# near/near-light-client

Measured on AMD Instinct MI355X. Metric: Sync/Verify proofs/sec at 1/2/4/8 MI355X + achieved HBM GB/s vs roofline, higher is better.
Workload: dtype u64 (Goldilocks field, integer)

## Files before the change

### include/nlx.h

```cpp
#ifndef NLX_H
#define NLX_H
#include <stddef.h>
#include <stdint.h>

#ifdef __cplusplus
extern "C" {
#endif

#define NLX_OK 0
#define NLX_E_INVAL (-1)
#define NLX_E_NOMEM (-2)
#define NLX_E_HIP (-3)
#define NLX_E_RANGE (-4)
#define NLX_E_UNSUPPORTED (-5)

typedef struct nlx_ctx nlx_ctx;
typedef struct nlx_commit nlx_commit;

uint32_t nlx_version(void);
const char* nlx_strerror(int32_t code);
void nlx_field_generators(uint64_t out[2]);
int32_t nlx_abi_selftest(int32_t kind);

int32_t nlx_ctx_create(int device, nlx_ctx** out);
void nlx_ctx_destroy(nlx_ctx* ctx);
const char* nlx_last_error(const nlx_ctx* ctx);
int32_t nlx_ctx_set_stream(nlx_ctx* ctx, void* hip_stream);
int32_t nlx_ctx_synchronize(nlx_ctx* ctx);
int32_t nlx_ctx_set_priority(nlx_ctx* ctx, int high);
int32_t nlx_ctx_set_cu_mask(nlx_ctx* ctx, const uint32_t* mask, uint32_t n_words);
typedef struct nlx_buf nlx_buf;
int32_t nlx_buf_create(nlx_ctx* ctx, size_t bytes, nlx_buf** out);
void nlx_buf_destroy(nlx_buf* buf);
void* nlx_buf_device_ptr(const nlx_buf* buf);
size_t nlx_buf_size(const nlx_buf* buf);
int32_t nlx_buf_upload(nlx_buf* buf, size_t offset, const void* src, size_t bytes);
int32_t nlx_buf_download(nlx_buf* buf, size_t offset, void* dst, size_t bytes);
int32_t nlx_ctx_memory(const nlx_ctx* ctx, size_t* reserved_bytes, size_t* in_use_bytes);
int32_t nlx_ctx_trim(nlx_ctx* ctx);
int32_t nlx_ctx_kernel_timing(nlx_ctx* ctx, int enable);
int32_t nlx_ctx_kernel_stats(nlx_ctx* ctx, const char* name, uint64_t* calls, double* total_ms, double* alg_bytes);
int32_t nlx_ctx_kernel_units(nlx_ctx* ctx, const char* name, double* units);

int32_t nlx_field_ops(nlx_ctx* ctx, const uint64_t* a, const uint64_t* b, size_t n, uint64_t* out);

int32_t nlx_poseidon_permute_batch(nlx_ctx* ctx, uint64_t* states, size_t n);

int32_t nlx_hash_rows(nlx_ctx* ctx, const uint64_t* rows, size_t n_rows, size_t row_len, uint64_t* digests_out);

size_t nlx_merkle_digest_words(size_t n_leaves, uint32_t cap_height);
int32_t nlx_merkle_build(nlx_ctx* ctx, const uint64_t* leaves, size_t n_leaves, size_t leaf_len,
                         uint32_t cap_height, uint64_t* digests_out, uint64_t* cap_out);

int32_t nlx_poseidon_bn128_permute_batch(nlx_ctx* ctx, uint64_t* states, size_t n);
int32_t nlx_poseidon_bn128_hash_rows(nlx_ctx* ctx, const uint64_t* rows, size_t n_rows, size_t row_len, uint64_t* digests_out);
int32_t nlx_poseidon_bn128_merkle_build(nlx_ctx* ctx, const uint64_t* leaves, size_t n_leaves, size_t leaf_len, uint32_t cap_height,
                                        uint64_t* digests_out, uint64_t* cap_out);

int32_t nlx_ntt_batch(nlx_ctx* ctx, uint64_t* cols, size_t n_cols, uint32_t log_n, int inverse,
                      uint64_t coset_shift);

int32_t nlx_ntt_split_level(nlx_ctx* ctx, uint64_t* mine, const uint64_t* theirs, size_t n_cols, uint32_t log_n, uint32_t world_log,
                            uint32_t rank, uint32_t level);

#define NLX_BN254_MONTGOMERY 1u
int32_t nlx_bn254_ntt_batch(nlx_ctx* ctx, uint64_t* cols, size_t n_cols, uint32_t log_n, int inverse, uint32_t flags);
#define NLX_BN254_BITREV_OUT 2u
#define NLX_BN254_BITREV_IN 4u
int32_t nlx_bn254_ntt_batch_coset(nlx_ctx* ctx, uint64_t* cols, size_t n_cols, uint32_t log_n, int inverse, uint32_t flags,
                                  const uint64_t* coset_shift);
int32_t nlx_bn254_msm_g1(nlx_ctx* ctx, const uint64_t* points, const uint64_t* scalars, uint64_t n, uint32_t flags, uint64_t out[8]);
int32_t nlx_bn254_msm_g2(nlx_ctx* ctx, const uint64_t* points, const uint64_t* scalars, uint64_t n, uint32_t flags, uint64_t out[16]);
int32_t nlx_bn254_g1_sum(const uint64_t* points, uint64_t n, uint64_t out[8]);
int32_t nlx_bn254_g2_sum(const uint64_t* points, uint64_t n, uint64_t out[16]);
int32_t nlx_bn254_g1_multiples(nlx_ctx* ctx, const uint64_t base[8], uint64_t n, uint64_t* out);

typedef struct {
    uint32_t log_n;
    uint32_t flags;
    const uint64_t *ql, *qr, *qm, *qo, *qk;
    const uint64_t *s1, *s2, *s3;
    const uint64_t *l, *r, *o;
    const uint64_t *z;
    const uint64_t *pi;
    const uint64_t *coset_shift, *k1, *k2;
    const uint64_t *alpha, *beta, *gamma;
    const uint64_t *blinding;
    uint32_t n_commit;
    const uint64_t *const *qcp;
    const uint64_t *const *pi2;
} nlx_bn254_plonk_quotient_args;
#define NLX_BN254_PLONK_BLINDED 0x100u
#define NLX_BN254_PLONK_COMMIT 0x200u
#define NLX_BN254_PLONK_MAX_COMMIT 4u
int32_t nlx_bn254_plonk_quotient(nlx_ctx* ctx, const nlx_bn254_plonk_quotient_args* args, uint64_t* t_out, int32_t* high_chunk_is_zero);
int32_t nlx_bn254_plonk_grand_product(nlx_ctx* ctx, uint32_t log_n, const uint64_t* l, const uint64_t* r, const uint64_t* o,
                                      const uint64_t* s1, const uint64_t* s2, const uint64_t* s3, const uint64_t beta[4],
// ... 366 lines not shown
```

### near-light-client_amd/__init__.py

```python
from . import _lib as lib
from ._lib import Context, DeviceBuffer, NlxError, GOLDILOCKS_P
from .batch import PolynomialBatch, MerkleTree, poseidon_permute, hash_rows, poseidon_bn128_permute, poseidon_bn128_hash_rows, ntt, field_ops, bn254_ntt, bn254_pack, bn254_unpack, BN254_R, bn254_msm_g1, bn254_g1_pack, bn254_g1_unpack, bn254_g1_sum, bn254_g1_multiples, bn254_g2_pack, bn254_g2_unpack, bn254_msm_g2, bn254_g2_sum, BN254_Q, bn254_plonk_quotient, bn254_kzg_open
from .plonk import CircuitConfig, CircuitData, SyntheticCircuit, WitnessReport, pow_grind, batch_prove, ProveJob
from .stark import Air, Stark, StarkConfig, StarkProver, TraceReport, fibonacci_air, fibonacci_trace, wide_air, wide_trace
from . import sha256_air, sha512_air, logup, fp25519, ed25519_air, nearx_io, near_protocol, stark, plonk, succinct_io, split_ntt, bn254_plonk, bn254_groth16
```

### near-light-client_amd/_lib.py

```python
import ctypes
import os

import numpy as np

GOLDILOCKS_P = 0xFFFFFFFF00000001
_HERE = os.path.dirname(os.path.abspath(__file__))
_GEN_SET = os.environ.get("NLX_GL_GENERATOR_SET", "7")
LIB_PATH = os.path.join(_HERE, "libnlx.so" if _GEN_SET == "7" else "libnlx_gen%s.so" % _GEN_SET)
if os.environ.get("NLX_BUILD_VARIANT"):
    LIB_PATH = LIB_PATH[:-3] + "_" + os.environ["NLX_BUILD_VARIANT"] + ".so"

if os.environ.get("NLX_SKIP_TORCH_PRELOAD") != "1":
    try:
        import torch
    except Exception:
        pass

if not os.path.exists(LIB_PATH):
    raise ImportError(
        "nlx_amd: HIP extension %s not found. Build it with `python near-light-client_amd/build.py` "
        "(or __graft_entry__.build()). There is no CPU fallback." % LIB_PATH)

_dll = ctypes.CDLL(LIB_PATH, mode=ctypes.RTLD_GLOBAL)
SYNTH_LIB_PATH = os.path.join(_HERE, os.path.basename(LIB_PATH).replace("libnlx", "libnlx_synth", 1))
if not os.path.exists(SYNTH_LIB_PATH):
    raise ImportError("nlx_amd: %s not found. Build it with `python near-light-client_amd/build.py`." % SYNTH_LIB_PATH)
_synth_dll = ctypes.CDLL(SYNTH_LIB_PATH)

u64p = ctypes.POINTER(ctypes.c_uint64)
c_void_pp = ctypes.POINTER(ctypes.c_void_p)

SIGNATURES = {
    "nlx_version": (ctypes.c_uint32, []),
    "nlx_strerror": (ctypes.c_char_p, [ctypes.c_int32]),
    "nlx_abi_selftest": (ctypes.c_int32, [ctypes.c_int32]),
    "nlx_field_generators": (None, [ctypes.POINTER(ctypes.c_uint64)]),
    "nlx_ctx_create": (ctypes.c_int32, [ctypes.c_int, c_void_pp]),
    "nlx_ctx_destroy": (None, [ctypes.c_void_p]),
    "nlx_last_error": (ctypes.c_char_p, [ctypes.c_void_p]),
    "nlx_ctx_set_stream": (ctypes.c_int32, [ctypes.c_void_p, ctypes.c_void_p]),
    "nlx_ctx_synchronize": (ctypes.c_int32, [ctypes.c_void_p]),
    "nlx_ctx_set_priority": (ctypes.c_int32, [ctypes.c_void_p, ctypes.c_int]),
    "nlx_ctx_set_cu_mask": (ctypes.c_int32, [ctypes.c_void_p, ctypes.POINTER(ctypes.c_uint32), ctypes.c_uint32]),
    "nlx_buf_create": (ctypes.c_int32, [ctypes.c_void_p, ctypes.c_size_t, c_void_pp]),
    "nlx_buf_destroy": (None, [ctypes.c_void_p]),
    "nlx_buf_device_ptr": (ctypes.c_void_p, [ctypes.c_void_p]),
    "nlx_buf_size": (ctypes.c_size_t, [ctypes.c_void_p]),
    "nlx_buf_upload": (ctypes.c_int32, [ctypes.c_void_p, ctypes.c_size_t, ctypes.c_void_p, ctypes.c_size_t]),
    "nlx_buf_download": (ctypes.c_int32, [ctypes.c_void_p, ctypes.c_size_t, ctypes.c_void_p, ctypes.c_size_t]),
    "nlx_ctx_memory": (ctypes.c_int32, [ctypes.c_void_p, ctypes.POINTER(ctypes.c_size_t), ctypes.POINTER(ctypes.c_size_t)]),
    "nlx_ctx_trim": (ctypes.c_int32, [ctypes.c_void_p]),
    "nlx_ctx_kernel_timing": (ctypes.c_int32, [ctypes.c_void_p, ctypes.c_int]),
    "nlx_ctx_kernel_stats": (ctypes.c_int32, [ctypes.c_void_p, ctypes.c_char_p, ctypes.POINTER(ctypes.c_uint64),
                                              ctypes.POINTER(ctypes.c_double), ctypes.POINTER(ctypes.c_double)]),
    "nlx_ctx_kernel_units": (ctypes.c_int32, [ctypes.c_void_p, ctypes.c_char_p, ctypes.POINTER(ctypes.c_double)]),
    "nlx_field_ops": (ctypes.c_int32, [ctypes.c_void_p, ctypes.c_void_p, ctypes.c_void_p, ctypes.c_size_t, ctypes.c_void_p]),
    "nlx_poseidon_permute_batch": (ctypes.c_int32, [ctypes.c_void_p, ctypes.c_void_p, ctypes.c_size_t]),
    "nlx_hash_rows": (ctypes.c_int32, [ctypes.c_void_p, ctypes.c_void_p, ctypes.c_size_t, ctypes.c_size_t,
                                       ctypes.c_void_p]),
    "nlx_merkle_digest_words": (ctypes.c_size_t, [ctypes.c_size_t, ctypes.c_uint32]),
    "nlx_merkle_build": (ctypes.c_int32, [ctypes.c_void_p, ctypes.c_void_p, ctypes.c_size_t, ctypes.c_size_t,
                                          ctypes.c_uint32, ctypes.c_void_p, ctypes.c_void_p]),
    "nlx_poseidon_bn128_permute_batch": (ctypes.c_int32, [ctypes.c_void_p, ctypes.c_void_p, ctypes.c_size_t]),
    "nlx_poseidon_bn128_hash_rows": (ctypes.c_int32, [ctypes.c_void_p, ctypes.c_void_p, ctypes.c_size_t, ctypes.c_size_t,
                                                      ctypes.c_void_p]),
    "nlx_poseidon_bn128_merkle_build": (ctypes.c_int32, [ctypes.c_void_p, ctypes.c_void_p, ctypes.c_size_t, ctypes.c_size_t,
                                                         ctypes.c_uint32, ctypes.c_void_p, ctypes.c_void_p]),
    "nlx_ntt_batch": (ctypes.c_int32, [ctypes.c_void_p, ctypes.c_void_p, ctypes.c_size_t, ctypes.c_uint32,
                                       ctypes.c_int, ctypes.c_uint64]),
    "nlx_ntt_split_level": (ctypes.c_int32, [ctypes.c_void_p, ctypes.c_void_p, ctypes.c_void_p, ctypes.c_size_t, ctypes.c_uint32, ctypes.c_uint32,
                                              ctypes.c_uint32, ctypes.c_uint32]),
    "nlx_bn254_ntt_batch": (ctypes.c_int32, [ctypes.c_void_p, ctypes.c_void_p, ctypes.c_size_t, ctypes.c_uint32, ctypes.c_int,
                                              ctypes.c_uint32]),
    "nlx_bn254_ntt_batch_coset": (ctypes.c_int32, [ctypes.c_void_p, ctypes.c_void_p, ctypes.c_size_t, ctypes.c_uint32, ctypes.c_int,
                                                    ctypes.c_uint32, ctypes.c_void_p]),
    "nlx_bn254_msm_g1": (ctypes.c_int32, [ctypes.c_void_p, ctypes.c_void_p, ctypes.c_void_p, ctypes.c_uint64, ctypes.c_uint32,
                                           ctypes.c_void_p]),
    "nlx_bn254_g1_sum": (ctypes.c_int32, [ctypes.c_void_p, ctypes.c_uint64, ctypes.c_void_p]),
    "nlx_bn254_g2_sum": (ctypes.c_int32, [ctypes.c_void_p, ctypes.c_uint64, ctypes.c_void_p]),
    "nlx_bn254_msm_g2": (ctypes.c_int32, [ctypes.c_void_p, ctypes.c_void_p, ctypes.c_void_p, ctypes.c_uint64, ctypes.c_uint32,
                                           ctypes.c_void_p]),
    "nlx_bn254_g1_multiples": (ctypes.c_int32, [ctypes.c_void_p, ctypes.c_void_p, ctypes.c_uint64, ctypes.c_void_p]),
    "nlx_bn254_plonk_quotient": (ctypes.c_int32, [ctypes.c_void_p, ctypes.c_void_p, ctypes.c_void_p, ctypes.POINTER(ctypes.c_int32)]),
    "nlx_bn254_plonk_grand_product": (ctypes.c_int32, [ctypes.c_void_p, ctypes.c_uint32] + [ctypes.c_void_p] * 11 + [ctypes.POINTER(ctypes.c_int32)]),
    "nlx_bn254_fr_lincomb": (ctypes.c_int32, [ctypes.c_void_p, ctypes.c_uint64, ctypes.c_uint32, ctypes.c_void_p, ctypes.c_void_p, ctypes.c_void_p]),
    "nlx_bn254_groth16_quotient": (ctypes.c_int32, [ctypes.c_void_p, ctypes.c_uint32] + [ctypes.c_void_p] * 5),
    "nlx_bn254_kzg_open": (ctypes.c_int32, [ctypes.c_void_p, ctypes.c_void_p, ctypes.c_uint64, ctypes.c_void_p, ctypes.c_void_p,
                                            ctypes.c_void_p, ctypes.c_void_p, ctypes.c_void_p]),
    "nlx_bn254_groth16_key_create": (ctypes.c_int32, [ctypes.c_void_p, ctypes.c_void_p, c_void_pp]),
    "nlx_bn254_groth16_key_destroy": (None, [ctypes.c_void_p]),
    "nlx_bn254_groth16_key_info": (ctypes.c_int32, [ctypes.c_void_p, ctypes.c_void_p]),
    "nlx_bn254_r1cs_eval": (ctypes.c_int32, [ctypes.c_void_p] * 6),
    "nlx_bn254_groth16_prove": (ctypes.c_int32, [ctypes.c_void_p] * 11),
    "nlx_bn254_groth16_key_create_committed": (ctypes.c_int32, [ctypes.c_void_p, ctypes.c_void_p, ctypes.c_void_p, c_void_pp]),
    "nlx_bn254_groth16_commit": (ctypes.c_int32, [ctypes.c_void_p, ctypes.c_void_p, ctypes.c_uint32, ctypes.c_void_p, ctypes.c_void_p]),
    "nlx_bn254_groth16_prove_committed": (ctypes.c_int32, [ctypes.c_void_p] * 14),
    "nlx_bn254_plonk_key_create": (ctypes.c_int32, [ctypes.c_void_p, ctypes.c_void_p, c_void_pp]),
    "nlx_bn254_plonk_key_destroy": (None, [ctypes.c_void_p]),
    "nlx_bn254_plonk_key_info": (ctypes.c_int32, [ctypes.c_void_p, ctypes.c_void_p]),
    "nlx_bn254_plonk_key_commitments": (ctypes.c_int32, [ctypes.c_void_p, ctypes.c_void_p]),
    "nlx_bn254_plonk_proof_bytes": (ctypes.c_size_t, [ctypes.c_void_p]),
    "nlx_bn254_plonk_commit": (ctypes.c_int32, [ctypes.c_void_p, ctypes.c_void_p, ctypes.c_uint32, ctypes.c_void_p, ctypes.c_void_p,
                                                 ctypes.c_void_p, ctypes.c_void_p]),
    "nlx_bn254_plonk_prove": (ctypes.c_int32, [ctypes.c_void_p] * 6 + [ctypes.c_uint64, ctypes.c_void_p, ctypes.c_void_p, ctypes.c_void_p,
                                                                       ctypes.c_size_t, ctypes.POINTER(ctypes.c_size_t)]),
    "nlx_bn254_fr_eval_many": (ctypes.c_int32, [ctypes.c_void_p, ctypes.c_uint32, ctypes.c_void_p, ctypes.c_void_p, ctypes.c_void_p,
                                                 ctypes.c_void_p]),
    "nlx_bn254_hash_to_field": (ctypes.c_int32, [ctypes.c_void_p, ctypes.c_size_t, ctypes.c_void_p, ctypes.c_size_t, ctypes.c_void_p]),
    "nlx_commit_from_values": (ctypes.c_int32, [ctypes.c_void_p, ctypes.c_void_p, ctypes.c_size_t, ctypes.c_uint32,
# ... 239 lines not shown
```

### near-light-client_amd/airgen.py

```python
import os
import sys
import types

import numpy as np

HERE = os.path.dirname(os.path.abspath(__file__))
OUT_DIR = os.path.join(HERE, "csrc", "airgen")
P = 0xFFFFFFFF00000001
MASK64 = (1 << 64) - 1

(LOCAL, NEXT, PUBLIC, CONST, ADD, SUB, MUL, EMIT_TRANSITION, EMIT_FIRST, EMIT_LAST, EMIT, PERIODIC, PACK_LOCAL, PACK_NEXT, EMIT_BOOL,
 LOADV, XOR3, CH, MAJ, SEGMENT, EMIT_LOGUP, MAC) = range(22)


def program_hash(words):
    h = 0xcbf29ce484222325
    for b in np.ascontiguousarray(words, dtype="<u8").tobytes():
        h = ((h ^ b) * 0x100000001b3) & MASK64
    return h


def canonical_words(words):
    out, i = [int(w) for w in words], 0
    while i < len(out):
        if (out[i] & 0xFF) == CONST:
            out[i + 1] %= P
            i += 2
        else:
            i += 1
    return np.array(out, dtype=np.uint64)


def _segments(words):
    segs, lo, i = [], 0, 0
    while i < len(words):
        op = int(words[i]) & 0xFF
        if op == SEGMENT:
            segs.append((lo, i))
            lo = i + 1
        i += 2 if op == CONST else 1
    segs.append((lo, len(words)))
    return segs


def _emit_constraint(lines, expr):
    lines.append("    c = %s;" % expr)
    lines.append("    acc0 = gl::add(gl::mul(acc0, g.a0), c); acc1 = gl::add(gl::mul(acc1, g.a1), c);")


SCHED_EVERY = 4


def _segment_body(words, lo, hi):
    L, i, since = [], lo, 0
    R = lambda k: "r%d" % k
    while i < hi:
        if since >= SCHED_EVERY:
            L.append("    __builtin_amdgcn_sched_barrier(0);")
            since = 0
        if (int(words[i]) & 0xFF) in (LOCAL, NEXT, PUBLIC, CONST, ADD, SUB, MUL, PERIODIC, PACK_LOCAL, PACK_NEXT, XOR3, CH, MAJ, MAC):
            since += 1
        w = int(words[i])
        op, dst, a, b, sh = w & 0xFF, (w >> 8) & 0xFFFF, (w >> 24) & 0xFFFF, (w >> 40) & 0xFFFF, (w >> 56) & 0x3F
        i += 1
        if op == LOCAL:
            L.append("    %s = COL(%d, g.row);" % (R(dst), a))
        elif op == NEXT:
            L.append("    %s = COL(%d, g.row_next);" % (R(dst), a))
        elif op == PUBLIC:
            L.append("    %s = PIS(%d);" % (R(dst), a))
        elif op == PERIODIC:
            L.append("    %s = g.per[(size_t)%d * g.per_stride + g.per_off];" % (R(dst), a))
        elif op == CONST:
            L.append("    %s = 0x%016xull;" % (R(dst), int(words[i]) % P))
            i += 1
        elif op == ADD:
            L.append("    %s = gl::add(%s, mul_pow2(%s, %d));" % (R(dst), R(a), R(b), sh) if sh else "    %s = gl::add(%s, %s);" % (R(dst), R(a), R(b)))
        elif op == SUB:
            L.append("    %s = gl::sub(%s, mul_pow2(%s, %d));" % (R(dst), R(a), R(b), sh) if sh else "    %s = gl::sub(%s, %s);" % (R(dst), R(a), R(b)))
        elif op == MUL:
            L.append("    %s = gl::mul(%s, %s);" % (R(dst), R(a), R(b)))
        elif op == MAC:
            L.append("    %s = gl::add(%s, gl::mul(%s, %s));" % (R(dst), R(sh), R(a), R(b)))
        elif op == CH:
            L.append("    %s = gl::add(%s, gl::mul(%s, gl::sub(%s, %s)));" % (R(dst), R(sh), R(a), R(b), R(sh)))
        elif op in (XOR3, MAJ):
            L.append("    { const uint64_t xy = gl::mul(%s, %s), sx = gl::sub(gl::add(%s, %s), gl::add(xy, xy));" % (R(a), R(b), R(a), R(b)))
            if op == XOR3:
                L.append("      const uint64_t sz = gl::mul(sx, %s); %s = gl::sub(gl::add(sx, %s), gl::add(sz, sz)); }" % (R(sh), R(dst), R(sh)))
            else:
                L.append("      %s = gl::add(xy, gl::mul(%s, sx)); }" % (R(dst), R(sh)))
        elif op in (PACK_LOCAL, PACK_NEXT):
            row = "g.row" if op == PACK_LOCAL else "g.row_next"
            L.append("    { uint64_t v[%d];" % b)
            for k in range(b):
                L.append("      v[%d] = COL(%d, %s);" % (k, a + k, row))
            L.append("      uint64_t acc = 0;")
            for k in range(b):
                L.append("      acc = gl::add(acc, mul_pow2(v[%d], %d));" % (k, k))
            L.append("      %s = acc; }" % R(dst))
        elif op == EMIT_BOOL:
            cnt = b if b else 1
            for i0 in range(0, cnt, 8):
                m = min(8, cnt - i0)
                L.append("    { uint64_t v[%d];" % m)
                for k in range(m):
                    L.append("      v[%d] = COL(%d, g.row);" % (k, a + i0 + k))
                for k in range(m):
                    L.append("      c = gl::mul(v[%d], gl::sub(v[%d], 1)); acc0 = gl::add(gl::mul(acc0, g.a0), c); acc1 = gl::add(gl::mul(acc1, g.a1), c);" % (k, k))
                L.append("    }")
        elif op == EMIT_LOGUP:
            L.append("    { const uint64_t al0 = PIS(g.n_pis + %d), al1 = PIS(g.n_pis + %d);" % (sh, sh + 1))
            L.append("      const uint64_t h0 = COL(%d, g.row), h1 = COL(%d, g.row), v1 = COL(%d, g.row);" % (b, b + 1, a))
            L.append("      uint64_t c0, c1;")
            if dst == 0xFFFF:
                L.append("      const uint64_t d0 = gl::add(al0, v1);")
                L.append("      c0 = gl::sub(gl::add(gl::mul(h0, d0), mul_pow2(gl::mul(h1, al1), 3)), gl::add(gl::mul(h1, al1), 1));")
                L.append("      c1 = gl::add(gl::mul(h0, al1), gl::mul(h1, d0));")
            else:
                L.append("      const uint64_t v2 = COL(%d, g.row);" % dst)
                L.append("      const uint64_t s2 = gl::add(gl::add(al0, al0), gl::add(v1, v2));")
                L.append("      const uint64_t a1sq = gl::mul(al1, al1);")
                L.append("      const uint64_t u0 = gl::add(gl::mul(gl::add(al0, v1), gl::add(al0, v2)), gl::sub(mul_pow2(a1sq, 3), a1sq));")
                L.append("      const uint64_t u1 = gl::mul(al1, s2);")
                L.append("      const uint64_t hu = gl::mul(h1, u1);")
                L.append("      c0 = gl::sub(gl::add(gl::mul(h0, u0), gl::sub(mul_pow2(hu, 3), hu)), s2);")
                L.append("      c1 = gl::sub(gl::add(gl::mul(h0, u1), gl::mul(h1, u0)), gl::add(al1, al1));")
            L.append("      acc0 = gl::add(gl::mul(gl::add(gl::mul(acc0, g.a0), c0), g.a0), c1);")
            L.append("      acc1 = gl::add(gl::mul(gl::add(gl::mul(acc1, g.a1), c0), g.a1), c1); }")
        elif op == LOADV:
            L.append("    __builtin_amdgcn_sched_barrier(0);")
        elif op == EMIT_TRANSITION:
            _emit_constraint(L, "gl::mul(%s, g.z_last)" % R(a))
        elif op == EMIT_FIRST:
            _emit_constraint(L, "gl::mul(%s, g.l_first)" % R(a))
        elif op == EMIT_LAST:
            _emit_constraint(L, "gl::mul(%s, g.l_last)" % R(a))
        elif op == EMIT:
            _emit_constraint(L, R(a))
        else:
            raise ValueError("unknown opcode %d at word %d" % (op, i - 1))
    return L


def _registers_of(words, lo, hi):
    regs, i = set(), lo
    while i < hi:
        w = int(words[i])
        op = w & 0xFF
        if op in (LOCAL, NEXT, PUBLIC, CONST, ADD, SUB, MUL, PERIODIC, PACK_LOCAL, PACK_NEXT, XOR3, CH, MAJ, MAC):
            regs.add((w >> 8) & 0xFFFF)
        i += 2 if op == CONST else 1
    return sorted(regs)


PART_WORDS = 10000


def generate_sources(name, words):
    words = canonical_words(words)
    h = program_hash(words)
    segs = _segments(words)
    parts, cur, cur_words = [], [], 0
    for lo, hi in segs:
        if cur and cur_words + (hi - lo) > PART_WORDS:
            parts.append(cur)
            cur, cur_words = [], 0
        cur.append((lo, hi))
        cur_words += hi - lo
    parts.append(cur)
    files = {}
    for pi, part in enumerate(parts):
        ns = "airgen_%s_p%d" % (name, pi)
        out = ["// GENERATED by near-light-client_amd/airgen.py from the program words of AIR '%s' (%d words, %d segments, hash 0x%016x):" % (name, len(words), len(segs), h),
               "// part %d of %d, segments starting at words %s." % (pi + 1, len(parts), ", ".join(str(lo) for lo, _ in part)),
               "// Do not edit: the interpreter k_air_quotient (stark.hip) runs the same words and is the parity reference.",
               '#include "../air_vm.hpp"', "", "namespace nlx {", "namespace %s {" % ns, "",
               "// what a segment needs of the point: passed BY VALUE (registers); the wave-uniform members are made scalar again inside",
               "// the function (readfirstlane), so a column's base address is a scalar load and its element ONE vector load",
               "// The column-pointer table and the public inputs are the same for every lane and constant for the launch: read through the",
               "// constant address space they are scalar loads (s_load), and a column's value is then ONE global load with the pointer in",
               "// SGPRs and the row's byte offset in a VGPR.  Through plain pointers hipcc made each a per-lane flat load with a wait",
               "// between the pointer and the value (two memory latencies per column, two more VGPRs per load in flight).",
               "// row / row_next are BYTE offsets (LDE rows * 8 < 2^32: the host selects these kernels for LDEs of <= 2^28 rows only).",
               "typedef const uint64_t __attribute__((address_space(4)))* airgen_kptr;",
               "typedef const char __attribute__((address_space(1)))* airgen_gptr;",
               "#define COL(c, off) (*(const uint64_t __attribute__((address_space(1)))*)((airgen_gptr)((airgen_kptr)g.cols)[c] + (off)))",
               "#define PIS(i) (((airgen_kptr)g.pis)[i])",
               "struct G {", "    uint64_t cols, pis; const uint64_t* per;",
               "    size_t per_stride, per_off; uint64_t a0, a1, z_last, l_first, l_last; uint32_t row, row_next, n_pis;", "};",
               "struct Acc { uint64_t a0, a1; };",
               "template <typename T> __device__ __forceinline__ T* uni(T* p) {",
               "    const uint64_t v = (uint64_t)p;",
               "    return (T*)(((uint64_t)(uint32_t)__builtin_amdgcn_readfirstlane((int)(v >> 32)) << 32) | (uint32_t)__builtin_amdgcn_readfirstlane((int)v));",
               "}",
               "__device__ __forceinline__ uint64_t uni(uint64_t v) {",
               "    return ((uint64_t)(uint32_t)__builtin_amdgcn_readfirstlane((int)(v >> 32)) << 32) | (uint32_t)__builtin_amdgcn_readfirstlane((int)v);",
               "}", ""]
        for lo, hi in part:
            regs = _registers_of(words, lo, hi)
            out.append("static __device__ __noinline__ Acc seg_%d(G gv) {" % lo)
            out.append("    G g = gv;")
            out.append("    g.cols = uni(gv.cols); g.pis = uni(gv.pis); g.per = uni(gv.per); g.per_stride = uni((uint64_t)gv.per_stride);")
            out.append("    g.a0 = uni(gv.a0); g.a1 = uni(gv.a1); g.n_pis = (uint32_t)__builtin_amdgcn_readfirstlane((int)gv.n_pis);")
            out.append("    uint64_t c, acc0 = 0, acc1 = 0;")
            if regs:
                out.append("    uint64_t %s;" % ", ".join("r%d" % r for r in regs))
            out += _segment_body(words, lo, hi)
            out.append("    return Acc{acc0, acc1};")
            out.append("}")
            out.append("")
        out += [
            "// the interpreter's prologue and epilogue (csrc/stark.hip k_air_quotient), the program between them as a switch on the segment",
            "__global__ __launch_bounds__(AIRGEN_BLOCK) void kernel(AirParams p) {",
            "    const uint32_t sg = blockIdx.y;",
            "    const uint32_t first = p.n_seg > 1 ? p.seg[2 * sg] : 0u;",
            "    if (%s) return;   // another part's segment" % " && ".join("first != %du" % lo for lo, _ in part),
            "    const size_t pos = (size_t)blockIdx.x * blockDim.x + threadIdx.x;",
            "    const unsigned log_Q = p.log_n + p.qdb;",
            "    if (pos >> log_Q) return;",
            "    const size_t n = (size_t)1 << p.log_n;",
            "    const uint32_t rq = (uint32_t)(pos >> p.log_n), k = (uint32_t)(pos & (n - 1));",
            "    const uint32_t r = rq << (p.rate_bits - p.qdb);",
            "    const size_t qrow_next = ((size_t)rq << p.log_n) + ((k + 1) & (n - 1));",
            "    const uint64_t x = gl::mul(p.coset_base[rq], root_pow_(p.w_n_table, k, (uint32_t)(n >> 1)));",
            "    const uint64_t zh = gl::inv(p.zh_inv[rq]);",
            "    G g;",
            "    g.cols = (uint64_t)p.cols; g.pis = (uint64_t)p.pis; g.per = p.periodic; g.n_pis = p.n_pis;",
            "    g.row = (uint32_t)((((size_t)r << p.log_n) + k) << 3); g.row_next = (uint32_t)((((size_t)r << p.log_n) + ((k + 1) & (n - 1))) << 3);",
            "    g.per_stride = (size_t)1 << (p.qdb + p.period_bits);",
            "    g.per_off = ((size_t)rq << p.period_bits) + (k & ((1u << p.period_bits) - 1));",
            "    g.a0 = p.alphas[0]; g.a1 = p.alphas[1];",
            "    g.z_last = gl::sub(x, p.g_inv); g.l_first = gl::mul(zh, p.l_inv[pos]); g.l_last = gl::mul(zh, p.l_inv[qrow_next]);",
            "    Acc acc{0, 0};",
            "    switch (first) {",
        ]
        for lo, _ in part:
            out.append("        case %d: acc = seg_%d(g); break;" % (lo, lo))
        out += [
            "        default: break;",
            "    }",
            "    const size_t Q = (size_t)1 << log_Q;",
            "    if (p.n_seg > 1) {",
            "        uint64_t* dst = p.part + (((size_t)sg * p.nc) << log_Q) + pos;",
            "        dst[0] = gl::mul(acc.a0, p.seg_mul[2 * sg]);",
            "        dst[Q] = gl::mul(acc.a1, p.seg_mul[2 * sg + 1]);",
            "        return;",
            "    }",
            "    const uint64_t zi = p.zh_inv[rq];",
            "    p.out[pos] = gl::mul(acc.a0, zi);",
            "    p.out[Q + pos] = gl::mul(acc.a1, zi);",
            "}",
            "",
            "}  // namespace %s" % ns,
            "void airgen_launch_%s_p%d(hipStream_t st, unsigned tiles, unsigned n_segments, const AirParams& p) {" % (name, pi),
            "    hipLaunchKernelGGL(%s::kernel, dim3(tiles, n_segments), dim3(AIRGEN_BLOCK), 0, st, p);" % ns,
            "}",
            "}  // namespace nlx", ""]
        files["air_%s_p%d.hip" % (name, pi)] = "\n".join(out)
    main = ["// GENERATED by near-light-client_amd/airgen.py: AIR '%s' (%d words, %d segments in %d parts, hash 0x%016x)." % (name, len(words), len(segs), len(parts), h),
            '#include "../air_vm.hpp"', "", "namespace nlx {"]
    main += ["void airgen_launch_%s_p%d(hipStream_t st, unsigned tiles, unsigned n_segments, const AirParams& p);" % (name, pi) for pi in range(len(parts))]
    main += ["static void airgen_launch_%s(hipStream_t st, unsigned tiles, unsigned n_segments, const AirParams& p) {" % name]
    main += ["    airgen_launch_%s_p%d(st, tiles, n_segments, p);" % (name, pi) for pi in range(len(parts))]
    main += ["}",
             "#if !defined(__HIP_DEVICE_COMPILE__)   // a host object (it holds a host function's address): not for the device pass",
             'extern const AirGenEntry airgen_entry_%s = {0x%016xull, %du, "%s", airgen_launch_%s};' % (name, h, len(words), name, name),
             "#endif",
             "}  // namespace nlx", ""]
    files["air_%s.hip" % name] = "\n".join(main)
    return files


def registry_source(names):
    out = ["// GENERATED by near-light-client_amd/airgen.py: the table nlx_stark_build searches (csrc/air_vm.hpp airgen_find).",
           '#include "../air_vm.hpp"', "", "namespace nlx {"]
    out += ["extern const AirGenEntry airgen_entry_%s;" % n for n in names]
    out += ["", "#if !defined(__HIP_DEVICE_COMPILE__)", "const AirGenEntry* airgen_find(uint64_t program_hash, uint32_t n_words) {",
            "    static const AirGenEntry* const table[] = {%s};" % ", ".join(["&airgen_entry_%s" % n for n in names] + ["nullptr"]),
            "    for (const AirGenEntry* const* e = table; *e; e++)",
            "        if ((*e)->program_hash == program_hash && (*e)->n_words == n_words) return *e;",
            "    return nullptr;", "}", "#endif", "}  // namespace nlx", ""]
    return "\n".join(out)


# ... 54 lines not shown
```

### near-light-client_amd/batch.py

```python
import ctypes

import numpy as np

from ._lib import dll, ptr


def poseidon_permute(ctx, states):
    s = np.ascontiguousarray(states, dtype=np.uint64).copy()
    if s.ndim != 2 or s.shape[1] != 12:
        raise ValueError("states must have shape (n, 12)")
    ctx.check(dll.nlx_poseidon_permute_batch(ctx.handle, ptr(s), s.shape[0]))
    return s


def field_ops(ctx, a, b):
    a = np.ascontiguousarray(a, dtype=np.uint64)
    b = np.ascontiguousarray(b, dtype=np.uint64)
    out = np.zeros((5, a.size), dtype=np.uint64)
    ctx.check(dll.nlx_field_ops(ctx.handle, ptr(a), ptr(b), a.size, ptr(out)))
    return out


def hash_rows(ctx, rows):
    r = np.ascontiguousarray(rows, dtype=np.uint64)
    out = np.zeros((r.shape[0], 4), dtype=np.uint64)
    ctx.check(dll.nlx_hash_rows(ctx.handle, ptr(r), r.shape[0], r.shape[1], ptr(out)))
    return out


def ntt(ctx, cols, inverse=False, coset_shift=1):
    c = np.ascontiguousarray(cols, dtype=np.uint64).copy()
    n = c.shape[1]
    log_n = n.bit_length() - 1
    if 1 << log_n != n:
        raise ValueError("length must be a power of two")
    ctx.check(dll.nlx_ntt_batch(ctx.handle, ptr(c), c.shape[0], log_n, 1 if inverse else 0, int(coset_shift)))
    return c


HASHERS = {"poseidon_goldilocks": 0, "poseidon_bn128": 1}


def _hasher_id(hasher):
    if hasher not in HASHERS:
        raise ValueError("hasher must be one of %s" % ", ".join(sorted(HASHERS)))
    return HASHERS[hasher]


class MerkleTree:

    def __init__(self, ctx, leaves, cap_height, hasher="poseidon_goldilocks"):
        build = (dll.nlx_merkle_build, dll.nlx_poseidon_bn128_merkle_build)[_hasher_id(hasher)]
        lv = np.ascontiguousarray(leaves, dtype=np.uint64)
        self.n_leaves, self.leaf_len = lv.shape
        self.cap_height = cap_height
        self.hasher = hasher
        words = dll.nlx_merkle_digest_words(self.n_leaves, cap_height)
        if words == 0:
            raise ValueError("n_leaves must be a power of two")
        self.digests = np.zeros(words, dtype=np.uint64)
        self.cap = np.zeros((1 << cap_height, 4), dtype=np.uint64)
        ctx.check(build(ctx.handle, ptr(lv), self.n_leaves, self.leaf_len, cap_height, ptr(self.digests), ptr(self.cap)))
        self.leaves = lv

    def prove(self, leaf_index):
        sib, off, lvl, idx = [], 0, self.n_leaves, leaf_index
        while lvl > (1 << self.cap_height):
            s = off + (idx ^ 1) * 4
            sib.append(self.digests[s:s + 4].copy())
            off += lvl * 4
            lvl >>= 1
            idx >>= 1
# ... 362 lines not shown
```

### near-light-client_amd/build.py

```python
import os
import subprocess
import sys
from concurrent.futures import ThreadPoolExecutor

HERE = os.path.dirname(os.path.abspath(__file__))
CSRC = os.path.join(HERE, "csrc")
GEN_SET = os.environ.get("NLX_GL_GENERATOR_SET", "7")
if GEN_SET not in ("7", "2021"):
    raise RuntimeError("NLX_GL_GENERATOR_SET must be 7 or 2021")
_SUFFIX = "" if GEN_SET == "7" else "_gen" + GEN_SET
VARIANT = os.environ.get("NLX_BUILD_VARIANT", "")
if VARIANT:
    _SUFFIX += "_" + VARIANT
OBJ = os.path.join(CSRC, ".obj" + _SUFFIX)
LIB = os.path.join(HERE, "libnlx%s.so" % _SUFFIX)
SYNTH_SOURCES = ("synth.cpp",)
SYNTH_LIB = os.path.join(HERE, "libnlx_synth%s.so" % _SUFFIX)
HIPCC = os.environ.get("HIPCC", "/opt/rocm/bin/hipcc")
ARCH = "gfx950"
FLAGS = ["-O3", "-std=c++17", "-fPIC", "--offload-arch=" + ARCH, "-Xarch_host", "-mavx2", "-Wall", "-Wno-unused-function",
         "-I", os.path.join(HERE, "..", "include"), "-DNLX_GL_GENERATOR_SET=" + GEN_SET] + os.environ.get("NLX_EXTRA_FLAGS", "").split()


AIRGEN = os.path.join(CSRC, "airgen")


def _generate_air_kernels():
    r = subprocess.run([sys.executable, os.path.join(HERE, "airgen.py")], capture_output=True, text=True)
    if r.returncode != 0:
        raise RuntimeError("airgen.py failed:\n%s\n%s" % (r.stdout, r.stderr))


WITH_AIRGEN = GEN_SET == "7" and os.environ.get("NLX_NO_AIRGEN", "") != "1"
if not WITH_AIRGEN:
    FLAGS.append("-DNLX_NO_AIRGEN")


def _sources():
    top = sorted(f for f in os.listdir(CSRC) if f.endswith((".hip", ".cpp")))
    gen = sorted(os.path.join("airgen", f) for f in os.listdir(AIRGEN) if f.endswith(".hip")) if WITH_AIRGEN and os.path.isdir(AIRGEN) else []
    return top + gen


def _headers_mtime(only=None):
    m = 0.0
    for root in (CSRC, os.path.join(HERE, "..", "include")):
        for f in os.listdir(root):
            if f.endswith((".hpp", ".h", ".inc")) and (only is None or f in only):
                m = max(m, os.path.getmtime(os.path.join(root, f)))
    return m


AIRGEN_HEADERS = ("air_vm.hpp", "gl.hpp", "nlx.h", "nlx_field.h")


def _compile(src, verbose):
    obj = os.path.join(OBJ, src.replace(os.sep, "_") + ".o")
    cmd = [HIPCC] + FLAGS + ["-c", os.path.join(CSRC, src), "-o", obj]
    if verbose:
        print(" ".join(cmd), flush=True)
    r = subprocess.run(cmd, capture_output=True, text=True)
    if r.returncode != 0:
        raise RuntimeError("hipcc failed for %s:\n%s\n%s" % (src, r.stdout, r.stderr))
    if verbose and r.stderr.strip():
        print(r.stderr, file=sys.stderr)
    return obj


def build_lib(force=False, verbose=False):
    os.makedirs(OBJ, exist_ok=True)
    if WITH_AIRGEN:
        _generate_air_kernels()
    hm, hm_gen = _headers_mtime(), _headers_mtime(AIRGEN_HEADERS)
    todo, objs, synth_objs = [], [], []
    for src in _sources():
        obj = os.path.join(OBJ, src.replace(os.sep, "_") + ".o")
        (synth_objs if src in SYNTH_SOURCES else objs).append(obj)
        sm = max(os.path.getmtime(os.path.join(CSRC, src)), hm_gen if src.startswith("airgen" + os.sep) else hm)
        if force or not os.path.exists(obj) or os.path.getmtime(obj) < sm:
            todo.append(src)
    if todo:
        todo.sort(key=lambda s_: -os.path.getsize(os.path.join(CSRC, s_)))
        with ThreadPoolExecutor(max_workers=min(8, len(todo))) as ex:
            list(ex.map(lambda s: _compile(s, verbose), todo))
    for lib, members in ((LIB, objs), (SYNTH_LIB, synth_objs)):
        if todo or not os.path.exists(lib):
            cmd = [HIPCC, "-shared", "-fPIC", "--offload-arch=" + ARCH, "-o", lib] + members + os.environ.get("NLX_EXTRA_LDFLAGS", "").split()
            if verbose:
                print(" ".join(cmd), flush=True)
            r = subprocess.run(cmd, capture_output=True, text=True)
            if r.returncode != 0:
                raise RuntimeError("link failed:\n%s\n%s" % (r.stdout, r.stderr))
    return LIB


if __name__ == "__main__":
    print(build_lib(force="--force" in sys.argv, verbose=True))
```

### near-light-client_amd/csrc/air_vm.hpp

```cpp
#pragma once
#include <hip/hip_runtime.h>
#include <cstdint>
#include "gl.hpp"
#include "nlx.h"

namespace nlx {

struct AirParams {
    const uint64_t* const* cols;
    const uint64_t* program;
    const uint64_t* pis;
    const uint64_t* coset_base;
    const uint64_t* zh_inv;
    const uint64_t* l_inv;
    const uint64_t* periodic;
    const uint64_t* w_n_table;
    uint64_t* out;
    const uint32_t* seg;
    const uint64_t* seg_mul;
    uint64_t* part;
    uint32_t n_seg;
    uint64_t alphas[2];
    uint64_t g_inv;
    uint32_t log_n, rate_bits, qdb, n_words, nc, n_regs, period_bits, n_pis;
};

__device__ __forceinline__ uint64_t mul_pow2(uint64_t x, uint32_t sh) {
    if (sh == 0) return x;
    return gl::reduce128(x << sh, x >> (64 - sh));
}

__device__ __forceinline__ uint64_t root_pow_(const uint64_t* __restrict__ half_table, uint32_t e, uint32_t half) {
    return e < half ? half_table[e] : gl::P - half_table[e - half];
}


struct AirGenEntry {
    uint64_t program_hash;
    uint32_t n_words;
    const char* name;
    void (*launch)(hipStream_t st, unsigned tiles, unsigned n_segments, const AirParams& p);
};
constexpr unsigned AIRGEN_BLOCK = 256;
inline uint64_t airgen_program_hash(const uint64_t* words, size_t n) {
    uint64_t h = 0xcbf29ce484222325ull;
    for (size_t i = 0; i < n; i++)
        for (int b = 0; b < 8; b++) {
            h ^= (words[i] >> (8 * b)) & 0xFF;
            h *= 0x100000001b3ull;
        }
    return h;
}
#if defined(NLX_NO_AIRGEN)
inline const AirGenEntry* airgen_find(uint64_t, uint32_t) { return nullptr; }
#else
const AirGenEntry* airgen_find(uint64_t program_hash, uint32_t n_words);
#endif

}
```

### near-light-client_amd/csrc/commit.hip

```cpp
#include "commit.hpp"
#include "gl.hpp"
#include "poly.hpp"

namespace nlx {

size_t merkle_digest_words(size_t n_leaves, uint32_t cap_height) {
    size_t w = 0, lvl = n_leaves, cap = (size_t)1 << cap_height;
    for (;;) {
        w += lvl * 4;
        if (lvl <= cap) break;
        lvl >>= 1;
    }
    return w;
}

nlx_commit commit_view(const nlx_commit* c, uint32_t k) {
    nlx_commit v = *c;
    v.owner = false;
    v.n_trees = 1;
    v.group_digests = nullptr;
    if (c->n_trees > 1) {
        const uint32_t c0 = k * c->batch_cols;
        v.n_cols = c->n_cols - c0 < c->batch_cols ? c->n_cols - c0 : c->batch_cols;
        v.coeffs_br = c->coeffs_br + (size_t)c0 * c->n();
// ... 101 lines not shown
        ctx->end_kernel();
    } else {
        ctx->begin_kernel("hash_lde_leaves", 8.0 * n_cols * L + 32.0 * L, n_cols <= 4 ? 0.0 : (double)L * ((n_cols + 7) / 8));
        launch_hash_lde_leaves(st, c->lde, L, n_cols, log_n, rate_bits, c->digests);
        ctx->end_kernel();
    }
    if (!bn128) {
        ctx->begin_kernel("merkle_levels", 64.0 * L * c->n_trees, ((double)L - (double)((size_t)1 << cap_height)) * c->n_trees);
        c->cap = launch_merkle_levels(st, c->digests, L, cap_height, c->n_trees, c->tree_words);
        ctx->end_kernel();
    }
    hipError_t e = hipGetLastError();
    if (e != hipSuccess) {
        ctx->release(c->coeffs_br);
        ctx->release(c->lde);
        ctx->release(c->digests);
        ctx->release(c->group_digests);
        delete c;
        return ctx->hip_fail(e, "commit_build launch");
    }
    *out = c;
    return NLX_OK;
}

static int32_t copy_out(nlx_ctx* ctx, void* user, const void* dev, size_t bytes) {
    hipError_t e = hipMemcpyAsync(user, dev, bytes, is_device_ptr(user) ? hipMemcpyDeviceToDevice : hipMemcpyDeviceToHost,
                                  ctx->stream);
    if (e != hipSuccess) return ctx->hip_fail(e, "hipMemcpyAsync(out)");
    return NLX_OK;
}

}

using namespace nlx;

extern "C" {

int32_t nlx_field_ops(nlx_ctx* ctx, const uint64_t* a, const uint64_t* b, size_t n, uint64_t* out) NLX_TRY {
    if (!ctx) return NLX_E_INVAL;
    if (n == 0) return NLX_OK;
    if (!a || !b || !out) return ctx->fail(NLX_E_INVAL, "NULL buffer");
    (void)hipSetDevice(ctx->device);
    Staged sa(ctx, a, n * 8, true, false), sb(ctx, b, n * 8, true, false), so(ctx, out, 5 * n * 8, false, true);
    if (sa.status) return sa.status;
    if (sb.status) return sb.status;
    if (so.status) return so.status;
    launch_field_ops(ctx->stream, sa.as<uint64_t>(), sb.as<uint64_t>(), n, so.as<uint64_t>());
    int32_t rc = so.finish();
    if (rc) return rc;
    NLX_HIP(ctx, hipStreamSynchronize(ctx->stream));
    return NLX_OK;
} NLX_CATCH(ctx)

int32_t nlx_poseidon_permute_batch(nlx_ctx* ctx, uint64_t* states, size_t n) NLX_TRY {
    if (!ctx) return NLX_E_INVAL;
    if (n == 0) return NLX_OK;
    if (!states) return ctx->fail(NLX_E_INVAL, "states is NULL");
    (void)hipSetDevice(ctx->device);
    Staged s(ctx, states, n * 12 * 8, true, true);
    if (s.status) return s.status;
    launch_permute_batch(ctx->stream, s.as<uint64_t>(), n);
    int32_t rc = s.finish();
    if (rc) return rc;
    NLX_HIP(ctx, hipStreamSynchronize(ctx->stream));
    return NLX_OK;
} NLX_CATCH(ctx)

int32_t nlx_hash_rows(nlx_ctx* ctx, const uint64_t* rows, size_t n_rows, size_t row_len, uint64_t* digests_out) NLX_TRY {
    if (!ctx) return NLX_E_INVAL;
    if (n_rows == 0) return NLX_OK;
    if (!digests_out || (!rows && row_len)) return ctx->fail(NLX_E_INVAL, "NULL buffer");
    if (row_len > 0xFFFFFFFFull) return ctx->fail(NLX_E_RANGE, "row_len too large");
    (void)hipSetDevice(ctx->device);
    Staged in(ctx, rows, n_rows * row_len * 8, true, false);
    Staged out(ctx, digests_out, n_rows * 32, false, true);
    if (in.status) return in.status;
    if (out.status) return out.status;
    launch_hash_leaves_rowmajor(ctx->stream, in.as<uint64_t>(), (uint32_t)row_len, n_rows, out.as<uint64_t>());
    int32_t rc = out.finish();
    if (rc) return rc;
    NLX_HIP(ctx, hipStreamSynchronize(ctx->stream));
    return NLX_OK;
} NLX_CATCH(ctx)

size_t nlx_merkle_digest_words(size_t n_leaves, uint32_t cap_height) NLX_TRY {
    if (n_leaves == 0 || (n_leaves & (n_leaves - 1)) || cap_height > 63) return 0;
    return merkle_digest_words(n_leaves, cap_height);
} NLX_CATCH_VALUE(nullptr, 0)

int32_t nlx_merkle_build(nlx_ctx* ctx, const uint64_t* leaves, size_t n_leaves, size_t leaf_len, uint32_t cap_height,
                         uint64_t* digests_out, uint64_t* cap_out) NLX_TRY {
    if (!ctx) return NLX_E_INVAL;
    if (n_leaves == 0 || (n_leaves & (n_leaves - 1))) return ctx->fail(NLX_E_INVAL, "n_leaves must be a power of two");
    if (cap_height > 63 || ((size_t)1 << cap_height) > n_leaves)
        return ctx->fail(NLX_E_RANGE, "cap_height %u exceeds log2(n_leaves)", cap_height);
    if (!cap_out || (!leaves && leaf_len)) return ctx->fail(NLX_E_INVAL, "NULL buffer");
    if (leaf_len > 0xFFFFFFFFull) return ctx->fail(NLX_E_RANGE, "leaf_len too large");
    (void)hipSetDevice(ctx->device);
    size_t words = merkle_digest_words(n_leaves, cap_height);
    Staged in(ctx, leaves, n_leaves * leaf_len * 8, true, false);
    if (in.status) return in.status;
    Scratch scratch(ctx);
    const bool own_dig = !(digests_out && is_device_ptr(digests_out));
    uint64_t* d_dig = own_dig ? scratch.alloc_as<uint64_t>(words * 8) : digests_out;
    if (!d_dig) return NLX_E_NOMEM;
    launch_hash_leaves_rowmajor(ctx->stream, in.as<uint64_t>(), (uint32_t)leaf_len, n_leaves, d_dig);
// ... 261 lines not shown
```

### near-light-client_amd/csrc/gl.hpp

```cpp
#pragma once
#include <stdint.h>
#include <stddef.h>
#include "nlx_field.h"

#if defined(__HIP__)
#include <hip/hip_runtime.h>
#define GL_HD __host__ __device__ __forceinline__
#define GL_H __host__ inline
#else
#define GL_HD inline
#define GL_H inline
#endif

namespace gl {

constexpr uint64_t P = 0xFFFFFFFF00000001ULL;
constexpr uint64_t EPS = 0xFFFFFFFFULL;
constexpr uint64_t GEN = NLX_GL_MULTIPLICATIVE_GROUP_GENERATOR;
constexpr uint64_t POW2_GEN = NLX_GL_POWER_OF_TWO_GENERATOR;
constexpr unsigned TWO_ADICITY = 32;
constexpr uint64_t W = 7;

GL_HD uint64_t mulhi64(uint64_t a, uint64_t b) {
#if defined(__HIP_DEVICE_COMPILE__)
// ... 68 lines not shown
        : "vcc");
    uint64_t r;
    asm("v_mad_u64_u32 %[r], vcc, %[m], 1, %[s]" : [r] "=&v"(r) : [m] "v"(m), [s] "v"(((uint64_t)s1 << 32) | s0) : "vcc");
    return r;
}
#endif
GL_H uint64_t add_loose(uint64_t a, uint64_t c) {
    uint64_t s = a + c;
    return s < a ? s + EPS : s;
}

GL_HD uint64_t reduce128_loose(uint64_t lo, uint64_t hi) {
    uint64_t hi_hi = hi >> 32, hi_lo = hi & EPS;
    uint64_t t0 = lo - hi_hi;
    if (lo < hi_hi) t0 -= EPS;
    uint64_t t1 = (hi_lo << 32) - hi_lo;
    uint64_t r = t0 + t1;
    if (r < t1) r += EPS;
    return r;
}
GL_HD uint64_t reduce128(uint64_t lo, uint64_t hi) { return canon(reduce128_loose(lo, hi)); }

#if defined(__HIP_DEVICE_COMPILE__)
__device__ __forceinline__ uint64_t mul_loose_asm(uint64_t a, uint64_t b) {
    const uint32_t a0 = (uint32_t)a, a1 = (uint32_t)(a >> 32), b0 = (uint32_t)b, b1 = (uint32_t)(b >> 32);
    const uint64_t p0 = (uint64_t)a0 * b0;
    const uint64_t p1 = (uint64_t)a0 * b1 + (p0 >> 32);
    const uint64_t p2 = (uint64_t)a1 * b0 + (uint32_t)p1;
    uint64_t p3 = (uint64_t)a1 * b1 + (p1 >> 32), sink;
    asm("v_mad_u64_u32 %0, %1, %2, 1, %3" : "=v"(p3), "=s"(sink) : "v"((uint32_t)(p2 >> 32)), "v"(p3));
    uint32_t r0, r1, t0;
    const uint32_t w2 = (uint32_t)p3;
    asm("v_sub_co_u32 %[r0], vcc, %[w0], %[w3]\n\t"
        "v_subbrev_co_u32 %[r1], vcc, 0, %[w1], vcc\n\t"
        "v_cndmask_b32_e64 %[t0], 0, -1, vcc\n\t"
        "v_sub_co_u32 %[r0], vcc, %[r0], %[t0]\n\t"
        "v_subbrev_co_u32 %[r1], vcc, 0, %[r1], vcc"
        : [r0] "=&v"(r0), [r1] "=&v"(r1), [t0] "=&v"(t0)
        : [w0] "v"((uint32_t)p0), [w1] "v"((uint32_t)p2), [w3] "v"((uint32_t)(p3 >> 32))
        : "vcc");
    const uint64_t base = ((uint64_t)r1 << 32) | r0;
    uint64_t r;
    uint32_t tm;
    asm("v_mad_u64_u32 %[r], vcc, %[w2], -1, %[base]\n\t"
        "v_cndmask_b32_e64 %[t], 0, -1, vcc\n\t"
        "v_mad_u64_u32 %[r], vcc, %[t], 1, %[r]"
        : [r] "=&v"(r), [t] "=&v"(tm)
        : [w2] "v"(w2), [base] "v"(base)
        : "vcc");
    return r;
}
#endif

GL_HD uint64_t mul_loose(uint64_t a, uint64_t b) {
#if defined(__HIP_DEVICE_COMPILE__)
    return mul_loose_asm(a, b);
#else
    return reduce128_loose(a * b, mulhi64(a, b));
#endif
}
GL_HD uint64_t mul(uint64_t a, uint64_t b) { return canon(mul_loose(a, b)); }
GL_HD uint64_t sqr(uint64_t a) { return mul(a, a); }

GL_HD uint64_t pow(uint64_t b, uint64_t e) {
    uint64_t r = 1;
    while (e) {
        if (e & 1) r = mul(r, b);
        b = sqr(b);
        e >>= 1;
    }
    return r;
}
GL_HD uint64_t exp_pow2(uint64_t a, unsigned k) {
    while (k--) a = sqr(a);
    return a;
}
GL_HD uint64_t inv(uint64_t a) {
    uint64_t t2 = mul(sqr(a), a);
    uint64_t t3 = mul(sqr(t2), a);
    uint64_t t6 = mul(exp_pow2(t3, 3), t3);
    uint64_t t12 = mul(exp_pow2(t6, 6), t6);
    uint64_t t24 = mul(exp_pow2(t12, 12), t12);
    uint64_t t30 = mul(exp_pow2(t24, 6), t6);
    uint64_t t31 = mul(sqr(t30), a);
    uint64_t t32 = mul(sqr(t31), a);
    return mul(exp_pow2(t31, 33), t32);
}
GL_HD uint64_t root_of_unity(unsigned n_log) { return exp_pow2(POW2_GEN, TWO_ADICITY - n_log); }

struct Ext {
    uint64_t a, b;
};
GL_HD Ext ext(uint64_t a, uint64_t b = 0) { return Ext{a, b}; }
GL_HD Ext add(Ext x, Ext y) { return Ext{add(x.a, y.a), add(x.b, y.b)}; }
GL_HD Ext sub(Ext x, Ext y) { return Ext{sub(x.a, y.a), sub(x.b, y.b)}; }
GL_HD Ext mul(Ext x, Ext y) {
    uint64_t bb = mul(x.b, y.b);
    uint64_t c0 = add(mul(x.a, y.a), reduce128(bb * W, mulhi64(bb, W)));
    uint64_t c1 = add(mul(x.a, y.b), mul(x.b, y.a));
    return Ext{c0, c1};
}
GL_HD Ext mul(Ext x, uint64_t s) { return Ext{mul(x.a, s), mul(x.b, s)}; }
GL_HD Ext inv(Ext x) {
    uint64_t n = sub(sqr(x.a), mul(W, sqr(x.b)));
    uint64_t ni = inv(n);
    return Ext{mul(x.a, ni), mul(neg(x.b), ni)};
}
GL_HD Ext pow(Ext b, uint64_t e) {
    Ext r{1, 0};
    while (e) {
        if (e & 1) r = mul(r, b);
        b = mul(b, b);
        e >>= 1;
    }
    return r;
}
GL_HD bool eq(Ext x, Ext y) { return x.a == y.a && x.b == y.b; }

GL_HD uint32_t bitrev32(uint32_t x, unsigned bits) {
#if defined(__HIP_DEVICE_COMPILE__)
    return bits ? (__brev(x) >> (32 - bits)) : 0;
#else
    uint32_t r = 0;
    for (unsigned i = 0; i < bits; i++) r |= ((x >> i) & 1u) << (bits - 1 - i);
    return r;
#endif
}

}
```

### near-light-client_amd/csrc/poly.hpp

```cpp
#pragma once
#include <hip/hip_runtime.h>
#include <stdint.h>
#include <stddef.h>

namespace nlx {
size_t eval_scratch_words(uint32_t n_cols, unsigned log_n);
void launch_eval_br(hipStream_t st, const uint64_t* d_coeffs_br, size_t stride, uint32_t n_cols, unsigned log_n,
                    const uint64_t* d_z, uint64_t* d_out_ext, uint64_t* d_scratch, const uint64_t* d_zpow = nullptr);
void launch_gather_rows(hipStream_t st, const uint64_t* d_lde, size_t col_stride, uint32_t n_cols, unsigned log_n,
                        unsigned rate_bits, const uint64_t* d_idx, size_t k, uint64_t* d_rows_out);
void launch_gather_paths(hipStream_t st, const uint64_t* d_digests, unsigned log_leaves, unsigned cap_height,
                         const uint64_t* d_idx, size_t k, uint64_t* d_paths_out);
void launch_table_to_leaves(hipStream_t st, const uint64_t* d_lde, size_t col_stride, uint32_t n_cols,
                            unsigned log_n, unsigned rate_bits, uint64_t* d_leaves);
void launch_field_ops(hipStream_t st, const uint64_t* d_a, const uint64_t* d_b, size_t n, uint64_t* d_out);
}
```

### near-light-client_amd/csrc/poly_kernels.hip

```cpp
#include <hip/hip_runtime.h>
#include "gl.hpp"
#include "launch.hpp"
#include "poly.hpp"

namespace nlx {

constexpr unsigned EVAL_CHUNK_LOG = 11;

__device__ __forceinline__ gl::Ext shfl_down_ext(gl::Ext v, int d) {
    gl::Ext r;
    r.a = ((uint64_t)__shfl_down((uint32_t)(v.a >> 32), d, 64) << 32) | __shfl_down((uint32_t)v.a, d, 64);
    r.b = ((uint64_t)__shfl_down((uint32_t)(v.b >> 32), d, 64) << 32) | __shfl_down((uint32_t)v.b, d, 64);
    return r;
}

template <bool EXT_IN>
__global__ __launch_bounds__(256) void k_eval_fold(const uint64_t* __restrict__ in, size_t in_stride,
                                                   unsigned log_count,
                                                   unsigned level0,
                                                   unsigned log_n, const uint64_t* __restrict__ zpow,
                                                   uint64_t* __restrict__ out, size_t out_stride) {
    __shared__ uint64_t wave_part[8];
    const unsigned tid = threadIdx.x;
    const unsigned log_chunk = log_count < EVAL_CHUNK_LOG ? log_count : EVAL_CHUNK_LOG;
// ... 234 lines not shown
                       d_idx, k, d_rows_out);
}

__global__ void k_gather_paths(const uint64_t* __restrict__ digests, unsigned log_leaves, unsigned cap_height,
                               const uint64_t* __restrict__ idx, size_t k, uint64_t* __restrict__ paths_out) {
    size_t q = blockIdx.x;
    unsigned path_len = log_leaves - cap_height;
    unsigned lvl = threadIdx.x >> 2, w = threadIdx.x & 3;
    if (q >= k || lvl >= path_len) return;
    if (idx[q] >> log_leaves) return;
    size_t L = (size_t)1 << log_leaves;
    size_t off = 4 * (2 * L - (2 * L >> lvl));
    size_t node = (idx[q] >> lvl) ^ 1;
    paths_out[(q * path_len + lvl) * 4 + w] = digests[off + node * 4 + w];
}
void launch_gather_paths(hipStream_t st, const uint64_t* d_digests, unsigned log_leaves, unsigned cap_height,
                         const uint64_t* d_idx, size_t k, uint64_t* d_paths_out) {
    if (!k || log_leaves <= cap_height) return;
    hipLaunchKernelGGL(k_gather_paths, dim3((unsigned)k), dim3(128), 0, st, d_digests, log_leaves, cap_height, d_idx,
                       k, d_paths_out);
}

__global__ void k_table_to_leaves(const uint64_t* __restrict__ lde, size_t col_stride, uint32_t n_cols,
                                  unsigned log_n, unsigned rate_bits, uint64_t* __restrict__ leaves) {
    size_t leaf = (size_t)blockIdx.x * blockDim.x + threadIdx.x;
    if (leaf >> (log_n + rate_bits)) return;
    size_t pos = leaf_to_pos(leaf, log_n, rate_bits);
    for (uint32_t c = 0; c < n_cols; c++) leaves[leaf * n_cols + c] = lde[(size_t)c * col_stride + pos];
}
void launch_table_to_leaves(hipStream_t st, const uint64_t* d_lde, size_t col_stride, uint32_t n_cols,
                            unsigned log_n, unsigned rate_bits, uint64_t* d_leaves) {
    size_t rows = (size_t)1 << (log_n + rate_bits);
    hipLaunchKernelGGL(k_table_to_leaves, dim3((unsigned)((rows + 255) / 256)), dim3(256), 0, st, d_lde, col_stride,
                       n_cols, log_n, rate_bits, d_leaves);
}

__global__ void k_field_ops(const uint64_t* __restrict__ a, const uint64_t* __restrict__ b, size_t n,
                            uint64_t* __restrict__ out) {
    size_t i = (size_t)blockIdx.x * blockDim.x + threadIdx.x;
    if (i >= n) return;
    const uint64_t ar = a[i], br = b[i];
    const uint64_t x = gl::canon(ar), y = gl::canon(br);
    out[i] = gl::mul(x, y);
    out[n + i] = gl::add(x, y);
    out[2 * n + i] = gl::sub(x, y);
    out[3 * n + i] = x ? gl::inv(x) : 0;
    out[4 * n + i] = gl::canon(gl::mul_loose(ar, br));
}
void launch_field_ops(hipStream_t st, const uint64_t* d_a, const uint64_t* d_b, size_t n, uint64_t* d_out) {
    if (!n) return;
    hipLaunchKernelGGL(k_field_ops, dim3((unsigned)((n + 255) / 256)), dim3(256), 0, st, d_a, d_b, n, d_out);
}

}
```

### near-light-client_amd/csrc/prover.hip

```cpp
#include <algorithm>
#include <cstdlib>
#include <cstring>
#include <vector>
#include "commit.hpp"
#include "gl.hpp"
#include "poly.hpp"
#include "poseidon.hpp"
#include "prover.hpp"
#include "fri.hpp"
#include "transcript.hpp"

using namespace nlx;

namespace {
uint32_t fri_num_rounds(const nlx_circuit_desc& d) {
    return nlx::fri_num_rounds(d.degree_bits, d.rate_bits, d.cap_height, d.fri_arity_bits, d.fri_final_poly_bits);
}

uint32_t gate_num_constraints(const nlx_gate_desc& g) {
    const uint32_t p0 = g.param0, p1 = g.param1;
    switch (g.kind) {
        case NLX_GATE_CONSTANT: case NLX_GATE_ARITHMETIC: return p0;
        case NLX_GATE_PUBLIC_INPUT: return 4;
        case NLX_GATE_BASE_SUM: return 1 + p1;
// ... 127 lines not shown
        if (gt.kind == NLX_GATE_U32_ADD_MANY && (gt.param0 < 1 || gt.param0 > 15 || gt.param1 < 1 || (gt.param0 + 3 + 18) * gt.param1 > d.num_wires))
            return ctx->fail(NLX_E_INVAL, "U32AddManyGate does not fit the wires");
        if (gt.kind == NLX_GATE_U32_ARITHMETIC && (gt.param0 < 1 || (6 + 32) * gt.param0 > d.num_wires)) return ctx->fail(NLX_E_INVAL, "U32ArithmeticGate too wide");
        if (gt.kind == NLX_GATE_U32_SUBTRACTION && (gt.param0 < 1 || (5 + 16) * gt.param0 > d.num_wires)) return ctx->fail(NLX_E_INVAL, "U32SubtractionGate too wide");
        if (gt.kind == NLX_GATE_U32_RANGE_CHECK && (gt.param0 < 1 || 17 * gt.param0 > d.num_wires)) return ctx->fail(NLX_E_INVAL, "U32RangeCheckGate too wide");
        if (gt.kind == NLX_GATE_COMPARISON) {
            const uint32_t cb = gt.param1 ? (gt.param0 + gt.param1 - 1) / gt.param1 : 0;
            if (gt.param1 < 1 || cb < 1 || cb > 3 || cb * gt.param1 > 62 || 4 + 5 * gt.param1 + cb + 1 > d.num_wires)
                return ctx->fail(NLX_E_INVAL, "ComparisonGate: chunk_bits must be in [1, 3] and the gate must fit the wires");
        }
        if (gt.kind == NLX_GATE_COSET_INTERPOLATION) {
            const uint32_t np = gt.param0 <= 5 ? 1u << gt.param0 : 0;
            if (np < 4 || gt.param1 < 2 || gt.param1 > np || d.degree_bits < gt.param0 + 1 ||
                1 + 2 * np + 4 + 4 * ((np - 2) / (gt.param1 - 1)) + 2 > d.num_wires)
                return ctx->fail(NLX_E_INVAL, "CosetInterpolationGate does not fit");
        }
        if (gt.kind == NLX_GATE_RANDOM_ACCESS) {
            const uint32_t bits = gt.param0, copies = gt.param1 & 0xFFFF, extra = gt.param1 >> 16;
            if (bits < 1 || bits > 6 || copies < 1 || extra > d.num_constants ||
                (2 + (1u << bits)) * copies + extra + copies * bits > d.num_wires)
                return ctx->fail(NLX_E_INVAL, "RandomAccessGate does not fit the wires");
        }
        if (gt.kind == NLX_GATE_REDUCING_EXT && (gt.param0 < 1 || 6 + 2 * gt.param0 + 2 * (gt.param0 - 1) > d.num_wires)) return ctx->fail(NLX_E_INVAL, "ReducingExtensionGate too wide");
        if (gt.selector_index >= d.num_selectors || gt.group_end > d.num_gates || gt.group_start > gt.group_end)
            return ctx->fail(NLX_E_INVAL, "gate %u: bad selector group", g);
        if (gt.kind == NLX_GATE_POSEIDON && d.num_wires < 135) return ctx->fail(NLX_E_INVAL, "PoseidonGate needs 135 wires");
        if (gt.kind == NLX_GATE_ARITHMETIC && 4 * gt.param0 > d.num_wires) return ctx->fail(NLX_E_INVAL, "ArithmeticGate too wide");
        if (gt.kind == NLX_GATE_BASE_SUM && 1 + gt.param1 > d.num_wires) return ctx->fail(NLX_E_INVAL, "BaseSumGate too wide");
        if (gt.kind == NLX_GATE_CONSTANT && gt.param0 > d.num_constants) return ctx->fail(NLX_E_INVAL, "ConstantGate too wide");
    }
    if (d.num_luts) {
        if (d.num_luts > 16) return ctx->fail(NLX_E_RANGE, "at most 16 lookup tables");
        if (!d.lut_sizes || !d.lut_pairs || !d.lookup_rows || !d.lut_num_lookups) return ctx->fail(NLX_E_INVAL, "NULL lookup table array");
        const uint32_t n_lu = d.num_routed_wires / 2, n_lut = d.num_routed_wires / 3;
        if (n_lut < 1 || d.quotient_degree_factor < 2) return ctx->fail(NLX_E_INVAL, "too few routed wires for the lookup gates");
        for (uint32_t t = 0; t < d.num_luts; t++) {
            const uint32_t len = d.lut_sizes[t], lookups = d.lut_num_lookups[t];
            const uint32_t last_lu = d.lookup_rows[3 * t], last_lut = d.lookup_rows[3 * t + 1], first_lut = d.lookup_rows[3 * t + 2];
            if (len < 1 || len > 65536 || lookups < 1) return ctx->fail(NLX_E_RANGE, "table %u: 1 .. 65536 entries and at least one lookup", t);
            if (!(last_lu < last_lut && last_lut <= first_lut) || (uint64_t)first_lut + 1 >= ((uint64_t)1 << d.degree_bits))
                return ctx->fail(NLX_E_INVAL, "table %u: lookup rows out of order or past the circuit", t);
            if (last_lut - last_lu != (lookups + n_lu - 1) / n_lu || first_lut - last_lut + 1 != (len + n_lut - 1) / n_lut)
                return ctx->fail(NLX_E_INVAL, "table %u: row counts do not match its lookups / entries", t);
        }
    }
    (void)hipSetDevice(ctx->device);
    nlx_circuit* c = new (std::nothrow) nlx_circuit();
    if (!c) return ctx->fail(NLX_E_NOMEM, "host allocation failed");
    c->ctx = ctx;
    c->d = d;
    c->hasher = hasher;
    c->gates.assign(d.gates, d.gates + d.num_gates);
    for (const nlx_gate_desc& gt : c->gates) c->max_gate_constraints = std::max(c->max_gate_constraints, gate_num_constraints(gt));
    c->k_is.assign(d.k_is, d.k_is + d.num_routed_wires);
    c->d.gates = c->gates.data();
    c->d.k_is = c->k_is.data();
    if (d.num_luts) {
        const uint32_t T = d.num_luts;
        c->lk.num_luts = T;
        c->lk.n_lu_slots = d.num_routed_wires / 2;
        c->lk.n_lut_slots = d.num_routed_wires / 3;
        c->lk.lu_degree = d.quotient_degree_factor - 1;
        c->lk.n_sldc = (c->lk.n_lu_slots + c->lk.lu_degree - 1) / c->lk.lu_degree;
        c->lk.lut_degree = (c->lk.n_lut_slots + c->lk.n_sldc - 1) / c->lk.n_sldc;
        c->n_lk_sel = 4 + T;
        c->n_lk_polys = d.num_challenges * (1 + c->lk.n_sldc);
        c->n_lk_terms = 4 + T + 2 * c->lk.n_sldc;
        c->lut_sizes.assign(d.lut_sizes, d.lut_sizes + T);
        c->lut_num_lookups.assign(d.lut_num_lookups, d.lut_num_lookups + T);
        c->lookup_rows.assign(d.lookup_rows, d.lookup_rows + 3 * T);
        c->lut_offsets.assign(T + 1, 0);
        for (uint32_t t = 0; t < T; t++) c->lut_offsets[t + 1] = c->lut_offsets[t] + c->lut_sizes[t];
        c->lut_pairs.assign(d.lut_pairs, d.lut_pairs + 2 * (size_t)c->lut_offsets[T]);
        c->d.lut_sizes = c->lut_sizes.data(); c->d.lut_num_lookups = c->lut_num_lookups.data();
        c->d.lookup_rows = c->lookup_rows.data(); c->d.lut_pairs = c->lut_pairs.data();
    }
    c->n_consts_all = d.num_selectors + c->n_lk_sel + d.num_constants;
    c->n_cs = c->n_consts_all + d.num_routed_wires;
    c->n_zpp = d.num_challenges * (1 + d.num_partial_products);
    c->n_zs = c->n_zpp + c->n_lk_polys;
    c->n_q = d.num_challenges * d.quotient_degree_factor;
    c->n_fri_rounds = fri_num_rounds(d);
    const size_t n = c->n(), L = c->L();
    const unsigned log_n = d.degree_bits, log_L = d.degree_bits + d.rate_bits;
    const uint32_t R = 1u << d.rate_bits, A = 1u << d.fri_arity_bits;
    int32_t rc = ctx->ensure_tables(log_L);
    auto fail = [&](int32_t code) {
        nlx_circuit_destroy(c);
        return code;
    };
    if (rc) return fail(rc);
    rc = ctx->get_coset_scale(log_n, d.rate_bits, &c->d_inv_scale_br, true);
    if (rc) return fail(rc);
    if (hasher == NLX_HASHER_POSEIDON_BN128) {
        c->d_bad = (uint32_t*)ctx->alloc(256);
        if (!c->d_bad) return fail(NLX_E_NOMEM);
        if (hipMemsetAsync(c->d_bad, 0, 4, ctx->stream) != hipSuccess) return fail(ctx->fail(NLX_E_HIP, "hipMemsetAsync failed"));
    }

    {
        uint64_t* d_vals = (uint64_t*)ctx->alloc((size_t)c->n_cs * n * 8);
        if (!d_vals) return fail(NLX_E_NOMEM);
        const size_t cb = (size_t)c->n_consts_all * n * 8, sb = (size_t)d.num_routed_wires * n * 8;
        hipError_t e1 = hipMemcpyAsync(d_vals, constants, cb, is_device_ptr(constants) ? hipMemcpyDeviceToDevice : hipMemcpyHostToDevice, ctx->stream);
        hipError_t e2 = hipMemcpyAsync((uint8_t*)d_vals + cb, sigmas, sb, is_device_ptr(sigmas) ? hipMemcpyDeviceToDevice : hipMemcpyHostToDevice, ctx->stream);
        if (e1 != hipSuccess || e2 != hipSuccess) { ctx->release(d_vals); return fail(ctx->hip_fail(e1 != hipSuccess ? e1 : e2, "hipMemcpyAsync")); }
// ... 263 lines not shown
    zp.sigmas = c->d_sigma_values;
    zp.k_is = c->d_k_is;
    zp.w_n_table = ctx->tables.fwd[log_n];
    for (int i = 0; i < 2; i++) { zp.betas[i] = betas[i]; zp.gammas[i] = gammas[i]; }
    zp.out = d_zs;
    zp.log_n = log_n; zp.routed = d.num_routed_wires; zp.chunk = d.quotient_degree_factor; zp.nc = d.num_challenges;
    zp.npp = d.num_partial_products;
    launch_zs(ctx->stream, zp, d_zs_scratch);
    if (c->n_lk_polys)
        launch_lookup_polys(ctx->stream, c->lk, c->d_tabs, c->h_tabs.data(), d_wire_values, n, d.num_challenges, d_deltas,
                            d_zs + (size_t)c->n_zpp * n);
    return commit_for(c, d_zs, CommitInput::ValuesNatural, c->n_zs, cz);
}

int32_t quotient_degree_check(nlx_circuit* c, const uint64_t* d_qchunks) {
    nlx_ctx* ctx = c->ctx;
    const nlx_circuit_desc& d = c->d;
    const size_t n = c->n();
    const uint32_t R = 1u << d.rate_bits, nc = d.num_challenges;
    if (n < 2 * (size_t)R) return NLX_OK;
    uint64_t top[2 * 8];
    const size_t stride = n / R;
    int32_t rc = ensure_pinned(ctx, 1u << 20);
    if (rc) return rc;
    for (uint32_t ch = 0; ch < nc; ch++) {
        const uint64_t* src = d_qchunks + ((size_t)ch * R + (R - 1)) * n + (stride - 1);
        NLX_HIP(ctx, hipMemcpy2DAsync((uint64_t*)ctx->pinned + (size_t)ch * R, 8, src, stride * 8, 8, R, hipMemcpyDeviceToHost, ctx->stream));
    }
    NLX_HIP(ctx, hipStreamSynchronize(ctx->stream));
    memcpy(top, ctx->pinned, (size_t)nc * R * 8);
    for (uint32_t i = 0; i < nc * R; i++)
        if (gl::canon(top[i]) != 0)
            return ctx->fail(NLX_E_INVAL, "the witness does not satisfy the circuit: the quotient of challenge %u has degree above %u n - %u (the vanishing polynomial is not divisible by Z_H)",
                             i / R, R, R + 1);
    return NLX_OK;
}

int32_t quotient_stage(nlx_circuit* c, const nlx_commit* cw, const nlx_commit* cz, const uint64_t betas[2],
                       const uint64_t gammas[2], const uint64_t alphas[2], const uint64_t pih[4],
                       const uint64_t* d_deltas, const uint64_t* d_lut_polys, CommitPtr& cq, StageClock& clock, Scratch& scratch) {
    nlx_ctx* ctx = c->ctx;
    const nlx_circuit_desc& d = c->d;
    hipStream_t st = ctx->stream;
    const unsigned log_n = d.degree_bits;
    const size_t L = c->L();
    const uint32_t nc = d.num_challenges, npp = d.num_partial_products;
    c->n_terms = nc + nc * (npp + 1) + nc * c->n_lk_terms + c->max_gate_constraints;
    uint64_t* d_alpha_pows = scratch.alloc_as<uint64_t>((size_t)2 * c->n_terms * 8);
    uint64_t* d_qvals = scratch.alloc_as<uint64_t>((size_t)nc * L * 8);
    uint64_t* d_qchunks = scratch.alloc_as<uint64_t>((size_t)nc * L * 8);
    if (!d_alpha_pows || !d_qvals || !d_qchunks) return NLX_E_NOMEM;
    launch_pow_table(st, d_alpha_pows, alphas[0], alphas[1], c->n_terms, c->n_terms);
    QuotientParams qp{};
    qp.cs = c->cs->lde; qp.wires = cw->lde; qp.zs = cz->lde;
    qp.gates = c->d_gates; qp.k_is = c->d_k_is; qp.coset_base = c->d_coset_base;
    qp.w_n_table = ctx->tables.fwd[log_n];
    qp.zh_inv = c->d_zh_inv; qp.l0_scaled = c->d_l0_scaled; qp.alpha_pows = d_alpha_pows;
    qp.out = d_qvals;
    for (int i = 0; i < 2; i++) { qp.betas[i] = betas[i]; qp.gammas[i] = gammas[i]; }
    for (int i = 0; i < 4; i++) qp.pih[i] = pih[i];
    qp.alpha_stride = c->n_terms;
    qp.num_wires = d.num_wires; qp.work = c->d_work; qp.work_stride = c->work_stride;
    qp.log_n = log_n; qp.rate_bits = d.rate_bits; qp.n_gates = d.num_gates; qp.n_selectors = d.num_selectors;
    qp.n_consts_all = c->n_consts_all; qp.routed = d.num_routed_wires; qp.chunk = d.quotient_degree_factor; qp.nc = nc; qp.npp = npp;
    qp.gate_const0 = d.num_selectors + c->n_lk_sel;
    qp.n_lk_terms = c->n_lk_terms;
    if (c->n_lk_terms) {
        LookupTermsParams lp{};
        lp.cs = c->cs->lde; lp.wires = cw->lde; lp.zs = cz->lde;
        lp.deltas = d_deltas; lp.lut_polys = d_lut_polys; lp.alpha_pows = d_alpha_pows; lp.out = d_qvals;
        lp.alpha_stride = c->n_terms; lp.t_lk = nc + nc * (npp + 1);
        lp.log_n = log_n; lp.rate_bits = d.rate_bits; lp.nc = nc; lp.sel0 = d.num_selectors; lp.lk0 = c->n_zpp;
        lp.n_lk_terms = c->n_lk_terms; lp.s = c->lk;
        ctx->begin_kernel("lookup_terms", 8.0 * L * (c->n_lk_sel + d.num_routed_wires + 2.0 * c->n_lk_polys + nc));
        launch_lookup_terms(st, lp);
        ctx->end_kernel();
        qp.accumulate = 1;
    }
    ctx->begin_kernel("quotient", 8.0 * L * (c->n_cs + d.num_wires + c->n_zs + nc) + 8.0 * L * nc);
    for (uint32_t g : c->poseidon_gates) {
        launch_quotient_poseidon(st, qp, g, qp.accumulate != 0);
        qp.accumulate = 1;
    }
    launch_quotient(st, qp);
    ctx->end_kernel();
    clock.stage("quotient_intt");
    launch_intt_dif_cosets(st, ctx->tables, d_qvals, nc, log_n, d.rate_bits, c->d_inv_scale_br);
    launch_quotient_chunks(st, d_qvals, d_qchunks, log_n, d.rate_bits, nc, c->d_wR_inv, c->d_chunk_scale);
    clock.stage("commit_quotient");
    NLX_RC(commit_for(c, d_qchunks, CommitInput::CoeffsBitrev, c->n_q, cq));
    return c->hasher == NLX_HASHER_POSEIDON_BN128 ? quotient_degree_check(c, d_qchunks) : NLX_OK;
}

struct ProveCall {
    CommitPtr cw, cz, cq;
    uint64_t deltas[8] = {}, lut_polys[2 * 16] = {};
    OpeningPoints points;
    Scratch scratch;
    explicit ProveCall(nlx_ctx* ctx) : scratch(ctx) {}
};

int32_t prove_stages(nlx_circuit* c, ProveCall& pc, const uint64_t* wires, const uint64_t* public_inputs, Writer& w, size_t* proof_len) {
    nlx_ctx* ctx = c->ctx;
    const nlx_circuit_desc& d = c->d;
    hipStream_t st = ctx->stream;
    const size_t n = c->n();
// ... 540 lines not shown
```

### near-light-client_amd/csrc/prover.hpp

```cpp
#pragma once
#include <hip/hip_runtime.h>
#include <stdint.h>
#include <stddef.h>
#include "../../include/nlx.h"

namespace nlx {

struct GateDev {
    uint32_t kind, selector_index, group_start, group_end, index, param0, param1;
};

struct ZsParams {
    const uint64_t* wires;
    size_t wires_stride;
    const uint64_t* sigmas;
    const uint64_t* k_is;
    const uint64_t* w_n_table;
    uint64_t betas[2], gammas[2];
    uint64_t* out;
    uint32_t log_n, routed, chunk, nc, npp;
};
size_t zs_scratch_words(unsigned log_n, uint32_t nc);
void launch_zs(hipStream_t st, const ZsParams& p, uint64_t* d_scratch);

struct QuotientParams {
    const uint64_t* cs;
    const uint64_t* wires;
    const uint64_t* zs;
    const GateDev* gates;
    const uint64_t* k_is;
    const uint64_t* coset_base;
    const uint64_t* w_n_table;
    const uint64_t* zh_inv;
    const uint64_t* l0_scaled;
    const uint64_t* alpha_pows;
    uint64_t* out;
    uint64_t betas[2], gammas[2], pih[4];
    uint32_t alpha_stride;
    uint32_t log_n, rate_bits, n_gates, n_selectors, n_consts_all, routed, chunk, nc, npp;
    uint32_t gate_const0;
    uint32_t n_lk_terms;
    uint32_t accumulate;
    uint32_t num_wires;
    const uint32_t* work;
    uint32_t work_stride;
};
void launch_quotient(hipStream_t st, const QuotientParams& p);
void launch_quotient_poseidon(hipStream_t st, const QuotientParams& p, uint32_t gate, bool add);
size_t quotient_lds_bytes(uint32_t num_wires, uint32_t n_consts_all);
uint32_t quotient_waves();
void launch_l0_table(hipStream_t st, uint64_t* d_out, unsigned log_n, unsigned rate_bits, const uint64_t* d_coset_base,
                     const uint64_t* d_w_n_table);
void launch_quotient_chunks(hipStream_t st, const uint64_t* d_in, uint64_t* d_out, unsigned log_n, unsigned rate_bits,
                            uint32_t nc, const uint64_t* d_w_R_inv_pows, const uint64_t* d_chunk_scale);

struct LookupShape {
    uint32_t num_luts, n_lu_slots, n_lut_slots, lu_degree, lut_degree, n_sldc;
};
struct LookupTableDev {
    uint32_t len, lookups, last_lu, last_lut, first_lut, pad_;
    const uint32_t* pairs;
    const int32_t* idx_of;
    uint32_t* mult;
};
void launch_set_lookup_wires(hipStream_t st, const LookupShape& s, const LookupTableDev* d_tabs, const LookupTableDev* h_tabs,
                             uint64_t* d_wires, size_t n, uint32_t* d_mult_all, size_t mult_words, uint32_t* d_err);
void launch_lookup_polys(hipStream_t st, const LookupShape& s, const LookupTableDev* d_tabs, const LookupTableDev* h_tabs,
                         const uint64_t* d_wires, size_t n, uint32_t nc, const uint64_t* d_deltas, uint64_t* d_cols);
struct LookupTermsParams {
    const uint64_t* cs;
    const uint64_t* wires;
    const uint64_t* zs;
    const uint64_t* deltas;
    const uint64_t* lut_polys;
    const uint64_t* alpha_pows;
    uint64_t* out;
    uint32_t alpha_stride, t_lk;
    uint32_t log_n, rate_bits, nc, sel0, lk0, n_lk_terms;
    LookupShape s;
};
void launch_lookup_terms(hipStream_t st, const LookupTermsParams& p);

struct CheckBlock {
    unsigned long long gate_rows_bad, gate_first;
    unsigned long long copy_cells_bad, copy_first;
    unsigned long long lookup_slots_bad, lookup_first;
    unsigned long long sigma_undecodable;
    unsigned long long gate_value;
// ... 2 lines not shown
constexpr unsigned long long CHECK_NONE = ~0ull;
void launch_check_reset(hipStream_t st, CheckBlock* d_block);
struct CheckGatesParams {
    QuotientParams q;
    const uint64_t* consts;
    const uint64_t* wires;
    CheckBlock* block;
};
void launch_check_gates(hipStream_t st, const CheckGatesParams& p, uint32_t report_row);
void launch_sigma_decode(hipStream_t st, const uint64_t* d_sigmas, const uint64_t* d_k_is, const uint64_t* d_kn, const uint64_t* d_kinv,
                         const uint64_t* d_w_n_table, const uint64_t* d_w_n_inv_table, unsigned log_n, uint32_t routed,
                         uint32_t* d_to_row, uint16_t* d_to_col, CheckBlock* d_block);
void launch_check_copies(hipStream_t st, const uint64_t* d_wires, unsigned log_n, uint32_t routed, const uint32_t* d_to_row,
                         const uint16_t* d_to_col, CheckBlock* d_block);
void launch_check_lookups(hipStream_t st, const LookupShape& s, const LookupTableDev* d_tabs, const LookupTableDev* h_tabs,
                          const uint64_t* d_wires, size_t n, CheckBlock* d_block);

constexpr int FRI_VIEWS = 33;
struct FriCombineParams {
    const uint64_t* tables[FRI_VIEWS];
    uint32_t n_cols[FRI_VIEWS];
    const uint64_t* alpha_pows;
    const uint64_t* coset_base;
    const uint64_t* w_n_table;
    uint64_t zeta[2], gzeta[2], c0[2], c1[2], alpha_nz[2];
    uint64_t* out;
    uint32_t log_n, rate_bits;
    uint32_t nz[FRI_VIEWS];
    uint32_t nz_off[FRI_VIEWS];
};
size_t fri_combine_scratch_words(const FriCombineParams& p);
void launch_fri_combine(hipStream_t st, const FriCombineParams& p, uint64_t* scratch);
void launch_fri_leaves(hipStream_t st, const uint64_t* d_values, unsigned log_n, unsigned rate_bits,
                       unsigned arity_bits, uint64_t* d_digests);
void launch_fri_leaves_wide(hipStream_t st, const uint64_t* d_values, unsigned log_n, unsigned rate_bits,
                            unsigned arity_bits, uint64_t* d_digests);
void launch_fri_fold(hipStream_t st, const uint64_t* d_values, uint64_t* d_out, unsigned log_n, unsigned rate_bits,
                     unsigned arity_bits, const uint64_t beta[2], uint64_t shift_inv, const uint64_t* d_w_L_inv_table,
                     const uint64_t* d_w_A_inv_pows);
void launch_fri_final_coeffs(hipStream_t st, const uint64_t* d_values, unsigned log_n, unsigned rate_bits,
                             uint64_t shift, uint64_t* d_out, uint32_t n_out);

struct PowParams {
    uint64_t state[12];
    uint64_t max_rounds;
    uint32_t pos, bits;
};
void launch_pow_grind(hipStream_t st, const PowParams& p, unsigned long long* d_best);
void launch_fri_gather_leaf(hipStream_t st, const uint64_t* d_values, unsigned log_n, unsigned rate_bits,
                            unsigned arity_bits, const uint64_t* d_leaf_idx, uint32_t n_q, uint64_t* d_out,
                            size_t out_stride_words);
void launch_shift_indices(hipStream_t st, const uint64_t* d_in, uint64_t* d_out, uint32_t n, unsigned shift);
void launch_pow_table(hipStream_t st, uint64_t* d_out, uint64_t a0, uint64_t a1, uint32_t count, uint32_t stride);
void launch_ext_pow_table(hipStream_t st, uint64_t* d_out, const uint64_t alpha[2], uint32_t count);

}
```

### near-light-client_amd/csrc/prover_kernels.hip

```cpp
#include <hip/hip_runtime.h>
#include "gl.hpp"
#include "poseidon.hpp"
#include "poseidon_fast_constants.inc"
#include "prover.hpp"

namespace nlx {

__constant__ static const uint64_t FAST_FIRST[12] = NLX_POSEIDON_FAST_FIRST_RC_INIT;
__constant__ static const uint64_t FAST_RC[22] = NLX_POSEIDON_FAST_RC_INIT;
__constant__ static const uint64_t FAST_VS[22][11] = NLX_POSEIDON_FAST_VS_INIT;
__constant__ static const uint64_t FAST_W[22][11] = NLX_POSEIDON_FAST_W_HATS_INIT;
__constant__ static const uint64_t FAST_INIT[11][11] = NLX_POSEIDON_FAST_INITIAL_MATRIX_INIT;

__device__ __forceinline__ uint64_t root_pow(const uint64_t* __restrict__ half_table, uint32_t e, uint32_t half) {
    return e < half ? half_table[e] : gl::P - half_table[e - half];
}

__global__ __launch_bounds__(256) void k_zs_row_products(ZsParams p) {
    const size_t i = (size_t)blockIdx.x * blockDim.x + threadIdx.x;
    const size_t n = (size_t)1 << p.log_n;
    if (i >= n) return;
    const uint64_t x = root_pow(p.w_n_table, (uint32_t)i, (uint32_t)(n >> 1));
    constexpr int MAXQ = 10;
    uint64_t num[2 * MAXQ], den[2 * MAXQ];
    const uint32_t n_chunks = (p.routed + p.chunk - 1) / p.chunk;
    const uint64_t bx0 = gl::mul(p.betas[0], x), bx1 = gl::mul(p.betas[1], x);
#pragma unroll
    for (int q = 0; q < MAXQ; q++) {
        uint64_t nm0 = 1, dn0 = 1, nm1 = 1, dn1 = 1;
        if ((uint32_t)q < n_chunks) {
            for (uint32_t j = q * p.chunk; j < (q + 1) * p.chunk && j < p.routed; j++) {
                const uint64_t w = p.wires[(size_t)j * p.wires_stride + i];
                const uint64_t sg = p.sigmas[(size_t)j * n + i];
                const uint64_t kj = p.k_is[j];
                nm0 = gl::mul(nm0, gl::add(gl::add(w, gl::mul(bx0, kj)), p.gammas[0]));
                dn0 = gl::mul(dn0, gl::add(gl::add(w, gl::mul(p.betas[0], sg)), p.gammas[0]));
                if (p.nc > 1) {
                    nm1 = gl::mul(nm1, gl::add(gl::add(w, gl::mul(bx1, kj)), p.gammas[1]));
                    dn1 = gl::mul(dn1, gl::add(gl::add(w, gl::mul(p.betas[1], sg)), p.gammas[1]));
                }
            }
        }
        num[q] = nm0;
        den[q] = dn0;
        num[MAXQ + q] = nm1;
        den[MAXQ + q] = dn1;
    }
    uint64_t pref[2 * MAXQ];
    uint64_t acc = 1;
#pragma unroll
    for (int t = 0; t < 2 * MAXQ; t++) {
        pref[t] = acc;
        acc = gl::mul(acc, den[t]);
    }
// ... 60 lines not shown
        run = gl::mul(run, v[k]);
    }
    if (threadIdx.x == 255) totals[(size_t)blockIdx.y * totals_stride + blockIdx.x] = run;
}

__global__ __launch_bounds__(256) void k_scan_mul_apply(uint64_t* __restrict__ data, size_t stride, size_t count,
                                                        const uint64_t* __restrict__ prefix, size_t prefix_stride) {
    const size_t i = (size_t)blockIdx.x * blockDim.x + threadIdx.x;
    if (i >= count) return;
    uint64_t* col = data + (size_t)blockIdx.y * stride;
    const uint64_t f = prefix[(size_t)blockIdx.y * prefix_stride + i / SCAN_ELEMS];
    col[i] = gl::mul(col[i], f);
}

__global__ __launch_bounds__(256) void k_zs_apply(uint64_t* __restrict__ out, unsigned log_n, uint32_t nc, uint32_t npp) {
    const size_t i = (size_t)blockIdx.x * blockDim.x + threadIdx.x;
    const size_t n = (size_t)1 << log_n;
    if (i >= n) return;
    const uint32_t c = blockIdx.y / npp, q = blockIdx.y % npp;
    const uint64_t z = out[(size_t)c * n + i];
    uint64_t* pp = out + (size_t)(nc + c * npp + q) * n;
    pp[i] = gl::mul(pp[i], z);
}

void launch_zs(hipStream_t st, const ZsParams& p, uint64_t* d_scratch) {
    const size_t n = (size_t)1 << p.log_n;
    const unsigned blocks = (unsigned)((n + 255) / 256);
    hipLaunchKernelGGL(k_zs_row_products, dim3(blocks), dim3(256), 0, st, p);
    size_t count = n;
    size_t nb = (count + SCAN_ELEMS - 1) / SCAN_ELEMS;
    uint64_t* tot1 = d_scratch;
    uint64_t* tot2 = d_scratch + p.nc * nb;
    hipLaunchKernelGGL(k_scan_mul_local, dim3((unsigned)nb, p.nc), dim3(256), 0, st, p.out, n, count, tot1, nb);
    if (nb > 1) {
        size_t nb2 = (nb + SCAN_ELEMS - 1) / SCAN_ELEMS;
        hipLaunchKernelGGL(k_scan_mul_local, dim3((unsigned)nb2, p.nc), dim3(256), 0, st, tot1, nb, nb, tot2, nb2);
        if (nb2 > 1) {
            uint64_t* tot3 = tot2 + p.nc * nb2;
            hipLaunchKernelGGL(k_scan_mul_local, dim3(1, p.nc), dim3(256), 0, st, tot2, nb2, nb2, tot3, (size_t)1);
            hipLaunchKernelGGL(k_scan_mul_apply, dim3((unsigned)((nb + 255) / 256), p.nc), dim3(256), 0, st, tot1, nb, nb,
                               tot2, nb2);
        }
        hipLaunchKernelGGL(k_scan_mul_apply, dim3(blocks, p.nc), dim3(256), 0, st, p.out, n, count, tot1, nb);
    }
    hipLaunchKernelGGL(k_zs_apply, dim3(blocks, p.nc * p.npp), dim3(256), 0, st, p.out, p.log_n, p.nc, p.npp);
}
size_t zs_scratch_words(unsigned log_n, uint32_t nc) {
    size_t n = (size_t)1 << log_n;
    size_t nb = (n + SCAN_ELEMS - 1) / SCAN_ELEMS;
    size_t nb2 = (nb + SCAN_ELEMS - 1) / SCAN_ELEMS;
    return nc * (nb + nb2 + 2) + 16;
}

struct GateAcc {
    const uint64_t* __restrict__ ap0;
    const uint64_t* __restrict__ ap1;
    uint64_t a[8];
    uint32_t kc[8];
    uint32_t k;
    uint64_t base[2];
    __device__ __forceinline__ void reset() {
#pragma unroll
        for (int i = 0; i < 8; i++) { a[i] = 0; kc[i] = 0; }
        k = 0;
        base[0] = base[1] = 0;
    }
    __device__ __forceinline__ void stash() {
        base[0] = gl::add(base[0], fold_columns(a, kc));
        base[1] = gl::add(base[1], fold_columns(a + 4, kc + 4));
#pragma unroll
        for (int i = 0; i < 8; i++) { a[i] = 0; kc[i] = 0; }
    }
    __device__ __forceinline__ void emit_at(uint32_t idx, uint64_t c) { mac(c, ap0[idx], ap1[idx]); }
    __device__ __forceinline__ void mac(uint64_t c, uint64_t b0, uint64_t b1) {
        const uint32_t c0 = (uint32_t)c, c1 = (uint32_t)(c >> 32);
        asm("v_mad_u64_u32 %[a0], vcc, %[c0], %[p0], %[a0]\n\t"
            "v_addc_co_u32 %[k0], vcc, 0, %[k0], vcc\n\t"
            "v_mad_u64_u32 %[a1], vcc, %[c0], %[p1], %[a1]\n\t"
            "v_addc_co_u32 %[k1], vcc, 0, %[k1], vcc\n\t"
            "v_mad_u64_u32 %[a2], vcc, %[c1], %[p0], %[a2]\n\t"
            "v_addc_co_u32 %[k2], vcc, 0, %[k2], vcc\n\t"
            "v_mad_u64_u32 %[a3], vcc, %[c1], %[p1], %[a3]\n\t"
            "v_addc_co_u32 %[k3], vcc, 0, %[k3], vcc\n\t"
            "v_mad_u64_u32 %[a4], vcc, %[c0], %[q0], %[a4]\n\t"
            "v_addc_co_u32 %[k4], vcc, 0, %[k4], vcc\n\t"
            "v_mad_u64_u32 %[a5], vcc, %[c0], %[q1], %[a5]\n\t"
            "v_addc_co_u32 %[k5], vcc, 0, %[k5], vcc\n\t"
            "v_mad_u64_u32 %[a6], vcc, %[c1], %[q0], %[a6]\n\t"
            "v_addc_co_u32 %[k6], vcc, 0, %[k6], vcc\n\t"
            "v_mad_u64_u32 %[a7], vcc, %[c1], %[q1], %[a7]\n\t"
            "v_addc_co_u32 %[k7], vcc, 0, %[k7], vcc"
            : [a0] "+v"(a[0]), [a1] "+v"(a[1]), [a2] "+v"(a[2]), [a3] "+v"(a[3]), [a4] "+v"(a[4]), [a5] "+v"(a[5]),
              [a6] "+v"(a[6]), [a7] "+v"(a[7]), [k0] "+v"(kc[0]), [k1] "+v"(kc[1]), [k2] "+v"(kc[2]), [k3] "+v"(kc[3]),
              [k4] "+v"(kc[4]), [k5] "+v"(kc[5]), [k6] "+v"(kc[6]), [k7] "+v"(kc[7])
            : [c0] "v"(c0), [c1] "v"(c1), [p0] "s"((uint32_t)b0), [p1] "s"((uint32_t)(b0 >> 32)), [q0] "s"((uint32_t)b1),
              [q1] "s"((uint32_t)(b1 >> 32))
            : "vcc");
    }
    __device__ __forceinline__ void emit(uint64_t c) { emit_at(k++, c); }
    __device__ __forceinline__ uint64_t finish(int ch) const { return gl::add(fold_columns(a + 4 * ch, kc + 4 * ch), base[ch]); }
    static __device__ __forceinline__ uint64_t fold_columns(const uint64_t* A, const uint32_t* K) {
        uint32_t t1, t2, t3, t4, m0, m1, cm;
        asm("v_add_co_u32 %[m0], vcc, %[a1l], %[a2l]\n\t"
            "v_addc_co_u32 %[m1], vcc, %[a1h], %[a2h], vcc\n\t"
            "v_addc_co_u32 %[cm], vcc, 0, 0, vcc\n\t"
            "v_add_co_u32 %[t1], vcc, %[a0h], %[m0]\n\t"
            "v_addc_co_u32 %[t2], vcc, %[m1], %[a3l], vcc\n\t"
            "v_addc_co_u32 %[t3], vcc, %[cm], %[a3h], vcc\n\t"
            "v_addc_co_u32 %[t4], vcc, 0, %[k3], vcc\n\t"
            "v_add_co_u32 %[t2], vcc, %[t2], %[k0]\n\t"
            "v_addc_co_u32 %[t3], vcc, %[t3], %[k1], vcc\n\t"
            "v_addc_co_u32 %[t4], vcc, 0, %[t4], vcc\n\t"
            "v_add_co_u32 %[t3], vcc, %[t3], %[k2]\n\t"
            "v_addc_co_u32 %[t4], vcc, 0, %[t4], vcc"
            : [t1] "=&v"(t1), [t2] "=&v"(t2), [t3] "=&v"(t3), [t4] "=&v"(t4), [m0] "=&v"(m0), [m1] "=&v"(m1), [cm] "=&v"(cm)
            : [a0h] "v"((uint32_t)(A[0] >> 32)), [a1l] "v"((uint32_t)A[1]), [a1h] "v"((uint32_t)(A[1] >> 32)), [a2l] "v"((uint32_t)A[2]),
              [a2h] "v"((uint32_t)(A[2] >> 32)), [a3l] "v"((uint32_t)A[3]), [a3h] "v"((uint32_t)(A[3] >> 32)), [k0] "v"(K[0]),
              [k1] "v"(K[1]), [k2] "v"(K[2]), [k3] "v"(K[3])
            : "vcc");
        const uint64_t r = gl::canon(gl32::to_u64(gl32::reduce128((uint32_t)A[0], t1, t2, t3)));
        return gl::sub(r, (uint64_t)t4 << 32);
    }
};

struct DotAcc {
    uint64_t a[4];
    uint32_t kc[4];
    __device__ __forceinline__ void reset() {
#pragma unroll
        for (int i = 0; i < 4; i++) { a[i] = 0; kc[i] = 0; }
    }
    __device__ __forceinline__ void mac(uint64_t x, uint64_t c) {
        const uint32_t x0 = (uint32_t)x, x1 = (uint32_t)(x >> 32);
        asm("v_mad_u64_u32 %[a0], vcc, %[x0], %[c0], %[a0]\n\t"
            "v_addc_co_u32 %[k0], vcc, 0, %[k0], vcc\n\t"
            "v_mad_u64_u32 %[a1], vcc, %[x0], %[c1], %[a1]\n\t"
            "v_addc_co_u32 %[k1], vcc, 0, %[k1], vcc\n\t"
            "v_mad_u64_u32 %[a2], vcc, %[x1], %[c0], %[a2]\n\t"
            "v_addc_co_u32 %[k2], vcc, 0, %[k2], vcc\n\t"
            "v_mad_u64_u32 %[a3], vcc, %[x1], %[c1], %[a3]\n\t"
            "v_addc_co_u32 %[k3], vcc, 0, %[k3], vcc"
            : [a0] "+v"(a[0]), [a1] "+v"(a[1]), [a2] "+v"(a[2]), [a3] "+v"(a[3]), [k0] "+v"(kc[0]), [k1] "+v"(kc[1]),
              [k2] "+v"(kc[2]), [k3] "+v"(kc[3])
            : [x0] "v"(x0), [x1] "v"(x1), [c0] "s"((uint32_t)c), [c1] "s"((uint32_t)(c >> 32))
            : "vcc");
    }
    __device__ __forceinline__ uint64_t value() const { return GateAcc::fold_columns(a, kc); }
};

struct Sum128 {
    uint64_t lo = 0, hi = 0;
    __device__ __forceinline__ void add(uint64_t x, uint32_t sh) {
        const uint64_t tl = x << sh, th = sh ? x >> (64 - sh) : 0;
        lo += tl;
        hi += th + (lo < tl ? 1u : 0u);
    }
    __device__ __forceinline__ uint64_t value() const { return gl::reduce128(lo, hi); }
};

__device__ __forceinline__ uint64_t limb4(uint64_t l) {
    const uint64_t u = gl::mul_loose(l, gl::sub(l, 3));
    return gl::mul_loose(u, gl::add_loose(u, 2));
}

__device__ __forceinline__ uint64_t sbox7c(uint64_t x) {
    uint64_t x2 = gl::mul_loose(x, x), x4 = gl::mul_loose(x2, x2), x3 = gl::mul_loose(x, x2);
    const uint64_t r = gl::mul_loose(x3, x4);
    __builtin_amdgcn_sched_barrier(0);
    return r;
}
__device__ __forceinline__ void mds_canon(uint64_t (&s)[12]) {
    constexpr uint32_t C[12] = {17, 15, 41, 16, 2, 28, 13, 13, 39, 18, 34, 20};
    uint64_t o[12];
#pragma unroll
    for (int r = 0; r < 12; r++) {
        uint64_t al = 0, ah = 0;
#pragma unroll
        for (int i = 0; i < 12; i++) {
            al += (uint64_t)(uint32_t)s[(i + r) % 12] * C[i];
            ah += (uint64_t)(uint32_t)(s[(i + r) % 12] >> 32) * C[i];
        }
        if (r == 0) {
            al += (uint64_t)(uint32_t)s[0] * 8u;
            ah += (uint64_t)(uint32_t)(s[0] >> 32) * 8u;
        }
        o[r] = gl::canon(gl32::to_u64(gl32::fold_acc(al, ah)));
        __builtin_amdgcn_sched_barrier(0);
    }
#pragma unroll
    for (int i = 0; i < 12; i++) s[i] = o[i];
}

template <class WireFn, class Acc>
struct GateBlockSboxes {
    Acc& acc;
    WireFn W;
    uint32_t r0;
    __device__ __forceinline__ gl32::F at(uint32_t r, gl32::F computed) const {
        const uint64_t in = W(65 + r);
        acc.emit_at(41 + r, gl::sub(gl32::to_u64(computed), in));
        const gl32::F u = gl32::sbox7(gl32::from_u64(in));
        __builtin_amdgcn_sched_barrier(0);
        return u;
    }
    __device__ __forceinline__ gl32::F first(gl32::F s0) const { return at(r0, s0); }
    __device__ __forceinline__ gl32::F inner(int i, gl32::F w) const { return at(r0 + (uint32_t)i, w); }
    __device__ __forceinline__ void before_matrix_pass() const { acc.stash(); }
};

template <class WireFn, class Acc>
__device__ __forceinline__ void gate_poseidon_mx(WireFn W, Acc& acc, uint32_t parts) {
    const uint64_t* RC = poseidon::RC_DEV;
    const uint64_t* rcb = poseidon::LAYER_RCB_DEV;
    uint32_t lane = threadIdx.x & 63;
    asm("" : "+v"(lane) : "s"(parts));
    const gl32::i32x4_t afrag = gl32::mds_a_fragment(lane);
    gl32::F t[12];
    auto sbox_of_wires = [&](uint32_t w0) {
#pragma unroll
        for (int i = 0; i < 12; i++) {
            t[i] = gl32::sbox7(gl32::from_u64(W(w0 + i)));
            __builtin_amdgcn_sched_barrier(0);
        }
    };
    auto check_against_wires = [&](uint32_t c0, uint32_t w0) {
#pragma unroll
        for (int i = 0; i < 12; i++) {
            acc.emit_at(c0 + i, gl::sub(gl32::to_u64(t[i]), W(w0 + i)));
            __builtin_amdgcn_sched_barrier(0);
        }
    };
    if (parts & 1u) {
        const uint64_t swap = W(24);
        acc.emit_at(0, gl::mul(swap, gl::sub(swap, 1)));
        uint64_t st[12];
#pragma unroll
        for (int i = 0; i < 4; i++) {
            const uint64_t lhs = W(i), rhs = W(i + 4), delta = W(25 + i);
            acc.emit_at(1 + i, gl::sub(gl::mul(swap, gl::sub(rhs, lhs)), delta));
            st[i] = gl::add(lhs, delta);
            st[i + 4] = gl::sub(rhs, delta);
        }
#pragma unroll
        for (int i = 8; i < 12; i++) st[i] = W(i);
#pragma unroll
        for (int i = 0; i < 12; i++) {
            t[i] = gl32::sbox7(gl32::from_u64(gl::add_loose(st[i], RC[i])));
            __builtin_amdgcn_sched_barrier(0);
        }
#pragma unroll 1
        for (int r = 0; r < 3; r++) {
            if (r) sbox_of_wires(29 + 12 * (r - 1));
            gl32::mds_layer_mfma<2>(t, afrag, rcb + (r + 1) * 24);
            check_against_wires(5 + 12 * r, 29 + 12 * r);
        }
    }
    if (parts & 2u) {
        const gl32::BlockOperands op = poseidon::block_operands(lane);
        sbox_of_wires(29 + 24);
        gl32::mds_layer_mfma<2>(t, afrag, rcb + 4 * 24);
#pragma unroll 1
        for (uint32_t b = 0; b < NLX_POSEIDON_N_BLOCKS; b++)
            gl32::partial_block3<NLX_POSEIDON_BLOCK_GAMMA21>(t, op, poseidon::BLOCK_KAPPA_DEV + b * 6, GateBlockSboxes<WireFn, Acc>{acc, W, 3 * b});
        t[0] = GateBlockSboxes<WireFn, Acc>{acc, W, 21}.first(t[0]);
        gl32::mds_layer_mfma<2>(t, afrag, rcb + 26 * 24);
        check_against_wires(63, 87);
    }
    if (parts & 4u) {
#pragma unroll 1
        for (int r = 0; r < 4; r++) {
            sbox_of_wires(87 + 12 * r);
            if (r < 3) {
                gl32::mds_layer_mfma<2>(t, afrag, rcb + (27 + r) * 24);
                check_against_wires(63 + 12 * (r + 1), 87 + 12 * (r + 1));
            } else {
                gl32::mds_layer_mfma<0>(t, afrag, rcb);
                check_against_wires(111, 12);
            }
        }
    }
}

template <class WireFn, class Acc>
__device__ __forceinline__ void gate_poseidon_fast(WireFn W, Acc& acc, uint32_t parts) {
    const uint64_t* RC = poseidon::RC_DEV;
    uint64_t st[12];
    if (parts & 1u) {
        const uint64_t swap = W(24);
        acc.emit_at(0, gl::mul(swap, gl::sub(swap, 1)));
#pragma unroll
        for (int i = 0; i < 4; i++) {
            const uint64_t lhs = W(i), rhs = W(i + 4), delta = W(25 + i);
            acc.emit_at(1 + i, gl::sub(gl::mul(swap, gl::sub(rhs, lhs)), delta));
            st[i] = gl::add(lhs, delta);
            st[i + 4] = gl::sub(rhs, delta);
        }
#pragma unroll
        for (int i = 8; i < 12; i++) st[i] = W(i);
#pragma unroll
        for (int i = 0; i < 12; i++) st[i] = gl::add_loose(st[i], RC[i]);
#pragma unroll 1
        for (int r = 0; r < 3; r++) {
#pragma unroll
            for (int i = 0; i < 12; i++) st[i] = sbox7c(st[i]);
            mds_canon(st);
            __builtin_amdgcn_sched_barrier(0);
#pragma unroll
            for (int i = 0; i < 12; i++) {
                const uint64_t in = W(29 + 12 * r + i);
                acc.emit_at(5 + 12 * r + i, gl::sub(gl::add(st[i], RC[(r + 1) * 12 + i]), in));
                st[i] = in;
                __builtin_amdgcn_sched_barrier(0);
            }
        }
    }
    if (parts & 2u) {
#pragma unroll
        for (int i = 0; i < 12; i++) st[i] = sbox7c(W(29 + 24 + i));
        mds_canon(st);
#pragma unroll
        for (int i = 0; i < 12; i++) st[i] = gl::add(st[i], FAST_FIRST[i]);
        {
            uint64_t res[12];
            res[0] = st[0];
#pragma unroll
            for (int c = 1; c < 12; c++) {
                DotAcc dot;
                dot.reset();
#pragma unroll
                for (int r = 1; r < 12; r++) dot.mac(st[r], FAST_INIT[r - 1][c - 1]);
                res[c] = dot.value();
                __builtin_amdgcn_sched_barrier(0);
            }
#pragma unroll
            for (int i = 0; i < 12; i++) st[i] = res[i];
        }
#pragma unroll 1
        for (int r = 0; r < 22; r++) {
            const uint64_t in = W(65 + r);
            acc.emit_at(41 + r, gl::sub(st[0], in));
            uint64_t s0 = sbox7c(in);
            if (r < 21) s0 = gl::add_loose(s0, FAST_RC[r]);
            DotAcc dot;
            dot.reset();
            dot.mac(s0, 25);
#pragma unroll
            for (int i = 1; i < 12; i++) {
                dot.mac(st[i], FAST_W[r][i - 1]);
                st[i] = gl::add(st[i], gl::mul(s0, FAST_VS[r][i - 1]));
                __builtin_amdgcn_sched_barrier(0);
            }
            st[0] = dot.value();
        }
#pragma unroll
        for (int i = 0; i < 12; i++)
            acc.emit_at(63 + i, gl::sub(gl::add(st[i], RC[26 * 12 + i]), W(87 + i)));
    }
    if (parts & 4u) {
#pragma unroll 1
        for (int r = 0; r < 4; r++) {
            if (r != 0) {
#pragma unroll
                for (int i = 0; i < 12; i++) {
                    acc.emit_at(63 + 12 * r + i, gl::sub(gl::add(st[i], RC[(26 + r) * 12 + i]), W(87 + 12 * r + i)));
                    __builtin_amdgcn_sched_barrier(0);
                }
            }
#pragma unroll
            for (int i = 0; i < 12; i++) st[i] = sbox7c(W(87 + 12 * r + i));
            mds_canon(st);
            __builtin_amdgcn_sched_barrier(0);
        }
#pragma unroll
        for (int i = 0; i < 12; i++) acc.emit_at(111 + i, gl::sub(st[i], W(12 + i)));
    }
}

#ifndef NLX_PGATE_MX
#define NLX_PGATE_MX 0u
#endif
template <class WireFn, class Acc>
__device__ __forceinline__ void gate_poseidon(WireFn W, Acc& acc, uint32_t parts) {
    if (parts & NLX_PGATE_MX) gate_poseidon_mx(W, acc, parts & NLX_PGATE_MX);
    if (parts & ~NLX_PGATE_MX) gate_poseidon_fast(W, acc, parts & ~NLX_PGATE_MX);
}

template <class WireFn, class ConstFn, class Acc>
__device__ __forceinline__ void eval_gate(const GateDev& gd, const QuotientParams& p, WireFn W, ConstFn CC, Acc& acc, size_t n,
                                          uint32_t parts) {
    switch (gd.kind) {
        case NLX_GATE_CONSTANT:
            for (uint32_t i = 0; i < gd.param0; i++) acc.emit(gl::sub(CC(p.gate_const0 + i), W(i)));
            break;
        case NLX_GATE_PUBLIC_INPUT:
            for (uint32_t i = 0; i < 4; i++) acc.emit(gl::sub(W(i), p.pih[i]));
            break;
        case NLX_GATE_ARITHMETIC: {
            const uint64_t c0 = CC(p.gate_const0), c1 = CC(p.gate_const0 + 1);
            for (uint32_t i = 0; i < gd.param0; i++) {
                const uint64_t m0 = W(4 * i), m1 = W(4 * i + 1), ad = W(4 * i + 2), o = W(4 * i + 3);
                acc.emit(gl::sub(o, gl::add(gl::mul(gl::mul(m0, m1), c0), gl::mul(ad, c1))));
            }
            break;
        }
        case NLX_GATE_BASE_SUM: {
            const uint32_t B = gd.param0, nl = gd.param1;
            uint64_t sum = 0;
            for (uint32_t i = nl; i-- > 0;) sum = gl::add(gl::mul(sum, (uint64_t)B), W(1 + i));
            acc.emit(gl::sub(sum, W(0)));
            for (uint32_t i = 0; i < nl; i++) {
                const uint64_t limb = W(1 + i);
                uint64_t prod = 1;
                for (uint32_t t = 0; t < B; t++) prod = gl::mul(prod, gl::sub(limb, (uint64_t)t));
                acc.emit(prod);
            }
            break;
        }
        case NLX_GATE_POSEIDON:
            gate_poseidon(W, acc, parts);
            break;
        case NLX_GATE_ARITHMETIC_EXT: {
            const uint64_t c0 = CC(p.gate_const0), c1 = CC(p.gate_const0 + 1);
            for (uint32_t i = 0; i < gd.param0; i++) {
                const gl::Ext m0{W(8 * i), W(8 * i + 1)}, m1{W(8 * i + 2), W(8 * i + 3)};
                const gl::Ext pr = gl::mul(m0, m1);
                acc.emit(gl::sub(W(8 * i + 6), gl::add(gl::mul(pr.a, c0), gl::mul(W(8 * i + 4), c1))));
                acc.emit(gl::sub(W(8 * i + 7), gl::add(gl::mul(pr.b, c0), gl::mul(W(8 * i + 5), c1))));
            }
            break;
        }
        case NLX_GATE_MUL_EXT: {
            const uint64_t c0 = CC(p.gate_const0);
            for (uint32_t i = 0; i < gd.param0; i++) {
                const gl::Ext m0{W(6 * i), W(6 * i + 1)}, m1{W(6 * i + 2), W(6 * i + 3)};
                const gl::Ext pr = gl::mul(m0, m1);
                acc.emit(gl::sub(W(6 * i + 4), gl::mul(pr.a, c0)));
                acc.emit(gl::sub(W(6 * i + 5), gl::mul(pr.b, c0)));
            }
            break;
        }
        case NLX_GATE_REDUCING:
        case NLX_GATE_REDUCING_EXT: {
            const uint32_t nco = gd.param0;
            const bool ext = gd.kind == NLX_GATE_REDUCING_EXT;
            const uint32_t start_coeffs = 6, start_accs = start_coeffs + (ext ? 2 * nco : nco);
            const gl::Ext alpha{W(2), W(3)};
            gl::Ext a{W(4), W(5)};
            for (uint32_t i = 0; i < nco; i++) {
                const uint32_t aw = (i == nco - 1) ? 0 : start_accs + 2 * i;
                const gl::Ext nxt{W(aw), W(aw + 1)};
                const gl::Ext pr = gl::mul(a, alpha);
                if (ext) {
                    acc.emit(gl::sub(gl::add(pr.a, W(start_coeffs + 2 * i)), nxt.a));
                    acc.emit(gl::sub(gl::add(pr.b, W(start_coeffs + 2 * i + 1)), nxt.b));
                } else {
                    acc.emit(gl::sub(gl::add(pr.a, W(start_coeffs + i)), nxt.a));
                    acc.emit(gl::sub(pr.b, nxt.b));
                }
                a = nxt;
            }
            break;
        }
        case NLX_GATE_POSEIDON_MDS: {
#pragma unroll 1
            for (uint32_t comp = 0; comp < 2; comp++) {
                uint64_t st[12];
#pragma unroll
                for (int i = 0; i < 12; i++) st[i] = W(2 * i + comp);
                mds_canon(st);
                __builtin_amdgcn_sched_barrier(0);
#pragma unroll
                for (int rr = 0; rr < 12; rr++) {
                    acc.emit_at(2 * rr + comp, gl::sub(W(24 + 2 * rr + comp), st[rr]));
                    __builtin_amdgcn_sched_barrier(0);
                }
            }
            acc.k += 24;
            break;
        }
        case NLX_GATE_EXPONENTIATION: {
            const uint32_t nb = gd.param0;
            const uint64_t base = W(0);
            uint64_t prev_iv = 1;
            for (uint32_t i = 0; i < nb; i++) {
                const uint64_t prev = i ? gl::mul(prev_iv, prev_iv) : 1;
                const uint64_t bit = W(1 + (nb - 1 - i));
                const uint64_t sel = gl::add(gl::mul(bit, base), gl::sub(1, bit));
                const uint64_t iv = W(2 + nb + i);
                acc.emit(gl::sub(gl::mul(prev, sel), iv));
                prev_iv = iv;
            }
            acc.emit(gl::sub(W(1 + nb), prev_iv));
            break;
        }
        case NLX_GATE_U32_ADD_MANY: {
            const uint32_t na = gd.param0, nops = gd.param1, nl = 18, nrl = 16;
            for (uint32_t i = 0; i < nops; i++) {
                const uint32_t b0 = (na + 3) * i, lb = (na + 3) * nops + nl * i;
                uint64_t computed = W(b0 + na);
                for (uint32_t j = 0; j < na; j++) computed = gl::add(computed, W(b0 + j));
                const uint64_t res = W(b0 + na + 1), cy = W(b0 + na + 2);
                acc.emit(gl::sub(gl::add(gl::mul(cy, 1ULL << 32), res), computed));
                Sum128 cr, cc;
                for (uint32_t j = nl; j-- > 0;) {
                    const uint64_t l = W(lb + j);
                    acc.emit(limb4(l));
                    if (j < nrl) cr.add(l, 2 * j);
                    else cc.add(l, 2 * (j - nrl));
                }
                acc.emit(gl::sub(cr.value(), res));
                acc.emit(gl::sub(cc.value(), cy));
            }
            break;
        }
        case NLX_GATE_U32_ARITHMETIC: {
            const uint32_t nops = gd.param0;
            for (uint32_t i = 0; i < nops; i++) {
                const uint32_t b0 = 6 * i, lb = 6 * nops + 32 * i;
                const uint64_t computed = gl::add(gl::mul(W(b0), W(b0 + 1)), W(b0 + 2));
                const uint64_t lo = W(b0 + 3), hi = W(b0 + 4), inv = W(b0 + 5);
                const uint64_t hi_not_max = gl::sub(gl::mul(inv, gl::sub(0xFFFFFFFFULL, hi)), 1);
                acc.emit(gl::mul(hi_not_max, lo));
                acc.emit(gl::sub(gl::add(gl::mul(hi, 1ULL << 32), lo), computed));
                Sum128 cl, ch;
                for (uint32_t j = 32; j-- > 0;) {
                    const uint64_t l = W(lb + j);
                    acc.emit(limb4(l));
                    if (j < 16) cl.add(l, 2 * j);
                    else ch.add(l, 2 * (j - 16));
                }
                acc.emit(gl::sub(cl.value(), lo));
                acc.emit(gl::sub(ch.value(), hi));
            }
            break;
        }
        case NLX_GATE_U32_SUBTRACTION: {
            const uint32_t nops = gd.param0;
            for (uint32_t i = 0; i < nops; i++) {
                const uint32_t b0 = 5 * i, lb = 5 * nops + 16 * i;
                const uint64_t initial = gl::sub(gl::sub(W(b0), W(b0 + 1)), W(b0 + 2));
                const uint64_t res = W(b0 + 3), bo = W(b0 + 4);
                acc.emit(gl::sub(res, gl::add(initial, gl::mul(bo, 1ULL << 32))));
                Sum128 c;
                for (uint32_t j = 16; j-- > 0;) {
                    const uint64_t l = W(lb + j);
                    acc.emit(limb4(l));
                    c.add(l, 2 * j);
                }
                acc.emit(gl::sub(c.value(), res));
                acc.emit(gl::mul(bo, gl::sub(1, bo)));
            }
            break;
        }
        case NLX_GATE_U32_RANGE_CHECK: {
            const uint32_t nin = gd.param0;
            for (uint32_t i = 0; i < nin; i++) {
                const uint32_t ab = nin + 16 * i;
                Sum128 sum;
                for (uint32_t j = 0; j < 16; j++) sum.add(W(ab + j), 2 * j);
                acc.emit(gl::sub(sum.value(), W(i)));
                for (uint32_t j = 0; j < 16; j++) acc.emit(limb4(W(ab + j)));
            }
            break;
        }
        case NLX_GATE_COMPARISON: {
            const uint32_t nbits = gd.param0, nch = gd.param1, cb = (nbits + nch - 1) / nch;
            const uint32_t fc = 4, sc = 4 + nch, eqd = 4 + 2 * nch, ceq = 4 + 3 * nch, iv = 4 + 4 * nch, msb = 4 + 5 * nch;
            Sum128 fcomb, scomb;
            for (uint32_t i = 0; i < nch; i++) {
                fcomb.add(W(fc + i), cb * i);
                scomb.add(W(sc + i), cb * i);
            }
            acc.emit(gl::sub(fcomb.value(), W(0)));
            acc.emit(gl::sub(scomb.value(), W(1)));
            uint64_t msd = 0;
            for (uint32_t i = 0; i < nch; i++) {
                const uint64_t f = W(fc + i), s2 = W(sc + i);
                uint64_t p1, p2;
                if (cb == 2) {
                    p1 = limb4(f);
                    p2 = limb4(s2);
                } else {
                    p1 = f;
                    p2 = s2;
                    for (uint32_t x2 = 1; x2 < (1u << cb); x2++) {
                        p1 = gl::mul(p1, gl::sub(f, (uint64_t)x2));
                        p2 = gl::mul(p2, gl::sub(s2, (uint64_t)x2));
                    }
                }
                acc.emit(p1);
                acc.emit(p2);
                const uint64_t diff = gl::sub(s2, f), e = W(ceq + i), ivv = W(iv + i);
                acc.emit(gl::sub(gl::mul(diff, W(eqd + i)), gl::sub(1, e)));
                acc.emit(gl::mul(e, diff));
                acc.emit(gl::sub(ivv, gl::mul(e, msd)));
                msd = gl::add(ivv, gl::mul(gl::sub(1, e), diff));
            }
            acc.emit(gl::sub(W(3), msd));
            uint64_t bc = 0;
            for (uint32_t b = 0; b <= cb; b++) {
                const uint64_t bit = W(msb + b);
                acc.emit(gl::mul(bit, gl::sub(1, bit)));
            }
            for (uint32_t b = cb + 1; b-- > 0;) bc = gl::add(gl::add(bc, bc), W(msb + b));
            acc.emit(gl::sub(gl::add(1ULL << cb, W(3)), bc));
            acc.emit(gl::sub(W(2), W(msb + cb)));
            break;
        }
        case NLX_GATE_COSET_INTERPOLATION: {
            const uint32_t bits = gd.param0, deg = gd.param1, np = 1u << bits;
            const uint32_t sep = 1 + 2 * np, sev = sep + 2, si = sev + 2, ni = (np - 2) / (deg - 1), ssh = si + 4 * ni;
            const uint64_t shift = W(0);
            const gl::Ext pt{W(ssh), W(ssh + 1)};
            acc.emit(gl::sub(W(sep), gl::mul(pt.a, shift)));
            acc.emit(gl::sub(W(sep + 1), gl::mul(pt.b, shift)));
            uint64_t np_inv = 1;
            for (uint32_t i = 0; i < bits; i++) np_inv = gl::mul(np_inv, 0x7FFFFFFF80000001ULL);
            const uint32_t stride = (uint32_t)(n >> bits), half = (uint32_t)(n >> 1);
            gl::Ext ev{0, 0}, pr{1, 0};
            for (uint32_t c = 0; c <= ni; c++) {
                const uint32_t start = c == 0 ? 0 : 1 + (deg - 1) * c;
                uint32_t end = c == 0 ? deg : start + deg - 1;
                end = end > np ? np : end;
                for (uint32_t j = start; j < end; j++) {
                    const uint64_t xj = root_pow(p.w_n_table, j * stride, half);
                    const gl::Ext term{gl::sub(pt.a, xj), pt.b};
                    const gl::Ext vp = gl::mul(gl::Ext{W(1 + 2 * j), W(2 + 2 * j)}, pr);
                    ev = gl::add(gl::mul(ev, term), gl::mul(vp, gl::mul(xj, np_inv)));
                    pr = gl::mul(pr, term);
                }
                if (c < ni) {
                    const gl::Ext ie{W(si + 2 * c), W(si + 2 * c + 1)}, ip{W(si + 2 * (ni + c)), W(si + 2 * (ni + c) + 1)};
                    acc.emit(gl::sub(ie.a, ev.a));
                    acc.emit(gl::sub(ie.b, ev.b));
                    acc.emit(gl::sub(ip.a, pr.a));
                    acc.emit(gl::sub(ip.b, pr.b));
                    ev = ie;
                    pr = ip;
                }
            }
            acc.emit(gl::sub(W(sev), ev.a));
            acc.emit(gl::sub(W(sev + 1), ev.b));
            break;
        }
        case NLX_GATE_RANDOM_ACCESS: {
            const uint32_t bits = gd.param0, copies = gd.param1 & 0xFFFF, extra = gd.param1 >> 16;
            const uint32_t vec = 1u << bits, rt = (2 + vec) * copies + extra;
            for (uint32_t cpy = 0; cpy < copies; cpy++) {
                const uint32_t b0 = (2 + vec) * cpy, bw = rt + cpy * bits;
                for (uint32_t i = 0; i < bits; i++) {
                    const uint64_t b = W(bw + i);
                    acc.emit(gl::mul(b, gl::sub(b, 1)));
                }
                uint64_t rec = 0;
                for (uint32_t i = bits; i-- > 0;) rec = gl::add(gl::add(rec, rec), W(bw + i));
                acc.emit(gl::sub(rec, W(b0)));
                uint64_t stack[7];
                uint32_t depth_of[7];
                int sp = 0;
                for (uint32_t leaf = 0; leaf < vec; leaf++) {
                    uint64_t v = W(b0 + 2 + leaf);
                    uint32_t lvl = 0;
                    while (sp > 0 && depth_of[sp - 1] == lvl) {
                        const uint64_t left = stack[--sp];
                        const uint64_t b = W(bw + lvl);
                        v = gl::add(left, gl::mul(b, gl::sub(v, left)));
                        lvl++;
                    }
                    stack[sp] = v;
                    depth_of[sp] = lvl;
                    sp++;
                }
                acc.emit(gl::sub(stack[0], W(b0 + 1)));
            }
            for (uint32_t i = 0; i < extra; i++) acc.emit(gl::sub(CC(p.gate_const0 + i), W((2 + vec) * copies + i)));
            break;
        }
        default: break;
    }
}

#ifndef NLX_QW
#define NLX_QW 8
#endif
#ifndef NLX_QMINW
#define NLX_QMINW 4
#endif
constexpr int QW = NLX_QW;

__global__ __launch_bounds__(64 * QW, NLX_QMINW) void k_quotient(QuotientParams p) {
    extern __shared__ uint64_t q_lds[];
    const uint32_t lane = threadIdx.x & 63, wv = __builtin_amdgcn_readfirstlane(threadIdx.x >> 6);
    const unsigned log_L = p.log_n + p.rate_bits;
    const size_t n = (size_t)1 << p.log_n, L = (size_t)1 << log_L;
    struct Point { size_t pos; uint32_t r, k; bool live; };
    auto point_of = [&](uint32_t ln) {
        const size_t pos_raw = (size_t)blockIdx.x * 64 + ln;
        Point q;
        q.live = pos_raw < L;
        q.pos = q.live ? pos_raw : L - 1;
        q.r = (uint32_t)(q.pos >> p.log_n);
        q.k = (uint32_t)(q.pos & (n - 1));
        return q;
    };
    auto opaque = [](uint32_t v, uint32_t where) {
        asm("" : "+v"(v) : "s"(where));
        return v;
    };
    const size_t pos = point_of(lane).pos;
    uint64_t* lw = q_lds;
    uint64_t* lc = q_lds + (size_t)p.num_wires * 64;
    for (uint32_t c = wv; c < p.num_wires; c += QW) lw[c * 64 + lane] = p.wires[(size_t)c * L + pos];
    for (uint32_t c = wv; c < p.n_consts_all; c += QW) lc[c * 64 + lane] = p.cs[(size_t)c * L + pos];
    __syncthreads();
    auto W = [&](uint32_t c) { return lw[c * 64 + lane]; };
    auto CC = [&](uint32_t c) { return lc[c * 64 + lane]; };

    const uint32_t nc = p.nc, npp = p.npp;
    const uint32_t T0 = nc + nc * (npp + 1) + nc * p.n_lk_terms;
    const uint64_t* ap0 = p.alpha_pows;
    const uint64_t* ap1 = p.alpha_pows + p.alpha_stride;
    uint64_t tot0 = 0, tot1 = 0;
    uint64_t l0a = 0, l0b = 0;
    GateAcc acc;
    acc.ap0 = ap0 + T0;
    acc.ap1 = ap1 + T0;
    const uint32_t* work = p.work + (size_t)wv * p.work_stride;
    for (uint32_t wi = 0;; wi++) {
        const uint32_t word = __builtin_amdgcn_readfirstlane(work[wi]);
        if (word == 0xFFFFFFFFu) break;
        const uint32_t item = word & 0xFFFFu, parts = (word >> 16) ? (word >> 16) : 7u;
        if (item < p.n_gates) {
            const GateDev gd = p.gates[item];
            const uint64_t s = CC(gd.selector_index);
            uint64_t f = 1;
            for (uint32_t i = gd.group_start; i < gd.group_end; i++)
                if (i != gd.index) f = gl::mul(f, gl::sub((uint64_t)i, s));
            if (p.n_selectors > 1) f = gl::mul(f, gl::sub(0xFFFFFFFFULL, s));
            acc.reset();
            eval_gate(gd, p, W, CC, acc, n, parts);
            tot0 = gl::add(tot0, gl::mul(f, acc.finish(0)));
            tot1 = gl::add(tot1, gl::mul(f, acc.finish(1)));
        } else {
            const uint32_t c = item - p.n_gates;
            const uint32_t n_chunks = (p.routed + p.chunk - 1) / p.chunk;
            const Point pt = point_of(opaque(lane, wi));
            const size_t pos = pt.pos;
            auto ZS = [&](uint32_t col) { return p.zs[(size_t)col * L + pos]; };
            const size_t pos_next = ((size_t)pt.r << p.log_n) + ((pt.k + 1) & (n - 1));
            const uint64_t x = gl::mul(p.coset_base[pt.r], root_pow(p.w_n_table, pt.k, (uint32_t)(n >> 1)));
            const uint64_t beta = p.betas[c], gamma = p.gammas[c];
            const uint64_t bx = gl::mul(beta, x);
            const uint64_t z_x = ZS(c);
            const uint64_t z_gx = p.zs[(size_t)c * L + pos_next];
            const uint64_t zm1 = gl::sub(z_x, 1);
            l0a = gl::add(l0a, gl::mul(zm1, ap0[c]));
            l0b = gl::add(l0b, gl::mul(zm1, ap1[c]));
            uint64_t accv = z_x;
#pragma unroll 1
            for (uint32_t q = 0; q < n_chunks; q++) {
                uint64_t nm = 1, dn = 1;
                for (uint32_t j = q * p.chunk; j < (q + 1) * p.chunk && j < p.routed; j++) {
                    const uint64_t wg = gl::add(W(j), gamma);
                    const uint64_t sg = p.cs[(size_t)(p.n_consts_all + j) * L + pos];
                    nm = gl::mul_loose(nm, gl::add_loose(gl::mul_loose(bx, p.k_is[j]), wg));
                    dn = gl::mul_loose(dn, gl::add_loose(gl::mul_loose(beta, sg), wg));
                }
                const uint64_t new_acc = (q + 1 < n_chunks) ? ZS(nc + c * npp + q) : z_gx;
                const uint64_t term = gl::sub(gl::mul(accv, nm), gl::mul(new_acc, dn));
                const uint32_t t = nc + c * (npp + 1) + q;
                tot0 = gl::add(tot0, gl::mul(term, ap0[t]));
                tot1 = gl::add(tot1, gl::mul(term, ap1[t]));
                accv = new_acc;
            }
        }
    }
    __syncthreads();
    uint64_t* red = q_lds;
    red[(wv * 4 + 0) * 64 + lane] = tot0;
    red[(wv * 4 + 1) * 64 + lane] = tot1;
    red[(wv * 4 + 2) * 64 + lane] = l0a;
    red[(wv * 4 + 3) * 64 + lane] = l0b;
    __syncthreads();
    if (wv != 0) return;
    for (uint32_t w2 = 1; w2 < QW; w2++) {
        tot0 = gl::add(tot0, red[(w2 * 4 + 0) * 64 + lane]);
        tot1 = gl::add(tot1, red[(w2 * 4 + 1) * 64 + lane]);
        l0a = gl::add(l0a, red[(w2 * 4 + 2) * 64 + lane]);
        l0b = gl::add(l0b, red[(w2 * 4 + 3) * 64 + lane]);
    }
    const Point pe = point_of(opaque(lane, 0xFFFFFFFFu));
    const uint64_t zh_inv = p.zh_inv[pe.r];
    const uint64_t l0s = p.l0_scaled[pe.pos];
    if (!pe.live) return;
    if (p.accumulate) {
        tot0 = gl::add(tot0, p.out[pe.pos]);
        if (nc > 1) tot1 = gl::add(tot1, p.out[L + pe.pos]);
    }
    p.out[pe.pos] = gl::add(gl::mul(tot0, zh_inv), gl::mul(l0a, l0s));
    if (nc > 1) p.out[L + pe.pos] = gl::add(gl::mul(tot1, zh_inv), gl::mul(l0b, l0s));
}

size_t quotient_lds_bytes(uint32_t num_wires, uint32_t n_consts_all) {
    const size_t tile = (size_t)(num_wires + n_consts_all) * 64 * 8, red = (size_t)QW * 4 * 64 * 8;
    return tile > red ? tile : red;
}
uint32_t quotient_waves() { return QW; }

void launch_quotient(hipStream_t st, const QuotientParams& p) {
    const size_t L = (size_t)1 << (p.log_n + p.rate_bits);
    const size_t lds = quotient_lds_bytes(p.num_wires, p.n_consts_all);
    (void)hipFuncSetAttribute((const void*)k_quotient, hipFuncAttributeMaxDynamicSharedMemorySize, (int)lds);
    hipLaunchKernelGGL(k_quotient, dim3((unsigned)((L + 63) / 64)), dim3(64 * QW), lds, st, p);
}

__global__ __launch_bounds__(256, 3) void k_quotient_poseidon(QuotientParams p, uint32_t gate, uint32_t add) {
    const unsigned log_L = p.log_n + p.rate_bits;
    const size_t L = (size_t)1 << log_L;
    const size_t pos_raw = (size_t)blockIdx.x * blockDim.x + threadIdx.x;
    const bool live = pos_raw < L;
    const size_t pos = live ? pos_raw : L - 1;
    auto W = [&](uint32_t c) { return p.wires[(size_t)c * L + pos]; };
    const GateDev gd = p.gates[gate];
    const uint64_t s = p.cs[(size_t)gd.selector_index * L + pos];
    uint64_t f = 1;
    for (uint32_t i = gd.group_start; i < gd.group_end; i++)
        if (i != gd.index) f = gl::mul(f, gl::sub((uint64_t)i, s));
    if (p.n_selectors > 1) f = gl::mul(f, gl::sub(0xFFFFFFFFULL, s));
    const uint32_t T0 = p.nc + p.nc * (p.npp + 1) + p.nc * p.n_lk_terms;
    GateAcc acc;
    acc.ap0 = p.alpha_pows + T0;
    acc.ap1 = p.alpha_pows + p.alpha_stride + T0;
    acc.reset();
    gate_poseidon_mx(W, acc, 2u);
    uint64_t t0 = gl::mul(f, acc.finish(0)), t1 = gl::mul(f, acc.finish(1));
    if (!live) return;
    if (add) {
        t0 = gl::add(t0, p.out[pos]);
        if (p.nc > 1) t1 = gl::add(t1, p.out[L + pos]);
    }
    p.out[pos] = t0;
    if (p.nc > 1) p.out[L + pos] = t1;
}
void launch_quotient_poseidon(hipStream_t st, const QuotientParams& p, uint32_t gate, bool add) {
    const size_t L = (size_t)1 << (p.log_n + p.rate_bits);
    hipLaunchKernelGGL(k_quotient_poseidon, dim3((unsigned)((L + 255) / 256)), dim3(256), 0, st, p, gate, add ? 1u : 0u);
}

__global__ __launch_bounds__(256) void k_l0_table(uint64_t* __restrict__ out, unsigned log_n, unsigned rate_bits,
                                                  const uint64_t* __restrict__ coset_base,
                                                  const uint64_t* __restrict__ w_n_table) {
    const size_t pos = (size_t)blockIdx.x * blockDim.x + threadIdx.x;
    if (pos >> (log_n + rate_bits)) return;
    const size_t n = (size_t)1 << log_n;
    const uint32_t r = (uint32_t)(pos >> log_n), k = (uint32_t)(pos & (n - 1));
    const uint64_t x = gl::mul(coset_base[r], root_pow(w_n_table, k, (uint32_t)(n >> 1)));
    out[pos] = gl::inv(gl::mul((uint64_t)(n % gl::P), gl::sub(x, 1)));
}
void launch_l0_table(hipStream_t st, uint64_t* d_out, unsigned log_n, unsigned rate_bits, const uint64_t* d_coset_base,
                     const uint64_t* d_w_n_table) {
    const size_t L = (size_t)1 << (log_n + rate_bits);
    hipLaunchKernelGGL(k_l0_table, dim3((unsigned)((L + 255) / 256)), dim3(256), 0, st, d_out, log_n, rate_bits,
                       d_coset_base, d_w_n_table);
}

__global__ __launch_bounds__(256) void k_quotient_chunks(const uint64_t* __restrict__ in, uint64_t* __restrict__ out,
                                                         unsigned log_n, unsigned rate_bits,
                                                         const uint64_t* __restrict__ w_R_inv_pows,
                                                         const uint64_t* __restrict__ chunk_scale) {
    const size_t j = (size_t)blockIdx.x * blockDim.x + threadIdx.x;
    const size_t n = (size_t)1 << log_n;
    if (j >= n) return;
    const uint32_t R = 1u << rate_bits;
    const uint64_t* src = in + ((size_t)blockIdx.y << (log_n + rate_bits));
    uint64_t* dst = out + ((size_t)blockIdx.y << (log_n + rate_bits));
    uint64_t a[8];
    for (uint32_t r = 0; r < R; r++) a[r] = src[(size_t)r * n + j];
    for (uint32_t c = 0; c < R; c++) {
        uint64_t s = 0;
        for (uint32_t r = 0; r < R; r++) s = gl::add(s, gl::mul(a[r], w_R_inv_pows[(c * r) & (R - 1)]));
        dst[(size_t)c * n + j] = gl::mul(s, chunk_scale[c]);
    }
}
void launch_quotient_chunks(hipStream_t st, const uint64_t* d_in, uint64_t* d_out, unsigned log_n, unsigned rate_bits,
                            uint32_t nc, const uint64_t* d_w_R_inv_pows, const uint64_t* d_chunk_scale) {
// ... 261 lines not shown
#pragma unroll
        for (int i = 0; i < 8; i++)
            if ((uint32_t)i == p.pos) s[i] = cand;
        poseidon::permute(s);
        const uint64_t resp = s[7];
        const unsigned lz = resp ? (unsigned)__clzll((long long)resp) : 64u;
        if (valid && lz >= p.bits) atomicMin(best, (unsigned long long)cand);
    }
}
void launch_pow_grind(hipStream_t st, const PowParams& p, unsigned long long* d_best) {
    (void)hipMemsetAsync(d_best, 0xFF, 8, st);
    hipLaunchKernelGGL(k_pow_grind, dim3(POW_GRID), dim3(POW_BLOCK), 0, st, p, d_best);
}

__global__ void k_fri_gather_leaf(const uint64_t* __restrict__ values, unsigned log_n, unsigned rate_bits,
                                  unsigned arity_bits, const uint64_t* __restrict__ leaf_idx, uint64_t* __restrict__ out,
                                  size_t out_stride_words) {
    const uint32_t q = blockIdx.x;
    const uint32_t m = threadIdx.x;
    const uint32_t arity = 1u << arity_bits;
    if (m >= arity) return;
    const unsigned log_np = log_n - arity_bits;
    const size_t np = (size_t)1 << log_np, n = (size_t)1 << log_n;
    const uint64_t leaf = leaf_idx[q];
    const uint32_t r = gl::bitrev32((uint32_t)(leaf >> log_np), rate_bits);
    const uint32_t kp = gl::bitrev32((uint32_t)(leaf & (np - 1)), log_np);
    const uint32_t mm = gl::bitrev32(m, arity_bits);
    const size_t pos = (size_t)r * n + kp + (size_t)mm * np;
    uint64_t* o = out + (size_t)q * out_stride_words + 2 * m;
    o[0] = values[2 * pos];
    o[1] = values[2 * pos + 1];
}
void launch_fri_gather_leaf(hipStream_t st, const uint64_t* d_values, unsigned log_n, unsigned rate_bits,
                            unsigned arity_bits, const uint64_t* d_leaf_idx, uint32_t n_q, uint64_t* d_out,
                            size_t out_stride_words) {
    hipLaunchKernelGGL(k_fri_gather_leaf, dim3(n_q), dim3(64), 0, st, d_values, log_n, rate_bits, arity_bits,
                       d_leaf_idx, d_out, out_stride_words);
}

__global__ void k_shift_indices(const uint64_t* __restrict__ in, uint64_t* __restrict__ out, uint32_t n, unsigned shift) {
    const uint32_t q = blockIdx.x * blockDim.x + threadIdx.x;
    if (q < n) out[q] = in[q] >> shift;
}
void launch_shift_indices(hipStream_t st, const uint64_t* d_in, uint64_t* d_out, uint32_t n, unsigned shift) {
    hipLaunchKernelGGL(k_shift_indices, dim3((n + 63) / 64), dim3(64), 0, st, d_in, d_out, n, shift);
}

__global__ void k_pow_table(uint64_t* __restrict__ out, uint64_t a0, uint64_t a1, uint32_t count, uint32_t stride) {
    const uint32_t t = blockIdx.x * blockDim.x + threadIdx.x;
    if (t >= count) return;
    out[t] = gl::pow(a0, t);
    out[stride + t] = gl::pow(a1, t);
}
void launch_pow_table(hipStream_t st, uint64_t* d_out, uint64_t a0, uint64_t a1, uint32_t count, uint32_t stride) {
    hipLaunchKernelGGL(k_pow_table, dim3((count + 63) / 64), dim3(64), 0, st, d_out, a0, a1, count, stride);
}
__global__ void k_ext_pow_table(uint64_t* __restrict__ out, uint64_t a, uint64_t b, uint32_t count) {
    const uint32_t t = blockIdx.x * blockDim.x + threadIdx.x;
    if (t >= count) return;
    const gl::Ext v = gl::pow(gl::Ext{a, b}, t);
    out[2 * t] = v.a;
    out[2 * t + 1] = v.b;
}
void launch_ext_pow_table(hipStream_t st, uint64_t* d_out, const uint64_t alpha[2], uint32_t count) {
    hipLaunchKernelGGL(k_ext_pow_table, dim3((count + 63) / 64), dim3(64), 0, st, d_out, alpha[0], alpha[1], count);
}

struct CheckAcc {
    uint32_t k, first;
    uint64_t value;
    __device__ __forceinline__ void reset() { k = 0; first = 0xFFFFFFFFu; value = 0; }
    __device__ __forceinline__ void stash() {}
    __device__ __forceinline__ void emit_at(uint32_t idx, uint64_t c) {
        const uint64_t v = gl::canon(c);
        if (v != 0 && idx < first) { first = idx; value = v; }
    }
    __device__ __forceinline__ void emit(uint64_t c) { emit_at(k++, c); }
};

__global__ void k_check_reset(CheckBlock* __restrict__ b) {
    b->gate_rows_bad = b->copy_cells_bad = b->lookup_slots_bad = 0;
    b->gate_first = b->copy_first = b->lookup_first = b->sigma_undecodable = CHECK_NONE;
    b->gate_value = 0;
    b->gate_index = b->gate_constraint = 0;
}
void launch_check_reset(hipStream_t st, CheckBlock* d_block) { hipLaunchKernelGGL(k_check_reset, dim3(1), dim3(1), 0, st, d_block); }

__device__ __forceinline__ void check_report(bool bad, unsigned long long key, unsigned long long* count, unsigned long long* first) {
    const unsigned long long m = __ballot(bad);
    if (m == 0) return;
    if ((threadIdx.x & 63) == (uint32_t)__ffsll((long long)m) - 1) atomicAdd(count, (unsigned long long)__popcll(m));
    if (bad) atomicMin(first, key);
}

__global__ __launch_bounds__(256) void k_check_gates(CheckGatesParams p, uint32_t row0, uint32_t report_row) {
    const size_t n = (size_t)1 << p.q.log_n;
    const size_t raw = (size_t)row0 + (size_t)blockIdx.x * blockDim.x + threadIdx.x;
    const bool live = raw < n;
    const size_t row = live ? raw : n - 1;
    auto W = [&](uint32_t c) { return p.wires[(size_t)c * n + row]; };
    auto CC = [&](uint32_t c) { return p.consts[(size_t)c * n + row]; };
    uint32_t first = 0xFFFFFFFFu, gate = 0;
    uint64_t value = 0;
    for (uint32_t g = 0; g < p.q.n_gates; g++) {
        const GateDev gd = p.q.gates[g];
        const bool mine = live && CC(gd.selector_index) == (uint64_t)gd.index;
// ... 92 lines not shown
```

### near-light-client_amd/csrc/stark.hip

```cpp
#include <algorithm>
#include <vector>
#include "commit.hpp"
#include "fri.hpp"
#include "gl.hpp"
#include "poly.hpp"
#include "prover.hpp"
#include "transcript.hpp"
#include "air_vm.hpp"
#include "stark.hpp"

using namespace nlx;

namespace nlx {

__global__ __launch_bounds__(256) void k_air_quotient(AirParams p) {
    extern __shared__ uint64_t regs[];
    const size_t pos = (size_t)blockIdx.x * blockDim.x + threadIdx.x;
    const unsigned log_Q = p.log_n + p.qdb;
    if (pos >> log_Q) return;
    const size_t n = (size_t)1 << p.log_n;
    const uint32_t rq = (uint32_t)(pos >> p.log_n), k = (uint32_t)(pos & (n - 1));
    const uint32_t r = rq << (p.rate_bits - p.qdb);
    const size_t row = ((size_t)r << p.log_n) + k, row_next = ((size_t)r << p.log_n) + ((k + 1) & (n - 1));
    const size_t qrow_next = ((size_t)rq << p.log_n) + ((k + 1) & (n - 1));
// ... 507 lines not shown
    uint32_t col0[4] = {0, 0, 0, 0};
    Challenger ch;
    ch.observe(s->air_digest, 4);
    ch.observe(public_inputs, d.num_public_inputs);
    std::vector<uint64_t> cap(capw);
    std::vector<uint64_t>& values = sc.values;
    values.assign(public_inputs, public_inputs + d.num_public_inputs);
    std::vector<uint64_t> round_vals;
    std::vector<const uint64_t*>& h_cols = sc.h_cols;
    h_cols.resize(ncols);

    s->clock.begin(st);
    s->clock.stage("commit_trace");
    for (uint32_t r = 0; r < NRD; r++) {
        const uint32_t rcols = s->round_cols[r];
        const uint32_t n_rv = s->round_values[r];
        uint64_t rv[64];
        const uint64_t* tr_ptr = round_fn(user, r, values.data() + d.num_public_inputs, (uint32_t)(values.size() - d.num_public_inputs),
                                          n_rv ? rv : nullptr);
        if (!tr_ptr) return ctx->fail(NLX_E_INVAL, "round %u: the round callback returned NULL", r);
        for (uint32_t k = 0; k < n_rv; k++) rv[k] %= gl::P;
        Staged tr(ctx, tr_ptr, (size_t)rcols * n * 8, true, false);
        NLX_RC(tr.status);
        NLX_RC(commit_build(ctx, tr.as<uint64_t>(), n, CommitInput::ValuesNatural, rcols, log_n, d.rate_bits, cap_h, cr[r], d.leaf_group_cols,
                           d.batch_cols));
        for (uint32_t k = 0; k < cr[r]->n_trees; k++) {
            NLX_RC(fetch(ctx, cap.data(), cr[r]->cap + (size_t)k * cr[r]->tree_words, capw * 8));
            w.u64s(cap.data(), capw);
            ch.observe(cap.data(), capw);
        }
        if (n_rv) {
            ch.observe(rv, n_rv);
            values.insert(values.end(), rv, rv + n_rv);
            round_vals.insert(round_vals.end(), rv, rv + n_rv);
        }
        for (uint32_t k = 0; k < s->round_challenges[r]; k++) values.push_back(ch.challenge());
        for (uint32_t c = 0; c < rcols; c++) h_cols[col0[r] + c] = cr[r]->lde + (size_t)c * L;
        col0[r + 1] = col0[r] + rcols;
    }
    uint64_t alphas[2] = {0, 0};
    for (uint32_t i = 0; i < nc; i++) alphas[i] = ch.challenge();

    s->clock.stage("quotient_eval");
    const size_t Q = n << qdb;
    const uint32_t n_seg = (uint32_t)s->seg_after.size();
    const size_t n_values = values.size();
    for (uint32_t sg = 0; sg < n_seg; sg++)
        for (uint32_t i = 0; i < 2; i++) values.push_back(gl::pow(alphas[i], s->seg_after[sg]));
    uint64_t* d_pis = scratch.alloc_as<uint64_t>(values.size() * 8);
    const uint64_t** d_cols = scratch.alloc_as<const uint64_t*>((size_t)ncols * 8);
    uint64_t* d_qvals = scratch.alloc_as<uint64_t>((size_t)nc * Q * 8);
    uint64_t* d_qchunks = scratch.alloc_as<uint64_t>((size_t)nc * Q * 8);
    uint64_t* d_part = n_seg > 1 ? scratch.alloc_as<uint64_t>((size_t)n_seg * nc * Q * 8) : nullptr;
    if (!d_pis || !d_cols || !d_qvals || !d_qchunks || (n_seg > 1 && !d_part)) return NLX_E_NOMEM;
    NLX_HIP(ctx, hipMemcpyAsync(d_pis, values.data(), values.size() * 8, hipMemcpyHostToDevice, st));
    NLX_HIP(ctx, hipMemcpyAsync(d_cols, h_cols.data(), (size_t)ncols * 8, hipMemcpyHostToDevice, st));
    {
        AirParams ap{};
        ap.cols = d_cols; ap.program = s->d_program; ap.pis = d_pis;
        ap.coset_base = s->d_q_coset_base; ap.zh_inv = s->d_q_zh_inv; ap.l_inv = s->d_l_inv;
        ap.periodic = s->d_periodic; ap.period_bits = d.period_bits;
        ap.w_n_table = ctx->tables.fwd[log_n];
        ap.out = d_qvals;
        ap.alphas[0] = alphas[0]; ap.alphas[1] = alphas[1];
        ap.g_inv = gl::inv(gl::root_of_unity(log_n));
        ap.log_n = log_n; ap.rate_bits = d.rate_bits; ap.qdb = qdb; ap.n_words = d.n_words; ap.nc = nc;
        ap.n_regs = s->n_regs; ap.n_pis = d.num_public_inputs;
        ap.seg = s->d_seg; ap.seg_mul = d_pis + n_values; ap.part = d_part; ap.n_seg = n_seg;
        unsigned bs = 64;
        while (bs > n) bs >>= 1;
        ctx->begin_kernel("air_quotient", 8.0 * Q * (2.0 * ncols + nc));
        if (s->gen) s->gen->launch(st, (unsigned)(Q / AIRGEN_BLOCK), n_seg, ap);
        for (size_t gi = 0; !s->gen && gi < s->seg_group.size(); gi++) {
            const uint32_t first = s->seg_group[gi], last = gi + 1 < s->seg_group.size() ? s->seg_group[gi + 1] : n_seg;
            AirParams gp = ap;
            gp.seg = ap.seg + 2 * first;
            gp.seg_mul = ap.seg_mul + 2 * first;
            gp.part = n_seg > 1 ? ap.part + (size_t)first * nc * Q : nullptr;
            const size_t lds = (size_t)bs * s->seg_regs[last - 1] * 8;
            hipLaunchKernelGGL(k_air_quotient, dim3((unsigned)(Q / bs), last - first), dim3(bs), lds, st, gp);
        }
        if (n_seg > 1)
            hipLaunchKernelGGL(k_air_combine, dim3((unsigned)((nc * Q + 255) / 256)), dim3(256), 0, st, d_part, s->d_q_zh_inv,
                               d_qvals, n_seg, nc, log_n, log_n + qdb);
        ctx->end_kernel();
    }
    s->clock.stage("quotient_intt");
    launch_intt_dif_cosets(st, ctx->tables, d_qvals, nc, log_n, qdb, s->d_q_inv_scale_br);
    launch_quotient_chunks(st, d_qvals, d_qchunks, log_n, qdb, nc, s->d_q_wR_inv, s->d_q_chunk_scale);
    s->clock.stage("commit_quotient");
    NLX_RC(commit_build(ctx, d_qchunks, n, CommitInput::CoeffsBitrev, nq, log_n, d.rate_bits, cap_h, cq, d.leaf_group_cols));
    NLX_RC(fetch(ctx, cap.data(), cq->cap, capw * 8));
    w.u64s(cap.data(), capw);
    ch.observe(cap.data(), capw);

    s->clock.stage("openings");
    uint64_t zeta[2], gzeta[2];
    ch.ext_challenge(zeta);
    {
        const uint64_t g = gl::root_of_unity(log_n);
        gzeta[0] = gl::mul(zeta[0], g);
        gzeta[1] = gl::mul(zeta[1], g);
    }
    const uint32_t n_open = ncols + nq;
    uint32_t widest = nq;
    for (uint32_t r = 0; r < NRD; r++) widest = s->round_cols[r] > widest ? s->round_cols[r] : widest;
    const OpeningPoints& pts = sc.points;
    NLX_RC(sc.points.upload(scratch, zeta, gzeta, log_n));
    const size_t open_words = (size_t)(n_open + ncols) * 2;
    const size_t og = d.openings_group, og_runs = og ? (open_words + og - 1) / og : 0;
    uint64_t* d_open = scratch.alloc_as<uint64_t>((og ? og_runs * og + 4 * og_runs : open_words) * 8);
    uint64_t* d_eval_scratch = scratch.alloc_as<uint64_t>(eval_scratch_words(widest, log_n) * 8);
    if (!d_open || !d_eval_scratch) return NLX_E_NOMEM;
    {
        for (uint32_t r = 0; r < NRD; r++) {
            launch_eval_br(st, cr[r]->coeffs_br, n, s->round_cols[r], log_n, pts.zeta(), d_open + 2 * (size_t)col0[r],
                           d_eval_scratch, pts.zeta_pows());
// ... 96 lines not shown
```

Measured before the change: 23.24.

## Replace Horner constraint folding with wide lazy-reduced alpha-power MAC accumulators

Generated AIR segments now fold each constraint with precomputed alpha powers, accumulated in 32x32 MAD columns with carry counters and reduced once at the end, instead of a fully reduced Horner multiply-add per constraint. Many field multiplies and adds across the quotient and gate kernels switch to loose (non-canonical) variants, with canonicalisation only where values are reused. A per-proof alpha power table is built on the device, and an ext_ops test entry point is added. The aim is to cut modular reduction work in the constraint-heavy quotient kernels, at the cost of more registers, extra table loads and a risk of correctness bugs in the lazy arithmetic.

```diff
diff --git a/include/nlx.h b/include/nlx.h
--- a/include/nlx.h
+++ b/include/nlx.h
@@ -43,6 +43,7 @@
 int32_t nlx_ctx_kernel_units(nlx_ctx* ctx, const char* name, double* units);
 
 int32_t nlx_field_ops(nlx_ctx* ctx, const uint64_t* a, const uint64_t* b, size_t n, uint64_t* out);
+int32_t nlx_ext_ops(nlx_ctx* ctx, const uint64_t* a, const uint64_t* b, size_t n, uint64_t* out);
 
 int32_t nlx_poseidon_permute_batch(nlx_ctx* ctx, uint64_t* states, size_t n);
 
diff --git a/near-light-client_amd/__init__.py b/near-light-client_amd/__init__.py
--- a/near-light-client_amd/__init__.py
+++ b/near-light-client_amd/__init__.py
@@ -1,6 +1,6 @@
 from . import _lib as lib
 from ._lib import Context, DeviceBuffer, NlxError, GOLDILOCKS_P
-from .batch import PolynomialBatch, MerkleTree, poseidon_permute, hash_rows, poseidon_bn128_permute, poseidon_bn128_hash_rows, ntt, field_ops, bn254_ntt, bn254_pack, bn254_unpack, BN254_R, bn254_msm_g1, bn254_g1_pack, bn254_g1_unpack, bn254_g1_sum, bn254_g1_multiples, bn254_g2_pack, bn254_g2_unpack, bn254_msm_g2, bn254_g2_sum, BN254_Q, bn254_plonk_quotient, bn254_kzg_open
+from .batch import PolynomialBatch, MerkleTree, poseidon_permute, hash_rows, poseidon_bn128_permute, poseidon_bn128_hash_rows, ntt, field_ops, ext_ops, bn254_ntt, bn254_pack, bn254_unpack, BN254_R, bn254_msm_g1, bn254_g1_pack, bn254_g1_unpack, bn254_g1_sum, bn254_g1_multiples, bn254_g2_pack, bn254_g2_unpack, bn254_msm_g2, bn254_g2_sum, BN254_Q, bn254_plonk_quotient, bn254_kzg_open
 from .plonk import CircuitConfig, CircuitData, SyntheticCircuit, WitnessReport, pow_grind, batch_prove, ProveJob
 from .stark import Air, Stark, StarkConfig, StarkProver, TraceReport, fibonacci_air, fibonacci_trace, wide_air, wide_trace
 from . import sha256_air, sha512_air, logup, fp25519, ed25519_air, nearx_io, near_protocol, stark, plonk, succinct_io, split_ntt, bn254_plonk, bn254_groth16
diff --git a/near-light-client_amd/_lib.py b/near-light-client_amd/_lib.py
--- a/near-light-client_amd/_lib.py
+++ b/near-light-client_amd/_lib.py
@@ -55,6 +55,7 @@
                                               ctypes.POINTER(ctypes.c_double), ctypes.POINTER(ctypes.c_double)]),
     "nlx_ctx_kernel_units": (ctypes.c_int32, [ctypes.c_void_p, ctypes.c_char_p, ctypes.POINTER(ctypes.c_double)]),
     "nlx_field_ops": (ctypes.c_int32, [ctypes.c_void_p, ctypes.c_void_p, ctypes.c_void_p, ctypes.c_size_t, ctypes.c_void_p]),
+    "nlx_ext_ops": (ctypes.c_int32, [ctypes.c_void_p, ctypes.c_void_p, ctypes.c_void_p, ctypes.c_size_t, ctypes.c_void_p]),
     "nlx_poseidon_permute_batch": (ctypes.c_int32, [ctypes.c_void_p, ctypes.c_void_p, ctypes.c_size_t]),
     "nlx_hash_rows": (ctypes.c_int32, [ctypes.c_void_p, ctypes.c_void_p, ctypes.c_size_t, ctypes.c_size_t,
                                        ctypes.c_void_p]),
diff --git a/near-light-client_amd/airgen.py b/near-light-client_amd/airgen.py
--- a/near-light-client_amd/airgen.py
+++ b/near-light-client_amd/airgen.py
@@ -43,16 +43,49 @@
     return segs
 
 
-def _emit_constraint(lines, expr):
-    lines.append("    c = %s;" % expr)
-    lines.append("    acc0 = gl::add(gl::mul(acc0, g.a0), c); acc1 = gl::add(gl::mul(acc1, g.a1), c);")
+HORNER = "acc0 = gl::add_loose(gl::mul_loose(acc0, g.a0), %s); acc1 = gl::add_loose(gl::mul_loose(acc1, g.a1), %s);"
+HORNER_SEGMENTS = {
+    "ed25519_2p7_tagged": (2646, 6297, 6956, 7679, 8370, 9093, 14490, 15181, 15872),
+    "sha512_tagged": (8982, 10259, 11536, 12813, 14090, 15367, 16644, 17921, 19198, 20475, 21752, 23029, 24306, 25583, 26144, 26705,
+                      27266),
+}
+
+
+def segment_exponents(words, lo, hi):
+    n, i = 0, lo
+    while i < hi:
+        w = int(words[i])
+        op = w & 0xFF
+        if op in (EMIT_TRANSITION, EMIT_FIRST, EMIT_LAST, EMIT):
+            n += 1
+        elif op == EMIT_LOGUP:
+            n += 2
+        elif op == EMIT_BOOL:
+            n += ((w >> 40) & 0xFFFF) or 1
+        i += 2 if op == CONST else 1
+    return [n - 1 - k for k in range(n)]
+
+
+class _Fold:
+
+    def __init__(self, exponents, wide):
+        self.exponents, self.wide, self.k = exponents, wide, 0
+
+    def emit(self, lines, expr, indent="    ", canonical=False):
+        if self.wide:
+            e = self.exponents[self.k]
+            lines.append("%sacc.mac(%s, AP0(%d), AP1(%d));" % (indent, expr if canonical else expr.replace("gl::mul(", "gl::mul_loose(", 1), e, e))
+        else:
+            lines.append("%sc = %s; " % (indent, expr) + HORNER % ("c", "c"))
+        self.k += 1
 
 
 SCHED_EVERY = 4
 
 
-def _segment_body(words, lo, hi):
+def _segment_body(words, lo, hi, wide=False):
     L, i, since = [], lo, 0
+    fold = _Fold(segment_exponents(words, lo, hi), wide)
     R = lambda k: "r%d" % k
     while i < hi:
         if since >= SCHED_EVERY:
@@ -107,7 +140,7 @@
                 for k in range(m):
                     L.append("      v[%d] = COL(%d, g.row);" % (k, a + i0 + k))
                 for k in range(m):
-                    L.append("      c = gl::mul(v[%d], gl::sub(v[%d], 1)); acc0 = gl::add(gl::mul(acc0, g.a0), c); acc1 = gl::add(gl::mul(acc1, g.a1), c);" % (k, k))
+                    fold.emit(L, "gl::mul(v[%d], gl::sub(v[%d], 1))" % (k, k), indent="      ")
                 L.append("    }")
         elif op == EMIT_LOGUP:
             L.append("    { const uint64_t al0 = PIS(g.n_pis + %d), al1 = PIS(g.n_pis + %d);" % (sh, sh + 1))
@@ -126,20 +159,22 @@
                 L.append("      const uint64_t hu = gl::mul(h1, u1);")
                 L.append("      c0 = gl::sub(gl::add(gl::mul(h0, u0), gl::sub(mul_pow2(hu, 3), hu)), s2);")
                 L.append("      c1 = gl::sub(gl::add(gl::mul(h0, u1), gl::mul(h1, u0)), gl::add(al1, al1));")
-            L.append("      acc0 = gl::add(gl::mul(gl::add(gl::mul(acc0, g.a0), c0), g.a0), c1);")
-            L.append("      acc1 = gl::add(gl::mul(gl::add(gl::mul(acc1, g.a1), c0), g.a1), c1); }")
+            fold.emit(L, "c0", indent="      ", canonical=True)
+            fold.emit(L, "c1", indent="      ", canonical=True)
+            L.append("    }")
         elif op == LOADV:
             L.append("    __builtin_amdgcn_sched_barrier(0);")
         elif op == EMIT_TRANSITION:
-            _emit_constraint(L, "gl::mul(%s, g.z_last)" % R(a))
+            fold.emit(L, "gl::mul(%s, g.z_last)" % R(a))
         elif op == EMIT_FIRST:
-            _emit_constraint(L, "gl::mul(%s, g.l_first)" % R(a))
+            fold.emit(L, "gl::mul(%s, g.l_first)" % R(a))
         elif op == EMIT_LAST:
-            _emit_constraint(L, "gl::mul(%s, g.l_last)" % R(a))
+            fold.emit(L, "gl::mul(%s, g.l_last)" % R(a))
         elif op == EMIT:
-            _emit_constraint(L, R(a))
+            fold.emit(L, R(a), canonical=True)
         else:
             raise ValueError("unknown opcode %d at word %d" % (op, i - 1))
+    assert fold.k == len(fold.exponents)
     return L
 
 
@@ -187,7 +222,9 @@
                "typedef const char __attribute__((address_space(1)))* airgen_gptr;",
                "#define COL(c, off) (*(const uint64_t __attribute__((address_space(1)))*)((airgen_gptr)((airgen_kptr)g.cols)[c] + (off)))",
                "#define PIS(i) (((airgen_kptr)g.pis)[i])",
-               "struct G {", "    uint64_t cols, pis; const uint64_t* per;",
+               "#define AP0(j) (((airgen_kptr)g.ap0)[j])",
+               "#define AP1(j) (((airgen_kptr)g.ap1)[j])",
+               "struct G {", "    uint64_t cols, pis, ap0, ap1; const uint64_t* per;",
                "    size_t per_stride, per_off; uint64_t a0, a1, z_last, l_first, l_last; uint32_t row, row_next, n_pis;", "};",
                "struct Acc { uint64_t a0, a1; };",
                "template <typename T> __device__ __forceinline__ T* uni(T* p) {",
@@ -203,11 +240,20 @@
             out.append("    G g = gv;")
             out.append("    g.cols = uni(gv.cols); g.pis = uni(gv.pis); g.per = uni(gv.per); g.per_stride = uni((uint64_t)gv.per_stride);")
             out.append("    g.a0 = uni(gv.a0); g.a1 = uni(gv.a1); g.n_pis = (uint32_t)__builtin_amdgcn_readfirstlane((int)gv.n_pis);")
-            out.append("    uint64_t c, acc0 = 0, acc1 = 0;")
+            wide = lo not in HORNER_SEGMENTS.get(name, ())
+            if wide:
+                out.append("    g.ap0 = uni(gv.ap0); g.ap1 = uni(gv.ap1);")
+                out.append("    GateAcc acc;")
+                out.append("    acc.reset();")
+            else:
+                out.append("    uint64_t c, acc0 = 0, acc1 = 0;")
             if regs:
                 out.append("    uint64_t %s;" % ", ".join("r%d" % r for r in regs))
-            out += _segment_body(words, lo, hi)
-            out.append("    return Acc{acc0, acc1};")
+            out += _segment_body(words, lo, hi, wide)
+            if wide:
+                out.append("    return Acc{GateAcc::fold_columns(acc.a, acc.kc), GateAcc::fold_columns(acc.a + 4, acc.kc + 4)};")
+            else:
+                out.append("    return Acc{acc0, acc1};")
             out.append("}")
             out.append("")
         out += [
@@ -231,6 +277,7 @@
             "    g.per_stride = (size_t)1 << (p.qdb + p.period_bits);",
             "    g.per_off = ((size_t)rq << p.period_bits) + (k & ((1u << p.period_bits) - 1));",
             "    g.a0 = p.alphas[0]; g.a1 = p.alphas[1];",
+            "    g.ap0 = (uint64_t)p.alpha_pows; g.ap1 = (uint64_t)(p.alpha_pows + p.alpha_stride);",
             "    g.z_last = gl::sub(x, p.g_inv); g.l_first = gl::mul(zh, p.l_inv[pos]); g.l_last = gl::mul(zh, p.l_inv[qrow_next]);",
             "    Acc acc{0, 0};",
             "    switch (first) {",
diff --git a/near-light-client_amd/batch.py b/near-light-client_amd/batch.py
--- a/near-light-client_amd/batch.py
+++ b/near-light-client_amd/batch.py
@@ -18,6 +18,16 @@
     b = np.ascontiguousarray(b, dtype=np.uint64)
     out = np.zeros((5, a.size), dtype=np.uint64)
     ctx.check(dll.nlx_field_ops(ctx.handle, ptr(a), ptr(b), a.size, ptr(out)))
+    return out
+
+
+def ext_ops(ctx, a, b):
+    a = np.ascontiguousarray(a, dtype=np.uint64)
+    b = np.ascontiguousarray(b, dtype=np.uint64)
+    if a.ndim != 2 or a.shape[1] != 2 or a.shape != b.shape:
+        raise ValueError("a and b must both have shape (n, 2)")
+    out = np.zeros((8, a.shape[0]), dtype=np.uint64)
+    ctx.check(dll.nlx_ext_ops(ctx.handle, ptr(a), ptr(b), a.shape[0], ptr(out)))
     return out
 
 
diff --git a/near-light-client_amd/build.py b/near-light-client_amd/build.py
--- a/near-light-client_amd/build.py
+++ b/near-light-client_amd/build.py
@@ -51,7 +51,7 @@
     return m
 
 
-AIRGEN_HEADERS = ("air_vm.hpp", "gl.hpp", "nlx.h", "nlx_field.h")
+AIRGEN_HEADERS = ("air_vm.hpp", "gate_acc.hpp", "gl.hpp", "nlx.h", "nlx_field.h")
 
 
 def _compile(src, verbose):
diff --git a/near-light-client_amd/csrc/air_vm.hpp b/near-light-client_amd/csrc/air_vm.hpp
--- a/near-light-client_amd/csrc/air_vm.hpp
+++ b/near-light-client_amd/csrc/air_vm.hpp
@@ -2,6 +2,7 @@
 #include <hip/hip_runtime.h>
 #include <cstdint>
 #include "gl.hpp"
+#include "gate_acc.hpp"
 #include "nlx.h"
 
 namespace nlx {
@@ -21,6 +22,8 @@
     uint64_t* part;
     uint32_t n_seg;
     uint64_t alphas[2];
+    const uint64_t* alpha_pows;
+    uint32_t alpha_stride;
     uint64_t g_inv;
     uint32_t log_n, rate_bits, qdb, n_words, nc, n_regs, period_bits, n_pis;
 };
diff --git a/near-light-client_amd/csrc/commit.hip b/near-light-client_amd/csrc/commit.hip
--- a/near-light-client_amd/csrc/commit.hip
+++ b/near-light-client_amd/csrc/commit.hip
@@ -177,6 +177,22 @@
     return NLX_OK;
 } NLX_CATCH(ctx)
 
+int32_t nlx_ext_ops(nlx_ctx* ctx, const uint64_t* a, const uint64_t* b, size_t n, uint64_t* out) NLX_TRY {
+    if (!ctx) return NLX_E_INVAL;
+    if (n == 0) return NLX_OK;
+    if (!a || !b || !out) return ctx->fail(NLX_E_INVAL, "NULL buffer");
+    (void)hipSetDevice(ctx->device);
+    Staged sa(ctx, a, 2 * n * 8, true, false), sb(ctx, b, 2 * n * 8, true, false), so(ctx, out, 8 * n * 8, false, true);
+    if (sa.status) return sa.status;
+    if (sb.status) return sb.status;
+    if (so.status) return so.status;
+    launch_ext_ops(ctx->stream, sa.as<uint64_t>(), sb.as<uint64_t>(), n, so.as<uint64_t>());
+    int32_t rc = so.finish();
+    if (rc) return rc;
+    NLX_HIP(ctx, hipStreamSynchronize(ctx->stream));
+    return NLX_OK;
+} NLX_CATCH(ctx)
+
 int32_t nlx_poseidon_permute_batch(nlx_ctx* ctx, uint64_t* states, size_t n) NLX_TRY {
     if (!ctx) return NLX_E_INVAL;
     if (n == 0) return NLX_OK;
diff --git a/near-light-client_amd/csrc/gate_acc.hpp b/near-light-client_amd/csrc/gate_acc.hpp
--- /dev/null
+++ b/near-light-client_amd/csrc/gate_acc.hpp
@@ -0,0 +1,78 @@
+#pragma once
+#include <hip/hip_runtime.h>
+#include <cstdint>
+#include "gl.hpp"
+
+namespace nlx {
+
+struct GateAcc {
+    const uint64_t* __restrict__ ap0;
+    const uint64_t* __restrict__ ap1;
+    uint64_t a[8];
+    uint32_t kc[8];
+    uint32_t k;
+    uint64_t base[2];
+    __device__ __forceinline__ void reset() {
+#pragma unroll
+        for (int i = 0; i < 8; i++) { a[i] = 0; kc[i] = 0; }
+        k = 0;
+        base[0] = base[1] = 0;
+    }
+    __device__ __forceinline__ void stash() {
+        base[0] = gl::add(base[0], fold_columns(a, kc));
+        base[1] = gl::add(base[1], fold_columns(a + 4, kc + 4));
+#pragma unroll
+        for (int i = 0; i < 8; i++) { a[i] = 0; kc[i] = 0; }
+    }
+    __device__ __forceinline__ void emit_at(uint32_t idx, uint64_t c) { mac(c, ap0[idx], ap1[idx]); }
+    __device__ __forceinline__ void mac(uint64_t c, uint64_t b0, uint64_t b1) {
+        const uint32_t c0 = (uint32_t)c, c1 = (uint32_t)(c >> 32);
+        asm("v_mad_u64_u32 %[a0], vcc, %[c0], %[p0], %[a0]\n\t"
+            "v_addc_co_u32 %[k0], vcc, 0, %[k0], vcc\n\t"
+            "v_mad_u64_u32 %[a1], vcc, %[c0], %[p1], %[a1]\n\t"
+            "v_addc_co_u32 %[k1], vcc, 0, %[k1], vcc\n\t"
+            "v_mad_u64_u32 %[a2], vcc, %[c1], %[p0], %[a2]\n\t"
+            "v_addc_co_u32 %[k2], vcc, 0, %[k2], vcc\n\t"
+            "v_mad_u64_u32 %[a3], vcc, %[c1], %[p1], %[a3]\n\t"
+            "v_addc_co_u32 %[k3], vcc, 0, %[k3], vcc\n\t"
+            "v_mad_u64_u32 %[a4], vcc, %[c0], %[q0], %[a4]\n\t"
+            "v_addc_co_u32 %[k4], vcc, 0, %[k4], vcc\n\t"
+            "v_mad_u64_u32 %[a5], vcc, %[c0], %[q1], %[a5]\n\t"
+            "v_addc_co_u32 %[k5], vcc, 0, %[k5], vcc\n\t"
+            "v_mad_u64_u32 %[a6], vcc, %[c1], %[q0], %[a6]\n\t"
+            "v_addc_co_u32 %[k6], vcc, 0, %[k6], vcc\n\t"
+            "v_mad_u64_u32 %[a7], vcc, %[c1], %[q1], %[a7]\n\t"
+            "v_addc_co_u32 %[k7], vcc, 0, %[k7], vcc"
+            : [a0] "+v"(a[0]), [a1] "+v"(a[1]), [a2] "+v"(a[2]), [a3] "+v"(a[3]), [a4] "+v"(a[4]), [a5] "+v"(a[5]),
+              [a6] "+v"(a[6]), [a7] "+v"(a[7]), [k0] "+v"(kc[0]), [k1] "+v"(kc[1]), [k2] "+v"(kc[2]), [k3] "+v"(kc[3]),
+              [k4] "+v"(kc[4]), [k5] "+v"(kc[5]), [k6] "+v"(kc[6]), [k7] "+v"(kc[7])
+            : [c0] "v"(c0), [c1] "v"(c1), [p0] "s"((uint32_t)b0), [p1] "s"((uint32_t)(b0 >> 32)), [q0] "s"((uint32_t)b1),
+              [q1] "s"((uint32_t)(b1 >> 32))
+            : "vcc");
+    }
+    __device__ __forceinline__ void emit(uint64_t c) { emit_at(k++, c); }
+    __device__ __forceinline__ uint64_t finish(int ch) const { return gl::add(fold_columns(a + 4 * ch, kc + 4 * ch), base[ch]); }
+    static __device__ __forceinline__ uint64_t fold_columns(const uint64_t* A, const uint32_t* K) {
+        uint32_t t1, t2, t3, t4, m0, m1, cm;
+        asm("v_add_co_u32 %[m0], vcc, %[a1l], %[a2l]\n\t"
+            "v_addc_co_u32 %[m1], vcc, %[a1h], %[a2h], vcc\n\t"
+            "v_addc_co_u32 %[cm], vcc, 0, 0, vcc\n\t"
+            "v_add_co_u32 %[t1], vcc, %[a0h], %[m0]\n\t"
+            "v_addc_co_u32 %[t2], vcc, %[m1], %[a3l], vcc\n\t"
+            "v_addc_co_u32 %[t3], vcc, %[cm], %[a3h], vcc\n\t"
+            "v_addc_co_u32 %[t4], vcc, 0, %[k3], vcc\n\t"
+            "v_add_co_u32 %[t2], vcc, %[t2], %[k0]\n\t"
+            "v_addc_co_u32 %[t3], vcc, %[t3], %[k1], vcc\n\t"
+            "v_addc_co_u32 %[t4], vcc, 0, %[t4], vcc\n\t"
+            "v_add_co_u32 %[t3], vcc, %[t3], %[k2]\n\t"
+            "v_addc_co_u32 %[t4], vcc, 0, %[t4], vcc"
+            : [t1] "=&v"(t1), [t2] "=&v"(t2), [t3] "=&v"(t3), [t4] "=&v"(t4), [m0] "=&v"(m0), [m1] "=&v"(m1), [cm] "=&v"(cm)
+            : [a0h] "v"((uint32_t)(A[0] >> 32)), [a1l] "v"((uint32_t)A[1]), [a1h] "v"((uint32_t)(A[1] >> 32)), [a2l] "v"((uint32_t)A[2]),
+              [a2h] "v"((uint32_t)(A[2] >> 32)), [a3l] "v"((uint32_t)A[3]), [a3h] "v"((uint32_t)(A[3] >> 32)), [k0] "v"(K[0]),
+              [k1] "v"(K[1]), [k2] "v"(K[2]), [k3] "v"(K[3])
+            : "vcc");
+        return gl::reduce160((uint32_t)A[0], t1, t2, t3, t4);
+    }
+};
+
+}
diff --git a/near-light-client_amd/csrc/gl.hpp b/near-light-client_amd/csrc/gl.hpp
--- a/near-light-client_amd/csrc/gl.hpp
+++ b/near-light-client_amd/csrc/gl.hpp
@@ -144,6 +144,50 @@
 }
 #endif
 
+#if defined(__HIP__)
+template <bool CANON>
+__device__ __forceinline__ uint64_t reduce160_impl(uint32_t w0, uint32_t w1, uint32_t w2, uint32_t w3, uint32_t w4) {
+    uint32_t r0, r1, t0;
+    asm("v_sub_co_u32 %[r0], vcc, %[w0], %[w3]\n\t"
+        "v_subbrev_co_u32 %[r1], vcc, 0, %[w1], vcc\n\t"
+        "v_cndmask_b32_e64 %[t0], 0, -1, vcc\n\t"
+        "v_sub_co_u32 %[r0], vcc, %[r0], %[t0]\n\t"
+        "v_subbrev_co_u32 %[r1], vcc, 0, %[r1], vcc"
+        : [r0] "=&v"(r0), [r1] "=&v"(r1), [t0] "=&v"(t0)
+        : [w0] "v"(w0), [w1] "v"(w1), [w3] "v"(w3)
+        : "vcc");
+    const uint64_t base = ((uint64_t)r1 << 32) | r0;
+    uint64_t r;
+    uint32_t tm;
+    asm("v_mad_u64_u32 %[r], vcc, %[w2], -1, %[base]\n\t"
+        "v_cndmask_b32_e64 %[t], 0, -1, vcc\n\t"
+        "v_mad_u64_u32 %[r], vcc, %[t], 1, %[r]"
+        : [r] "=&v"(r), [t] "=&v"(tm)
+        : [w2] "v"(w2), [base] "v"(base)
+        : "vcc");
+    return sub(CANON ? canon(r) : r, (uint64_t)w4 << 32);
+}
+__device__ __forceinline__ uint64_t reduce160(uint32_t w0, uint32_t w1, uint32_t w2, uint32_t w3, uint32_t w4) {
+    return reduce160_impl<true>(w0, w1, w2, w3, w4);
+}
+__device__ __forceinline__ uint64_t reduce160_loose(uint32_t w0, uint32_t w1, uint32_t w2, uint32_t w3, uint32_t w4) {
+    return reduce160_impl<false>(w0, w1, w2, w3, w4);
+}
+struct Wide128 {
+    uint32_t w0, w1;
+    uint64_t w32;
+};
+__device__ __forceinline__ Wide128 mul_wide(uint64_t a, uint64_t b) {
+    const uint32_t a0 = (uint32_t)a, a1 = (uint32_t)(a >> 32), b0 = (uint32_t)b, b1 = (uint32_t)(b >> 32);
+    const uint64_t p0 = (uint64_t)a0 * b0;
+    const uint64_t p1 = (uint64_t)a0 * b1 + (p0 >> 32);
+    const uint64_t p2 = (uint64_t)a1 * b0 + (uint32_t)p1;
+    uint64_t p3 = (uint64_t)a1 * b1 + (p1 >> 32), sink;
+    asm("v_mad_u64_u32 %0, %1, %2, 1, %3" : "=v"(p3), "=s"(sink) : "v"((uint32_t)(p2 >> 32)), "v"(p3));
+    return Wide128{(uint32_t)p0, (uint32_t)p2, p3};
+}
+#endif
+
 GL_HD uint64_t mul_loose(uint64_t a, uint64_t b) {
 #if defined(__HIP_DEVICE_COMPILE__)
     return mul_loose_asm(a, b);
@@ -186,7 +230,34 @@
 GL_HD Ext ext(uint64_t a, uint64_t b = 0) { return Ext{a, b}; }
 GL_HD Ext add(Ext x, Ext y) { return Ext{add(x.a, y.a), add(x.b, y.b)}; }
 GL_HD Ext sub(Ext x, Ext y) { return Ext{sub(x.a, y.a), sub(x.b, y.b)}; }
-GL_HD Ext mul(Ext x, Ext y) {
+#if defined(__HIP__)
+template <bool CANON>
+__device__ __forceinline__ Ext mul_impl(Ext x, Ext y) {
+    const Wide128 ab = mul_wide(x.a, y.b), ba = mul_wide(x.b, y.a);
+    uint32_t s0, s1, s2, s3, s4;
+    asm("v_add_co_u32 %[s0], vcc, %[x0], %[y0]\n\t"
+        "v_addc_co_u32 %[s1], vcc, %[x1], %[y1], vcc\n\t"
+        "v_addc_co_u32 %[s2], vcc, %[x2], %[y2], vcc\n\t"
+        "v_addc_co_u32 %[s3], vcc, %[x3], %[y3], vcc\n\t"
+        "v_addc_co_u32 %[s4], vcc, 0, 0, vcc"
+        : [s0] "=&v"(s0), [s1] "=&v"(s1), [s2] "=&v"(s2), [s3] "=&v"(s3), [s4] "=&v"(s4)
+        : [x0] "v"(ab.w0), [x1] "v"(ab.w1), [x2] "v"((uint32_t)ab.w32), [x3] "v"((uint32_t)(ab.w32 >> 32)), [y0] "v"(ba.w0),
+          [y1] "v"(ba.w1), [y2] "v"((uint32_t)ba.w32), [y3] "v"((uint32_t)(ba.w32 >> 32))
+        : "vcc");
+    const uint64_t c1 = reduce160_impl<CANON>(s0, s1, s2, s3, s4);
+    __builtin_amdgcn_sched_barrier(0);
+    const Wide128 aa = mul_wide(x.a, y.a), bb = mul_wide(x.b, y.b);
+    const uint64_t t0 = (uint64_t)bb.w0 * (uint32_t)W + aa.w0;
+    const uint64_t t1 = (uint64_t)bb.w1 * (uint32_t)W + (((uint64_t)aa.w1) + (t0 >> 32));
+    const uint64_t t2 = (uint64_t)(uint32_t)bb.w32 * (uint32_t)W + ((aa.w32 & EPS) + (t1 >> 32));
+    const uint64_t t3 = (uint64_t)(uint32_t)(bb.w32 >> 32) * (uint32_t)W + ((aa.w32 >> 32) + (t2 >> 32));
+    const uint64_t c0 = reduce160_impl<CANON>((uint32_t)t0, (uint32_t)t1, (uint32_t)t2, (uint32_t)t3, (uint32_t)(t3 >> 32));
+    return Ext{c0, c1};
+}
+__device__ __forceinline__ Ext mul(Ext x, Ext y) { return mul_impl<true>(x, y); }
+__device__ __forceinline__ Ext mul_loose(Ext x, Ext y) { return mul_impl<false>(x, y); }
+#endif
+GL_H Ext mul(Ext x, Ext y) {
     uint64_t bb = mul(x.b, y.b);
     uint64_t c0 = add(mul(x.a, y.a), reduce128(bb * W, mulhi64(bb, W)));
     uint64_t c1 = add(mul(x.a, y.b), mul(x.b, y.a));
diff --git a/near-light-client_amd/csrc/poly.hpp b/near-light-client_amd/csrc/poly.hpp
--- a/near-light-client_amd/csrc/poly.hpp
+++ b/near-light-client_amd/csrc/poly.hpp
@@ -14,4 +14,5 @@
 void launch_table_to_leaves(hipStream_t st, const uint64_t* d_lde, size_t col_stride, uint32_t n_cols,
                             unsigned log_n, unsigned rate_bits, uint64_t* d_leaves);
 void launch_field_ops(hipStream_t st, const uint64_t* d_a, const uint64_t* d_b, size_t n, uint64_t* d_out);
+void launch_ext_ops(hipStream_t st, const uint64_t* d_a, const uint64_t* d_b, size_t n, uint64_t* d_out);
 }
diff --git a/near-light-client_amd/csrc/poly_kernels.hip b/near-light-client_amd/csrc/poly_kernels.hip
--- a/near-light-client_amd/csrc/poly_kernels.hip
+++ b/near-light-client_amd/csrc/poly_kernels.hip
@@ -310,4 +310,24 @@
     hipLaunchKernelGGL(k_field_ops, dim3((unsigned)((n + 255) / 256)), dim3(256), 0, st, d_a, d_b, n, d_out);
 }
 
-}
+__global__ void k_ext_ops(const uint64_t* __restrict__ a, const uint64_t* __restrict__ b, size_t n, uint64_t* __restrict__ out) {
+    size_t i = (size_t)blockIdx.x * blockDim.x + threadIdx.x;
+    if (i >= n) return;
+    const gl::Ext x{a[2 * i], a[2 * i + 1]}, y{b[2 * i], b[2 * i + 1]};
+    const gl::Ext pr = gl::mul(x, y), sc = gl::mul(x, y.a);
+    out[i] = pr.a;
+    out[n + i] = pr.b;
+    out[2 * n + i] = sc.a;
+    out[3 * n + i] = sc.b;
+    out[4 * n + i] = gl::reduce160((uint32_t)x.a, (uint32_t)(x.a >> 32), (uint32_t)x.b, (uint32_t)(x.b >> 32), (uint32_t)y.b);
+    const gl::Ext lp = gl::mul_loose(x, y);
+    out[5 * n + i] = gl::canon(lp.a);
+    out[6 * n + i] = gl::canon(lp.b);
+    out[7 * n + i] = gl::canon(gl::reduce160_loose((uint32_t)x.a, (uint32_t)(x.a >> 32), (uint32_t)x.b, (uint32_t)(x.b >> 32), (uint32_t)y.b));
+}
+void launch_ext_ops(hipStream_t st, const uint64_t* d_a, const uint64_t* d_b, size_t n, uint64_t* d_out) {
+    if (!n) return;
+    hipLaunchKernelGGL(k_ext_ops, dim3((unsigned)((n + 255) / 256)), dim3(256), 0, st, d_a, d_b, n, d_out);
+}
+
+}
diff --git a/near-light-client_amd/csrc/prover.hip b/near-light-client_amd/csrc/prover.hip
--- a/near-light-client_amd/csrc/prover.hip
+++ b/near-light-client_amd/csrc/prover.hip
@@ -203,6 +203,12 @@
     c->hasher = hasher;
     c->gates.assign(d.gates, d.gates + d.num_gates);
     for (const nlx_gate_desc& gt : c->gates) c->max_gate_constraints = std::max(c->max_gate_constraints, gate_num_constraints(gt));
+#ifdef NLX_GATEACC_LIMBS3
+    if (c->max_gate_constraints > GATEACC3_MAX_TERMS || d.num_partial_products + 1 > GATEACC3_MAX_TERMS) {
+        delete c;
+        return ctx->fail(NLX_E_INVAL, "a gate with more than %u constraints (this build accumulates them without carry counters)", GATEACC3_MAX_TERMS);
+    }
+#endif
     c->k_is.assign(d.k_is, d.k_is + d.num_routed_wires);
     c->d.gates = c->gates.data();
     c->d.k_is = c->k_is.data();
@@ -572,6 +578,12 @@
     if (!d_alpha_pows || !d_qvals || !d_qchunks) return NLX_E_NOMEM;
     launch_pow_table(st, d_alpha_pows, alphas[0], alphas[1], c->n_terms, c->n_terms);
     QuotientParams qp{};
+#ifdef NLX_GATEACC_LIMBS3
+    uint32_t* d_alpha_limbs = scratch.alloc_as<uint32_t>((size_t)2 * c->n_terms * 16);
+    if (!d_alpha_limbs) return NLX_E_NOMEM;
+    launch_pow_limbs(st, d_alpha_limbs, d_alpha_pows, 2 * c->n_terms);
+    qp.alpha_limbs = d_alpha_limbs;
+#endif
     qp.cs = c->cs->lde; qp.wires = cw->lde; qp.zs = cz->lde;
     qp.gates = c->d_gates; qp.k_is = c->d_k_is; qp.coset_base = c->d_coset_base;
     qp.w_n_table = ctx->tables.fwd[log_n];
diff --git a/near-light-client_amd/csrc/prover.hpp b/near-light-client_amd/csrc/prover.hpp
--- a/near-light-client_amd/csrc/prover.hpp
+++ b/near-light-client_amd/csrc/prover.hpp
@@ -34,6 +34,7 @@
     const uint64_t* zh_inv;
     const uint64_t* l0_scaled;
     const uint64_t* alpha_pows;
+    const uint32_t* alpha_limbs;
     uint64_t* out;
     uint64_t betas[2], gammas[2], pih[4];
     uint32_t alpha_stride;
@@ -142,6 +143,8 @@
                             size_t out_stride_words);
 void launch_shift_indices(hipStream_t st, const uint64_t* d_in, uint64_t* d_out, uint32_t n, unsigned shift);
 void launch_pow_table(hipStream_t st, uint64_t* d_out, uint64_t a0, uint64_t a1, uint32_t count, uint32_t stride);
+void launch_pow_limbs(hipStream_t st, uint32_t* d_out, const uint64_t* d_pows, uint32_t count);
+constexpr uint32_t GATEACC3_MAX_TERMS = 1024;
 void launch_ext_pow_table(hipStream_t st, uint64_t* d_out, const uint64_t alpha[2], uint32_t count);
 
 }
diff --git a/near-light-client_amd/csrc/prover_kernels.hip b/near-light-client_amd/csrc/prover_kernels.hip
--- a/near-light-client_amd/csrc/prover_kernels.hip
+++ b/near-light-client_amd/csrc/prover_kernels.hip
@@ -1,5 +1,6 @@
 #include <hip/hip_runtime.h>
 #include "gl.hpp"
+#include "gate_acc.hpp"
 #include "poseidon.hpp"
 #include "poseidon_fast_constants.inc"
 #include "prover.hpp"
@@ -166,76 +167,60 @@
     return nc * (nb + nb2 + 2) + 16;
 }
 
-struct GateAcc {
-    const uint64_t* __restrict__ ap0;
-    const uint64_t* __restrict__ ap1;
-    uint64_t a[8];
-    uint32_t kc[8];
+struct GateAcc3 {
+    const uint32_t* __restrict__ lp0;
+    const uint32_t* __restrict__ lp1;
+    uint64_t a[12];
     uint32_t k;
     uint64_t base[2];
     __device__ __forceinline__ void reset() {
 #pragma unroll
-        for (int i = 0; i < 8; i++) { a[i] = 0; kc[i] = 0; }
+        for (int i = 0; i < 12; i++) a[i] = 0;
         k = 0;
         base[0] = base[1] = 0;
     }
     __device__ __forceinline__ void stash() {
-        base[0] = gl::add(base[0], fold_columns(a, kc));
-        base[1] = gl::add(base[1], fold_columns(a + 4, kc + 4));
-#pragma unroll
-        for (int i = 0; i < 8; i++) { a[i] = 0; kc[i] = 0; }
-    }
-    __device__ __forceinline__ void emit_at(uint32_t idx, uint64_t c) { mac(c, ap0[idx], ap1[idx]); }
-    __device__ __forceinline__ void mac(uint64_t c, uint64_t b0, uint64_t b1) {
+        base[0] = gl::add(base[0], fold(0));
+        base[1] = gl::add(base[1], fold(1));
+#pragma unroll
+        for (int i = 0; i < 12; i++) a[i] = 0;
+    }
+    __device__ __forceinline__ void emit_at(uint32_t idx, uint64_t c) {
         const uint32_t c0 = (uint32_t)c, c1 = (uint32_t)(c >> 32);
-        asm("v_mad_u64_u32 %[a0], vcc, %[c0], %[p0], %[a0]\n\t"
-            "v_addc_co_u32 %[k0], vcc, 0, %[k0], vcc\n\t"
-            "v_mad_u64_u32 %[a1], vcc, %[c0], %[p1], %[a1]\n\t"
-            "v_addc_co_u32 %[k1], vcc, 0, %[k1], vcc\n\t"
-            "v_mad_u64_u32 %[a2], vcc, %[c1], %[p0], %[a2]\n\t"
-            "v_addc_co_u32 %[k2], vcc, 0, %[k2], vcc\n\t"
-            "v_mad_u64_u32 %[a3], vcc, %[c1], %[p1], %[a3]\n\t"
-            "v_addc_co_u32 %[k3], vcc, 0, %[k3], vcc\n\t"
-            "v_mad_u64_u32 %[a4], vcc, %[c0], %[q0], %[a4]\n\t"
-            "v_addc_co_u32 %[k4], vcc, 0, %[k4], vcc\n\t"
-            "v_mad_u64_u32 %[a5], vcc, %[c0], %[q1], %[a5]\n\t"
-            "v_addc_co_u32 %[k5], vcc, 0, %[k5], vcc\n\t"
-            "v_mad_u64_u32 %[a6], vcc, %[c1], %[q0], %[a6]\n\t"
-            "v_addc_co_u32 %[k6], vcc, 0, %[k6], vcc\n\t"
-            "v_mad_u64_u32 %[a7], vcc, %[c1], %[q1], %[a7]\n\t"
-            "v_addc_co_u32 %[k7], vcc, 0, %[k7], vcc"
-            : [a0] "+v"(a[0]), [a1] "+v"(a[1]), [a2] "+v"(a[2]), [a3] "+v"(a[3]), [a4] "+v"(a[4]), [a5] "+v"(a[5]),
-              [a6] "+v"(a[6]), [a7] "+v"(a[7]), [k0] "+v"(kc[0]), [k1] "+v"(kc[1]), [k2] "+v"(kc[2]), [k3] "+v"(kc[3]),
-              [k4] "+v"(kc[4]), [k5] "+v"(kc[5]), [k6] "+v"(kc[6]), [k7] "+v"(kc[7])
-            : [c0] "v"(c0), [c1] "v"(c1), [p0] "s"((uint32_t)b0), [p1] "s"((uint32_t)(b0 >> 32)), [q0] "s"((uint32_t)b1),
-              [q1] "s"((uint32_t)(b1 >> 32))
-            : "vcc");
+#pragma unroll
+        for (int j = 0; j < 3; j++) {
+            const uint32_t l0 = lp0[4 * idx + j], l1 = lp1[4 * idx + j];
+            a[j] += (uint64_t)c0 * l0;
+            a[3 + j] += (uint64_t)c1 * l0;
+            a[6 + j] += (uint64_t)c0 * l1;
+            a[9 + j] += (uint64_t)c1 * l1;
+        }
     }
     __device__ __forceinline__ void emit(uint64_t c) { emit_at(k++, c); }
-    __device__ __forceinline__ uint64_t finish(int ch) const { return gl::add(fold_columns(a + 4 * ch, kc + 4 * ch), base[ch]); }
-    static __device__ __forceinline__ uint64_t fold_columns(const uint64_t* A, const uint32_t* K) {
-        uint32_t t1, t2, t3, t4, m0, m1, cm;
-        asm("v_add_co_u32 %[m0], vcc, %[a1l], %[a2l]\n\t"
-            "v_addc_co_u32 %[m1], vcc, %[a1h], %[a2h], vcc\n\t"
-            "v_addc_co_u32 %[cm], vcc, 0, 0, vcc\n\t"
-            "v_add_co_u32 %[t1], vcc, %[a0h], %[m0]\n\t"
-            "v_addc_co_u32 %[t2], vcc, %[m1], %[a3l], vcc\n\t"
-            "v_addc_co_u32 %[t3], vcc, %[cm], %[a3h], vcc\n\t"
-            "v_addc_co_u32 %[t4], vcc, 0, %[k3], vcc\n\t"
-            "v_add_co_u32 %[t2], vcc, %[t2], %[k0]\n\t"
-            "v_addc_co_u32 %[t3], vcc, %[t3], %[k1], vcc\n\t"
-            "v_addc_co_u32 %[t4], vcc, 0, %[t4], vcc\n\t"
-            "v_add_co_u32 %[t3], vcc, %[t3], %[k2]\n\t"
-            "v_addc_co_u32 %[t4], vcc, 0, %[t4], vcc"
-            : [t1] "=&v"(t1), [t2] "=&v"(t2), [t3] "=&v"(t3), [t4] "=&v"(t4), [m0] "=&v"(m0), [m1] "=&v"(m1), [cm] "=&v"(cm)
-            : [a0h] "v"((uint32_t)(A[0] >> 32)), [a1l] "v"((uint32_t)A[1]), [a1h] "v"((uint32_t)(A[1] >> 32)), [a2l] "v"((uint32_t)A[2]),
-              [a2h] "v"((uint32_t)(A[2] >> 32)), [a3l] "v"((uint32_t)A[3]), [a3h] "v"((uint32_t)(A[3] >> 32)), [k0] "v"(K[0]),
-              [k1] "v"(K[1]), [k2] "v"(K[2]), [k3] "v"(K[3])
-            : "vcc");
-        const uint64_t r = gl::canon(gl32::to_u64(gl32::reduce128((uint32_t)A[0], t1, t2, t3)));
-        return gl::sub(r, (uint64_t)t4 << 32);
+    __device__ __forceinline__ uint64_t finish(int ch) const { return gl::add(fold(ch), base[ch]); }
+    __device__ __forceinline__ uint64_t fold(int ch) const {
+        const uint64_t* A = a + 6 * ch;
+        typedef unsigned __int128 u128;
+        const u128 t = (u128)A[0] + ((u128)A[1] << 22) + ((u128)A[2] << 44) + ((u128)A[3] << 32) + ((u128)A[4] << 54) +
+                       ((u128)(A[5] & 0xFFFFFu) << 76);
+        const uint64_t lo = (uint64_t)t, hi = (uint64_t)(t >> 64);
+        return gl::sub(gl::reduce160((uint32_t)lo, (uint32_t)(lo >> 32), (uint32_t)hi, (uint32_t)(hi >> 32), 0u), A[5] >> 20);
     }
 };
+#ifdef NLX_GATEACC_LIMBS3
+typedef GateAcc3 QuotAcc;
+#else
+typedef GateAcc QuotAcc;
+#endif
+__device__ __forceinline__ void quot_acc_base(QuotAcc& acc, const QuotientParams& p, uint32_t first) {
+#ifdef NLX_GATEACC_LIMBS3
+    acc.lp0 = p.alpha_limbs + 4 * (size_t)first;
+    acc.lp1 = p.alpha_limbs + 4 * ((size_t)p.alpha_stride + first);
+#else
+    acc.ap0 = p.alpha_pows + first;
+    acc.ap1 = p.alpha_pows + p.alpha_stride + first;
+#endif
+}
 
 struct DotAcc {
     uint64_t a[4];
@@ -270,6 +255,7 @@
         hi += th + (lo < tl ? 1u : 0u);
     }
     __device__ __forceinline__ uint64_t value() const { return gl::reduce128(lo, hi); }
+    __device__ __forceinline__ uint64_t loose() const { return gl::reduce128_loose(lo, hi); }
 };
 
 __device__ __forceinline__ uint64_t limb4(uint64_t l) {
@@ -283,6 +269,7 @@
     __builtin_amdgcn_sched_barrier(0);
     return r;
 }
+template <bool CANON = true>
 __device__ __forceinline__ void mds_canon(uint64_t (&s)[12]) {
     constexpr uint32_t C[12] = {17, 15, 41, 16, 2, 28, 13, 13, 39, 18, 34, 20};
     uint64_t o[12];
@@ -298,7 +285,7 @@
             al += (uint64_t)(uint32_t)s[0] * 8u;
             ah += (uint64_t)(uint32_t)(s[0] >> 32) * 8u;
         }
-        o[r] = gl::canon(gl32::to_u64(gl32::fold_acc(al, ah)));
+        o[r] = CANON ? gl::canon(gl32::to_u64(gl32::fold_acc(al, ah))) : gl32::to_u64(gl32::fold_acc(al, ah));
         __builtin_amdgcn_sched_barrier(0);
     }
 #pragma unroll
@@ -346,12 +333,12 @@
     };
     if (parts & 1u) {
         const uint64_t swap = W(24);
-        acc.emit_at(0, gl::mul(swap, gl::sub(swap, 1)));
+        acc.emit_at(0, gl::mul_loose(swap, gl::sub(swap, 1)));
         uint64_t st[12];
 #pragma unroll
         for (int i = 0; i < 4; i++) {
             const uint64_t lhs = W(i), rhs = W(i + 4), delta = W(25 + i);
-            acc.emit_at(1 + i, gl::sub(gl::mul(swap, gl::sub(rhs, lhs)), delta));
+            acc.emit_at(1 + i, gl::sub(gl::mul_loose(swap, gl::sub(rhs, lhs)), delta));
             st[i] = gl::add(lhs, delta);
             st[i + 4] = gl::sub(rhs, delta);
         }
@@ -401,11 +388,11 @@
     uint64_t st[12];
     if (parts & 1u) {
         const uint64_t swap = W(24);
-        acc.emit_at(0, gl::mul(swap, gl::sub(swap, 1)));
+        acc.emit_at(0, gl::mul_loose(swap, gl::sub(swap, 1)));
 #pragma unroll
         for (int i = 0; i < 4; i++) {
             const uint64_t lhs = W(i), rhs = W(i + 4), delta = W(25 + i);
-            acc.emit_at(1 + i, gl::sub(gl::mul(swap, gl::sub(rhs, lhs)), delta));
+            acc.emit_at(1 + i, gl::sub(gl::mul_loose(swap, gl::sub(rhs, lhs)), delta));
             st[i] = gl::add(lhs, delta);
             st[i + 4] = gl::sub(rhs, delta);
         }
@@ -417,12 +404,12 @@
         for (int r = 0; r < 3; r++) {
 #pragma unroll
             for (int i = 0; i < 12; i++) st[i] = sbox7c(st[i]);
-            mds_canon(st);
+            mds_canon<false>(st);
             __builtin_amdgcn_sched_barrier(0);
 #pragma unroll
             for (int i = 0; i < 12; i++) {
                 const uint64_t in = W(29 + 12 * r + i);
-                acc.emit_at(5 + 12 * r + i, gl::sub(gl::add(st[i], RC[(r + 1) * 12 + i]), in));
+                acc.emit_at(5 + 12 * r + i, gl::sub(gl::add_loose(st[i], RC[(r + 1) * 12 + i]), in));
                 st[i] = in;
                 __builtin_amdgcn_sched_barrier(0);
             }
@@ -476,13 +463,13 @@
             if (r != 0) {
 #pragma unroll
                 for (int i = 0; i < 12; i++) {
-                    acc.emit_at(63 + 12 * r + i, gl::sub(gl::add(st[i], RC[(26 + r) * 12 + i]), W(87 + 12 * r + i)));
+                    acc.emit_at(63 + 12 * r + i, gl::sub(gl::add_loose(st[i], RC[(26 + r) * 12 + i]), W(87 + 12 * r + i)));
                     __builtin_amdgcn_sched_barrier(0);
                 }
             }
 #pragma unroll
             for (int i = 0; i < 12; i++) st[i] = sbox7c(W(87 + 12 * r + i));
-            mds_canon(st);
+            mds_canon<false>(st);
             __builtin_amdgcn_sched_barrier(0);
         }
 #pragma unroll
@@ -513,19 +500,19 @@
             const uint64_t c0 = CC(p.gate_const0), c1 = CC(p.gate_const0 + 1);
             for (uint32_t i = 0; i < gd.param0; i++) {
                 const uint64_t m0 = W(4 * i), m1 = W(4 * i + 1), ad = W(4 * i + 2), o = W(4 * i + 3);
-                acc.emit(gl::sub(o, gl::add(gl::mul(gl::mul(m0, m1), c0), gl::mul(ad, c1))));
+                acc.emit(gl::sub(o, gl::canon(gl::add_loose(gl::mul_loose(gl::mul_loose(m0, m1), c0), gl::mul(ad, c1)))));
             }
             break;
         }
         case NLX_GATE_BASE_SUM: {
             const uint32_t B = gd.param0, nl = gd.param1;
             uint64_t sum = 0;
-            for (uint32_t i = nl; i-- > 0;) sum = gl::add(gl::mul(sum, (uint64_t)B), W(1 + i));
+            for (uint32_t i = nl; i-- > 0;) sum = gl::add_loose(gl::mul_loose(sum, (uint64_t)B), W(1 + i));
             acc.emit(gl::sub(sum, W(0)));
             for (uint32_t i = 0; i < nl; i++) {
                 const uint64_t limb = W(1 + i);
                 uint64_t prod = 1;
-                for (uint32_t t = 0; t < B; t++) prod = gl::mul(prod, gl::sub(limb, (uint64_t)t));
+                for (uint32_t t = 0; t < B; t++) prod = gl::mul_loose(prod, gl::sub(limb, (uint64_t)t));
                 acc.emit(prod);
             }
             break;
@@ -563,12 +550,12 @@
             for (uint32_t i = 0; i < nco; i++) {
                 const uint32_t aw = (i == nco - 1) ? 0 : start_accs + 2 * i;
                 const gl::Ext nxt{W(aw), W(aw + 1)};
-                const gl::Ext pr = gl::mul(a, alpha);
+                const gl::Ext pr = gl::mul_loose(a, alpha);
                 if (ext) {
-                    acc.emit(gl::sub(gl::add(pr.a, W(start_coeffs + 2 * i)), nxt.a));
-                    acc.emit(gl::sub(gl::add(pr.b, W(start_coeffs + 2 * i + 1)), nxt.b));
+                    acc.emit(gl::sub(gl::add_loose(pr.a, W(start_coeffs + 2 * i)), nxt.a));
+                    acc.emit(gl::sub(gl::add_loose(pr.b, W(start_coeffs + 2 * i + 1)), nxt.b));
                 } else {
-                    acc.emit(gl::sub(gl::add(pr.a, W(start_coeffs + i)), nxt.a));
+                    acc.emit(gl::sub(gl::add_loose(pr.a, W(start_coeffs + i)), nxt.a));
                     acc.emit(gl::sub(pr.b, nxt.b));
                 }
                 a = nxt;
@@ -597,11 +584,11 @@
             const uint64_t base = W(0);
             uint64_t prev_iv = 1;
             for (uint32_t i = 0; i < nb; i++) {
-                const uint64_t prev = i ? gl::mul(prev_iv, prev_iv) : 1;
+                const uint64_t prev = i ? gl::mul_loose(prev_iv, prev_iv) : 1;
                 const uint64_t bit = W(1 + (nb - 1 - i));
-                const uint64_t sel = gl::add(gl::mul(bit, base), gl::sub(1, bit));
+                const uint64_t sel = gl::add_loose(gl::mul_loose(bit, base), gl::sub(1, bit));
                 const uint64_t iv = W(2 + nb + i);
-                acc.emit(gl::sub(gl::mul(prev, sel), iv));
+                acc.emit(gl::sub(gl::mul_loose(prev, sel), iv));
                 prev_iv = iv;
             }
             acc.emit(gl::sub(W(1 + nb), prev_iv));
@@ -614,7 +601,7 @@
                 uint64_t computed = W(b0 + na);
                 for (uint32_t j = 0; j < na; j++) computed = gl::add(computed, W(b0 + j));
                 const uint64_t res = W(b0 + na + 1), cy = W(b0 + na + 2);
-                acc.emit(gl::sub(gl::add(gl::mul(cy, 1ULL << 32), res), computed));
+                acc.emit(gl::sub(gl::add_loose(gl::mul_loose(cy, 1ULL << 32), res), computed));
                 Sum128 cr, cc;
                 for (uint32_t j = nl; j-- > 0;) {
                     const uint64_t l = W(lb + j);
@@ -622,8 +609,8 @@
                     if (j < nrl) cr.add(l, 2 * j);
                     else cc.add(l, 2 * (j - nrl));
                 }
-                acc.emit(gl::sub(cr.value(), res));
-                acc.emit(gl::sub(cc.value(), cy));
+                acc.emit(gl::sub(cr.loose(), res));
+                acc.emit(gl::sub(cc.loose(), cy));
             }
             break;
         }
@@ -633,9 +620,9 @@
                 const uint32_t b0 = 6 * i, lb = 6 * nops + 32 * i;
                 const uint64_t computed = gl::add(gl::mul(W(b0), W(b0 + 1)), W(b0 + 2));
                 const uint64_t lo = W(b0 + 3), hi = W(b0 + 4), inv = W(b0 + 5);
-                const uint64_t hi_not_max = gl::sub(gl::mul(inv, gl::sub(0xFFFFFFFFULL, hi)), 1);
-                acc.emit(gl::mul(hi_not_max, lo));
-                acc.emit(gl::sub(gl::add(gl::mul(hi, 1ULL << 32), lo), computed));
+                const uint64_t hi_not_max = gl::sub(gl::mul_loose(inv, gl::sub(0xFFFFFFFFULL, hi)), 1);
+                acc.emit(gl::mul_loose(hi_not_max, lo));
+                acc.emit(gl::sub(gl::add_loose(gl::mul_loose(hi, 1ULL << 32), lo), computed));
                 Sum128 cl, ch;
                 for (uint32_t j = 32; j-- > 0;) {
                     const uint64_t l = W(lb + j);
@@ -643,8 +630,8 @@
                     if (j < 16) cl.add(l, 2 * j);
                     else ch.add(l, 2 * (j - 16));
                 }
-                acc.emit(gl::sub(cl.value(), lo));
-                acc.emit(gl::sub(ch.value(), hi));
+                acc.emit(gl::sub(cl.loose(), lo));
+                acc.emit(gl::sub(ch.loose(), hi));
             }
             break;
         }
@@ -661,8 +648,8 @@
                     acc.emit(limb4(l));
                     c.add(l, 2 * j);
                 }
-                acc.emit(gl::sub(c.value(), res));
-                acc.emit(gl::mul(bo, gl::sub(1, bo)));
+                acc.emit(gl::sub(c.loose(), res));
+                acc.emit(gl::mul_loose(bo, gl::sub(1, bo)));
             }
             break;
         }
@@ -672,7 +659,7 @@
                 const uint32_t ab = nin + 16 * i;
                 Sum128 sum;
                 for (uint32_t j = 0; j < 16; j++) sum.add(W(ab + j), 2 * j);
-                acc.emit(gl::sub(sum.value(), W(i)));
+                acc.emit(gl::sub(sum.loose(), W(i)));
                 for (uint32_t j = 0; j < 16; j++) acc.emit(limb4(W(ab + j)));
             }
             break;
@@ -685,8 +672,8 @@
                 fcomb.add(W(fc + i), cb * i);
                 scomb.add(W(sc + i), cb * i);
             }
-            acc.emit(gl::sub(fcomb.value(), W(0)));
-            acc.emit(gl::sub(scomb.value(), W(1)));
+            acc.emit(gl::sub(fcomb.loose(), W(0)));
+            acc.emit(gl::sub(scomb.loose(), W(1)));
             uint64_t msd = 0;
             for (uint32_t i = 0; i < nch; i++) {
                 const uint64_t f = W(fc + i), s2 = W(sc + i);
@@ -698,23 +685,23 @@
                     p1 = f;
                     p2 = s2;
                     for (uint32_t x2 = 1; x2 < (1u << cb); x2++) {
-                        p1 = gl::mul(p1, gl::sub(f, (uint64_t)x2));
-                        p2 = gl::mul(p2, gl::sub(s2, (uint64_t)x2));
+                        p1 = gl::mul_loose(p1, gl::sub(f, (uint64_t)x2));
+                        p2 = gl::mul_loose(p2, gl::sub(s2, (uint64_t)x2));
                     }
                 }
                 acc.emit(p1);
                 acc.emit(p2);
                 const uint64_t diff = gl::sub(s2, f), e = W(ceq + i), ivv = W(iv + i);
-                acc.emit(gl::sub(gl::mul(diff, W(eqd + i)), gl::sub(1, e)));
-                acc.emit(gl::mul(e, diff));
+                acc.emit(gl::sub(gl::mul_loose(diff, W(eqd + i)), gl::sub(1, e)));
+                acc.emit(gl::mul_loose(e, diff));
                 acc.emit(gl::sub(ivv, gl::mul(e, msd)));
-                msd = gl::add(ivv, gl::mul(gl::sub(1, e), diff));
-            }
-            acc.emit(gl::sub(W(3), msd));
+                msd = gl::add_loose(gl::mul_loose(gl::sub(1, e), diff), ivv);
+            }
+            acc.emit(gl::sub(W(3), gl::canon(msd)));
             uint64_t bc = 0;
             for (uint32_t b = 0; b <= cb; b++) {
                 const uint64_t bit = W(msb + b);
-                acc.emit(gl::mul(bit, gl::sub(1, bit)));
+                acc.emit(gl::mul_loose(bit, gl::sub(1, bit)));
             }
             for (uint32_t b = cb + 1; b-- > 0;) bc = gl::add(gl::add(bc, bc), W(msb + b));
             acc.emit(gl::sub(gl::add(1ULL << cb, W(3)), bc));
@@ -739,11 +726,14 @@
                 for (uint32_t j = start; j < end; j++) {
                     const uint64_t xj = root_pow(p.w_n_table, j * stride, half);
                     const gl::Ext term{gl::sub(pt.a, xj), pt.b};
-                    const gl::Ext vp = gl::mul(gl::Ext{W(1 + 2 * j), W(2 + 2 * j)}, pr);
-                    ev = gl::add(gl::mul(ev, term), gl::mul(vp, gl::mul(xj, np_inv)));
-                    pr = gl::mul(pr, term);
+                    const gl::Ext vp = gl::mul_loose(gl::Ext{W(1 + 2 * j), W(2 + 2 * j)}, pr);
+                    const gl::Ext et = gl::mul_loose(ev, term), vs = gl::mul(vp, gl::mul(xj, np_inv));
+                    ev = gl::Ext{gl::add_loose(et.a, vs.a), gl::add_loose(et.b, vs.b)};
+                    pr = gl::mul_loose(pr, term);
                 }
+                ev = gl::Ext{gl::canon(ev.a), gl::canon(ev.b)};
                 if (c < ni) {
+                    pr = gl::Ext{gl::canon(pr.a), gl::canon(pr.b)};
                     const gl::Ext ie{W(si + 2 * c), W(si + 2 * c + 1)}, ip{W(si + 2 * (ni + c)), W(si + 2 * (ni + c) + 1)};
                     acc.emit(gl::sub(ie.a, ev.a));
                     acc.emit(gl::sub(ie.b, ev.b));
@@ -764,7 +754,7 @@
                 const uint32_t b0 = (2 + vec) * cpy, bw = rt + cpy * bits;
                 for (uint32_t i = 0; i < bits; i++) {
                     const uint64_t b = W(bw + i);
-                    acc.emit(gl::mul(b, gl::sub(b, 1)));
+                    acc.emit(gl::mul_loose(b, gl::sub(b, 1)));
                 }
                 uint64_t rec = 0;
                 for (uint32_t i = bits; i-- > 0;) rec = gl::add(gl::add(rec, rec), W(bw + i));
@@ -778,10 +768,10 @@
                     while (sp > 0 && depth_of[sp - 1] == lvl) {
                         const uint64_t left = stack[--sp];
                         const uint64_t b = W(bw + lvl);
-                        v = gl::add(left, gl::mul(b, gl::sub(v, left)));
+                        v = gl::add_loose(gl::mul_loose(b, gl::sub(v, left)), left);
                         lvl++;
                     }
-                    stack[sp] = v;
+                    stack[sp] = lvl ? gl::canon(v) : v;
                     depth_of[sp] = lvl;
                     sp++;
                 }
@@ -836,9 +826,7 @@
     const uint64_t* ap1 = p.alpha_pows + p.alpha_stride;
     uint64_t tot0 = 0, tot1 = 0;
     uint64_t l0a = 0, l0b = 0;
-    GateAcc acc;
-    acc.ap0 = ap0 + T0;
-    acc.ap1 = ap1 + T0;
+    QuotAcc acc;
     const uint32_t* work = p.work + (size_t)wv * p.work_stride;
     for (uint32_t wi = 0;; wi++) {
         const uint32_t word = __builtin_amdgcn_readfirstlane(work[wi]);
@@ -849,9 +837,10 @@
             const uint64_t s = CC(gd.selector_index);
             uint64_t f = 1;
             for (uint32_t i = gd.group_start; i < gd.group_end; i++)
-                if (i != gd.index) f = gl::mul(f, gl::sub((uint64_t)i, s));
-            if (p.n_selectors > 1) f = gl::mul(f, gl::sub(0xFFFFFFFFULL, s));
+                if (i != gd.index) f = gl::mul_loose(f, gl::sub((uint64_t)i, s));
+            if (p.n_selectors > 1) f = gl::mul_loose(f, gl::sub(0xFFFFFFFFULL, s));
             acc.reset();
+            quot_acc_base(acc, p, T0);
             eval_gate(gd, p, W, CC, acc, n, parts);
             tot0 = gl::add(tot0, gl::mul(f, acc.finish(0)));
             tot1 = gl::add(tot1, gl::mul(f, acc.finish(1)));
@@ -871,6 +860,8 @@
             l0a = gl::add(l0a, gl::mul(zm1, ap0[c]));
             l0b = gl::add(l0b, gl::mul(zm1, ap1[c]));
             uint64_t accv = z_x;
+            acc.reset();
+            quot_acc_base(acc, p, nc + c * (npp + 1));
 #pragma unroll 1
             for (uint32_t q = 0; q < n_chunks; q++) {
                 uint64_t nm = 1, dn = 1;
@@ -881,12 +872,12 @@
                     dn = gl::mul_loose(dn, gl::add_loose(gl::mul_loose(beta, sg), wg));
                 }
                 const uint64_t new_acc = (q + 1 < n_chunks) ? ZS(nc + c * npp + q) : z_gx;
-                const uint64_t term = gl::sub(gl::mul(accv, nm), gl::mul(new_acc, dn));
-                const uint32_t t = nc + c * (npp + 1) + q;
-                tot0 = gl::add(tot0, gl::mul(term, ap0[t]));
-                tot1 = gl::add(tot1, gl::mul(term, ap1[t]));
+                const uint64_t term = gl::sub(gl::mul_loose(accv, nm), gl::mul(new_acc, dn));
+                acc.emit_at(q, term);
                 accv = new_acc;
             }
+            tot0 = gl::add(tot0, acc.finish(0));
+            tot1 = gl::add(tot1, acc.finish(1));
         }
     }
     __syncthreads();
@@ -942,9 +933,8 @@
         if (i != gd.index) f = gl::mul(f, gl::sub((uint64_t)i, s));
     if (p.n_selectors > 1) f = gl::mul(f, gl::sub(0xFFFFFFFFULL, s));
     const uint32_t T0 = p.nc + p.nc * (p.npp + 1) + p.nc * p.n_lk_terms;
-    GateAcc acc;
-    acc.ap0 = p.alpha_pows + T0;
-    acc.ap1 = p.alpha_pows + p.alpha_stride + T0;
+    QuotAcc acc;
+    quot_acc_base(acc, p, T0);
     acc.reset();
     gate_poseidon_mx(W, acc, 2u);
     uint64_t t0 = gl::mul(f, acc.finish(0)), t1 = gl::mul(f, acc.finish(1));
@@ -1312,6 +1302,18 @@
     out[t] = gl::pow(a0, t);
     out[stride + t] = gl::pow(a1, t);
 }
+__global__ void k_pow_limbs(uint32_t* __restrict__ out, const uint64_t* __restrict__ pows, uint32_t count) {
+    const uint32_t t = blockIdx.x * blockDim.x + threadIdx.x;
+    if (t >= count) return;
+    const uint64_t v = pows[t];
+    out[4 * t] = (uint32_t)v & 0x3FFFFFu;
+    out[4 * t + 1] = (uint32_t)(v >> 22) & 0x3FFFFFu;
+    out[4 * t + 2] = (uint32_t)(v >> 44);
+    out[4 * t + 3] = 0;
+}
+void launch_pow_limbs(hipStream_t st, uint32_t* d_out, const uint64_t* d_pows, uint32_t count) {
+    hipLaunchKernelGGL(k_pow_limbs, dim3((count + 63) / 64), dim3(64), 0, st, d_out, d_pows, count);
+}
 void launch_pow_table(hipStream_t st, uint64_t* d_out, uint64_t a0, uint64_t a1, uint32_t count, uint32_t stride) {
     hipLaunchKernelGGL(k_pow_table, dim3((count + 63) / 64), dim3(64), 0, st, d_out, a0, a1, count, stride);
 }
diff --git a/near-light-client_amd/csrc/stark.hip b/near-light-client_amd/csrc/stark.hip
--- a/near-light-client_amd/csrc/stark.hip
+++ b/near-light-client_amd/csrc/stark.hip
@@ -583,7 +583,10 @@
     uint64_t* d_qvals = scratch.alloc_as<uint64_t>((size_t)nc * Q * 8);
     uint64_t* d_qchunks = scratch.alloc_as<uint64_t>((size_t)nc * Q * 8);
     uint64_t* d_part = n_seg > 1 ? scratch.alloc_as<uint64_t>((size_t)n_seg * nc * Q * 8) : nullptr;
-    if (!d_pis || !d_cols || !d_qvals || !d_qchunks || (n_seg > 1 && !d_part)) return NLX_E_NOMEM;
+    const uint32_t n_apow = s->n_constraints + 1;
+    uint64_t* d_apow = s->gen ? scratch.alloc_as<uint64_t>((size_t)2 * n_apow * 8) : nullptr;
+    if (!d_pis || !d_cols || !d_qvals || !d_qchunks || (n_seg > 1 && !d_part) || (s->gen && !d_apow)) return NLX_E_NOMEM;
+    if (s->gen) launch_pow_table(st, d_apow, alphas[0], alphas[1], n_apow, n_apow);
     NLX_HIP(ctx, hipMemcpyAsync(d_pis, values.data(), values.size() * 8, hipMemcpyHostToDevice, st));
     NLX_HIP(ctx, hipMemcpyAsync(d_cols, h_cols.data(), (size_t)ncols * 8, hipMemcpyHostToDevice, st));
     {
@@ -594,6 +597,7 @@
         ap.w_n_table = ctx->tables.fwd[log_n];
         ap.out = d_qvals;
         ap.alphas[0] = alphas[0]; ap.alphas[1] = alphas[1];
+        ap.alpha_pows = d_apow; ap.alpha_stride = n_apow;
         ap.g_inv = gl::inv(gl::root_of_unity(log_n));
         ap.log_n = log_n; ap.rate_bits = d.rate_bits; ap.qdb = qdb; ap.n_words = d.n_words; ap.nc = nc;
         ap.n_regs = s->n_regs; ap.n_pis = d.num_public_inputs;
```

After: 23.56 (median of 6 runs). 1.4% higher.
